# JuliaMolSim/DFTK.jl

Hardware: AMD Instinct MI355X
Metric: SCF iterations/sec (Hψ applies/sec) at fixed Ecut·atoms (higher is better)
Workload: dtype f64

## Files before the change

### dftk.jl_amd/_lib.py

```python
from __future__ import annotations

import ctypes as C
import os

from . import _build

c_cplx_p = C.c_void_p
_i64 = C.c_int64


class dftk_mi_cplx(C.Structure):
    _fields_ = [("re", C.c_double), ("im", C.c_double)]


class dftk_mi_batch_op(C.Structure):
    _fields_ = ([(name, C.c_int32) for name in ("type", "fiber", "trans", "m", "k", "i0", "mode", "flags", "join_next",
                                                 "sync_after", "status", "reserved")] +
                [(name, _i64) for name in ("n", "gm", "gn", "gk", "lda", "ldb", "ldc")] +
                [("alpha", dftk_mi_cplx), ("beta", dftk_mi_cplx), ("s0", C.c_double)] +
                [(name, C.c_void_p) for name in ("A", "B", "W", "W2", "W3", "C", "D", "E", "F", "kb", "host")] +
                [("bytes", C.c_uint64)])


class DftkMiError(RuntimeError):
    def __init__(self, status, msg):
        super().__init__(f"dftk_mi355x status {status}: {msg}")
        self.status = status


_SIGNATURES = {
    "dftk_mi_last_error": (C.c_char_p, []),
    "dftk_mi_version": (C.c_char_p, []),
    "dftk_mi_basis_create": (C.c_int, [C.c_int, C.c_int, C.c_int, C.c_double, C.c_int, C.POINTER(C.c_void_p)]),
    "dftk_mi_basis_destroy": (C.c_int, [C.c_void_p]),
    "dftk_mi_basis_sync": (C.c_int, [C.c_void_p]),
    "dftk_mi_basis_set_fft_batch": (C.c_int, [C.c_void_p, C.c_int]),
    "dftk_mi_basis_stream": (C.c_void_p, [C.c_void_p]),
    "dftk_mi_kblock_create": (C.c_int, [C.c_void_p, _i64, C.c_void_p, C.c_void_p, C.POINTER(C.c_void_p)]),
    "dftk_mi_kblock_destroy": (C.c_int, [C.c_void_p]),
    "dftk_mi_kblock_set_projectors": (C.c_int, [C.c_void_p, C.c_int, C.c_void_p, _i64, C.c_void_p]),
    "dftk_mi_kblock_set_potential": (C.c_int, [C.c_void_p, C.c_void_p]),
    "dftk_mi_apply_H": (C.c_int, [C.c_void_p, C.c_int, C.c_void_p, _i64, C.c_void_p, _i64]),
    "dftk_mi_apply_H_parts": (C.c_int, [C.c_void_p, C.c_int, C.c_int, C.c_void_p, _i64, C.c_void_p, _i64]),
    "dftk_mi_local_potential": (C.c_int, [C.c_void_p, C.c_void_p, C.c_void_p, C.c_void_p, C.c_int, C.c_void_p,
                                          C.c_void_p]),
    "dftk_mi_local_potential_collinear": (C.c_int, [C.c_void_p, C.c_void_p, C.c_void_p, C.c_void_p, C.c_int, C.c_void_p,
                                                    C.c_void_p]),
    "dftk_mi_density_accumulate_spin": (C.c_int, [C.c_void_p, C.c_int, C.c_void_p, _i64, C.c_void_p, C.c_void_p, C.c_int,
                                                  C.c_int]),
    "dftk_mi_kpoint_sphere_host": (C.c_int, [C.c_int, C.c_int, C.c_int, C.c_void_p, C.c_void_p, C.c_double, _i64,
                                             C.POINTER(_i64), C.c_void_p, C.c_void_p, C.c_void_p]),
    "dftk_mi_build_projectors_hgh": (C.c_int, [C.c_void_p, _i64, C.c_void_p, C.c_void_p, C.c_void_p, C.c_double, C.c_int,
                                               C.c_void_p, C.c_void_p, C.c_int, C.c_void_p, C.c_void_p, C.c_void_p, _i64,
                                               C.POINTER(C.c_int)]),
    "dftk_mi_atomic_superposition": (C.c_int, [C.c_void_p, C.c_int, C.c_void_p, C.c_int, C.c_void_p, C.c_int, C.c_void_p,
                                               C.c_void_p, C.c_void_p]),
    "dftk_mi_forces_local": (C.c_int, [C.c_void_p, C.c_void_p, C.c_int, C.c_void_p, C.c_int, C.c_void_p, C.c_void_p,
                                       C.c_void_p, C.c_void_p]),
    "dftk_mi_radial_transform": (C.c_int, [C.c_void_p, C.c_int, C.c_int, C.c_int, C.c_void_p, C.c_void_p, C.c_double, _i64,
                                           C.c_void_p, C.c_void_p]),
    "dftk_mi_radial_tile": (C.c_int, []),
    "dftk_mi_build_projectors_radial": (C.c_int, [C.c_void_p, _i64, C.c_void_p, C.c_void_p, C.c_void_p, C.c_double,
                                                  C.c_int, C.c_void_p, _i64, C.c_void_p, C.c_void_p, C.c_int, C.c_void_p,
                                                  C.c_void_p, C.c_void_p, _i64, C.POINTER(C.c_int)]),
    "dftk_mi_atomic_superposition_table": (C.c_int, [C.c_void_p, C.c_void_p, C.c_int, C.c_void_p, C.c_int, C.c_void_p,
                                                     C.c_void_p, C.c_void_p, C.c_void_p]),
    "dftk_mi_forces_local_table": (C.c_int, [C.c_void_p, C.c_void_p, C.c_int, C.c_void_p, C.c_int, C.c_void_p, C.c_void_p,
                                             C.c_void_p, C.c_void_p]),
    "dftk_mi_forces_nonlocal": (C.c_int, [C.c_void_p, C.c_void_p, C.c_int, C.c_void_p, _i64, C.c_void_p, C.c_int,
                                          C.c_void_p, C.c_void_p]),
    "dftk_mi_local_potential_displacement": (C.c_int, [C.c_void_p, C.c_void_p, C.c_int, C.c_void_p, C.c_int, C.c_void_p,
                                                       C.c_void_p]),
    "dftk_mi_dynmat_local": (C.c_int, [C.c_void_p, C.c_void_p, C.c_int, C.c_void_p, C.c_int, C.c_void_p, C.c_void_p,
                                       C.c_void_p, C.c_void_p]),
    "dftk_mi_nonlocal_displacement_apply": (C.c_int, [C.c_void_p, C.c_void_p, C.c_int, C.c_int, C.c_void_p, C.c_int,
                                                      C.c_void_p, _i64, C.c_void_p, _i64]),
    "dftk_mi_dynmat_nonlocal": (C.c_int, [C.c_void_p, C.c_void_p, C.c_int, C.c_void_p, _i64, C.c_void_p, _i64, C.c_void_p,
                                          C.c_void_p, C.c_int, C.c_void_p, C.c_void_p, C.c_void_p]),
    "dftk_mi_stress_kinetic_nonlocal": (C.c_int, [C.c_void_p, C.c_void_p, C.c_void_p, C.c_int, C.c_void_p, _i64, C.c_void_p,
                                                  C.c_int, C.c_void_p, C.c_void_p, C.c_int, C.c_void_p, C.c_void_p,
                                                  C.c_void_p, C.c_void_p]),
    "dftk_mi_stress_cube": (C.c_int, [C.c_void_p, C.c_void_p, C.c_int, C.c_void_p, C.c_int, C.c_void_p, C.c_void_p,
                                      C.c_void_p, C.c_void_p]),
    "dftk_mi_stress_xc": (C.c_int, [C.c_void_p, _i64, C.c_int, C.c_void_p, C.c_void_p, C.c_void_p, C.c_void_p, C.c_void_p,
                                    C.c_void_p]),
    "dftk_mi_xc_gga": (C.c_int, [C.c_void_p, _i64, C.c_void_p, C.c_void_p, C.c_int, C.c_double, C.c_void_p, C.c_void_p,
                                 C.c_void_p]),
    "dftk_mi_ifft_sphere": (C.c_int, [C.c_void_p, C.c_void_p, C.c_void_p]),
    "dftk_mi_fft_sphere": (C.c_int, [C.c_void_p, C.c_void_p, C.c_void_p]),
    "dftk_mi_density_accumulate": (C.c_int, [C.c_void_p, C.c_int, C.c_void_p, _i64, C.c_void_p, C.c_void_p]),
    "dftk_mi_sternheimer": (C.c_int, [C.c_void_p, C.c_int, C.c_void_p, _i64, C.c_void_p, C.c_int, C.c_void_p, _i64, C.c_void_p,
                                      _i64, C.c_void_p, C.c_int, C.c_int, C.c_void_p, _i64, C.c_void_p, _i64,
                                      C.POINTER(C.c_int), C.c_void_p, C.POINTER(C.c_int)]),
    "dftk_mi_density_response_accumulate": (C.c_int, [C.c_void_p, C.c_int, C.c_void_p, _i64, C.c_void_p, _i64, C.c_void_p,
                                                      C.c_void_p, C.c_void_p]),
    "dftk_mi_apply_kernel": (C.c_int, [C.c_void_p, C.c_void_p, C.c_void_p, C.c_void_p, C.c_int, C.c_void_p]),
    "dftk_mi_exx_apply": (C.c_int, [C.c_void_p, C.c_int, C.c_void_p, _i64, C.c_void_p, C.c_void_p, C.c_int, C.c_void_p, _i64,
                                    C.c_void_p, _i64, C.c_int]),
    "dftk_mi_lobpcg": (C.c_int, [C.c_void_p, C.c_int, C.c_void_p, _i64, C.c_double, C.c_int, C.c_int, C.c_int,
                                 C.c_int, C.c_uint64, C.c_void_p, C.c_void_p, C.POINTER(C.c_int),
                                 C.POINTER(C.c_int), C.POINTER(_i64)]),
    "dftk_mi_local_potential_gga": (C.c_int, [C.c_void_p, C.c_void_p, C.c_void_p, C.c_void_p, C.c_void_p, C.c_int,
                                              C.c_double, C.c_void_p, C.c_void_p]),
    "dftk_mi_local_potential_collinear_gga": (C.c_int, [C.c_void_p, C.c_void_p, C.c_void_p, C.c_void_p, C.c_void_p, C.c_int,
                                                        C.c_double, C.c_void_p, C.c_void_p]),
    "dftk_mi_local_potential_core": (C.c_int, [C.c_void_p, C.c_void_p, C.c_int, C.c_void_p, C.c_void_p, C.c_void_p,
                                               C.c_void_p, C.c_void_p, C.c_int, C.c_double, C.c_void_p, C.c_void_p]),
    "dftk_mi_cube_gradient": (C.c_int, [C.c_void_p, C.c_void_p, C.c_void_p, C.c_void_p]),
    "dftk_mi_xc_gga_spin": (C.c_int, [C.c_void_p, _i64, C.c_void_p, C.c_void_p, C.c_int, C.c_double, C.c_void_p, C.c_void_p,
                                      C.c_void_p]),
    "dftk_mi_symmetrize_rho": (C.c_int, [C.c_void_p, C.c_int, C.c_void_p, C.c_void_p, C.c_int, C.c_void_p, C.c_void_p]),
    "dftk_mi_mix_kerker": (C.c_int, [C.c_void_p, C.c_void_p, C.c_double, C.c_void_p, C.c_void_p]),
    "dftk_mi_mix_dielectric": (C.c_int, [C.c_void_p, C.c_void_p, C.c_double, C.c_double, C.c_void_p, C.c_void_p]),
    "dftk_mi_chi0_dielectric_apply": (C.c_int, [C.c_void_p, C.c_void_p, C.c_double, C.c_double, C.c_void_p, C.c_void_p]),
    "dftk_mi_cube_fourier_filter": (C.c_int, [C.c_void_p, C.c_void_p, C.c_void_p, C.c_void_p]),
    "dftk_mi_kblocks_set_potential": (C.c_int, [C.c_int, C.c_void_p, C.c_void_p]),
    "dftk_mi_lobpcg_multi": (C.c_int, [C.c_int, C.c_void_p, C.c_int, C.c_void_p, C.c_void_p, C.c_double, C.c_int, C.c_int,
                                       C.c_int, C.c_int, C.c_void_p, C.c_void_p, C.c_void_p, C.c_void_p, C.c_void_p,
                                       C.c_void_p, C.c_void_p]),
    "dftk_mi_density_accumulate_multi": (C.c_int, [C.c_int, C.c_void_p, C.c_void_p, C.c_void_p, C.c_void_p, C.c_void_p,
                                                   C.c_void_p]),
    "dftk_mi_density_accumulate_multi2": (C.c_int, [C.c_int, C.c_void_p, C.c_void_p, C.c_void_p, C.c_void_p, C.c_void_p,
                                                    C.c_void_p, C.c_void_p, C.c_void_p]),
    "dftk_mi_band_kinetic_multi": (C.c_int, [C.c_int, C.c_void_p, C.c_void_p, C.c_void_p, C.c_void_p, C.c_void_p]),
    "dftk_mi_batch_stats": (C.c_int, [C.POINTER(_i64), C.POINTER(_i64), C.POINTER(_i64), C.POINTER(_i64)]),
    "dftk_mi_lobpcg_small_stats": (C.c_int, [C.POINTER(_i64), C.POINTER(_i64)]),
    "dftk_mi_ortho_small": (C.c_int, [C.c_void_p, _i64, C.c_int, C.c_void_p, _i64, C.c_int, C.c_void_p, _i64, C.c_void_p,
                                      C.c_double, C.c_void_p]),
    "dftk_mi_batch_replay": (C.c_int, [C.c_void_p, C.c_int, C.c_int, C.c_void_p]),
    "dftk_mi_lobpcg_last_AX": (C.c_void_p, [C.c_void_p]),
    "dftk_mi_lobpcg_history": (C.c_int, [C.c_void_p, C.POINTER(C.c_int), C.POINTER(C.c_int), C.c_void_p, C.c_size_t,
                                         C.POINTER(C.c_int)]),
    "dftk_mi_columnwise_norms": (C.c_int, [C.c_void_p, _i64, C.c_int, C.c_void_p, _i64, C.c_void_p]),
    "dftk_mi_columnwise_dots": (C.c_int, [C.c_void_p, _i64, C.c_int, C.c_void_p, _i64, C.c_void_p, _i64, C.c_void_p]),
    "dftk_mi_ortho_qr": (C.c_int, [C.c_void_p, _i64, C.c_int, C.c_void_p, _i64, C.c_int, C.POINTER(C.c_int),
                                   C.POINTER(C.c_int)]),
    "dftk_mi_tpa_precondprep": (C.c_int, [C.c_void_p, C.c_int, C.c_void_p, _i64, C.c_void_p]),
    "dftk_mi_tpa_ldiv": (C.c_int, [C.c_void_p, C.c_int, C.c_void_p, _i64, C.c_void_p, C.c_double, C.c_void_p, _i64]),
    "dftk_mi_block_residual": (C.c_int, [C.c_void_p, C.c_int, C.c_void_p, _i64, C.c_void_p, _i64, C.c_void_p,
                                         C.c_void_p, _i64, C.c_void_p, C.c_void_p, C.c_void_p]),
    "dftk_mi_kblock_set_gamma_real": (C.c_int, [C.c_void_p, C.c_int]),
    "dftk_mi_gamma_half_size": (C.c_int, [C.c_void_p, C.POINTER(_i64)]),
    "dftk_mi_gamma_tables_host": (C.c_int, [C.c_int, C.c_int, C.c_int, _i64, C.c_void_p, C.POINTER(_i64), C.c_void_p,
                                            C.c_void_p]),
    "dftk_mi_gamma_compress": (C.c_int, [C.c_void_p, C.c_int, C.c_void_p, _i64, C.c_void_p, _i64]),
    "dftk_mi_gamma_compress_aligned": (C.c_int, [C.c_void_p, C.c_int, C.c_void_p, _i64, C.c_void_p, _i64]),
    "dftk_mi_gamma_expand": (C.c_int, [C.c_void_p, C.c_int, C.c_void_p, _i64, C.c_void_p, _i64]),
    "dftk_mi_gamma_apply_H": (C.c_int, [C.c_void_p, C.c_int, C.c_int, C.c_void_p, _i64, C.c_void_p, _i64]),
    "dftk_mi_density_accumulate_real": (C.c_int, [C.c_void_p, C.c_int, C.c_void_p, _i64, C.c_void_p, C.c_void_p]),
    "dftk_mi_shard_plan_host": (C.c_int, [C.c_int, C.c_int, C.c_int, C.c_void_p, C.c_void_p, C.c_void_p, C.c_void_p,
                                          C.c_void_p, C.c_void_p]),
    "dftk_mi_kblock_set_shard": (C.c_int, [C.c_void_p, C.c_void_p, C.c_void_p]),
    "dftk_mi_zgemm": (C.c_int, [C.c_void_p, C.c_char, _i64, _i64, _i64, dftk_mi_cplx, C.c_void_p, _i64,
                                C.c_void_p, _i64, dftk_mi_cplx, C.c_void_p, _i64]),
    "dftk_mi_zgemm_ex": (C.c_int, [C.c_void_p, C.c_char, _i64, _i64, _i64, dftk_mi_cplx, C.c_void_p, _i64,
                                   C.c_void_p, _i64, dftk_mi_cplx, C.c_void_p, _i64, C.c_int]),
    "dftk_mi_zgemm_plan_host": (C.c_int, [C.c_char, _i64, _i64, _i64, C.c_int, C.POINTER(C.c_int)]),
    "dftk_mi_heev": (C.c_int, [C.c_void_p, C.c_int, C.c_void_p, _i64, C.c_void_p, C.c_void_p, _i64]),
    "dftk_mi_prof_zgemm_shapes": (C.c_int, [C.c_void_p, C.c_int, C.c_void_p, C.c_void_p, C.POINTER(C.c_int)]),
    "dftk_mi_heev_lowest": (C.c_int, [C.c_void_p, C.c_int, C.c_int, C.c_void_p, _i64, C.c_void_p, C.c_void_p, _i64]),
    "dftk_mi_heev_sigma_host": (C.c_int, [C.c_int, C.c_void_p, C.c_int, C.POINTER(C.c_double), C.POINTER(C.c_double),
                                          C.POINTER(C.c_int), C.c_double]),
    "dftk_mi_potrf_trtri": (C.c_int, [C.c_void_p, C.c_int, C.c_void_p, _i64, C.c_void_p, _i64]),
    "dftk_mi_potrf_trtri_real": (C.c_int, [C.c_void_p, C.c_int, C.c_void_p, _i64, C.c_void_p, _i64]),
    "dftk_mi_comm_get_unique_id": (C.c_int, [C.c_char_p]),
    "dftk_mi_comm_init_rank": (C.c_int, [C.c_char_p, C.c_int, C.c_int, C.c_int, C.POINTER(C.c_void_p)]),
    "dftk_mi_comm_create_host": (C.c_int, [C.c_int, C.c_int, C.c_int, C.c_void_p, C.c_void_p, C.c_void_p,
                                           C.POINTER(C.c_void_p)]),
    "dftk_mi_comm_destroy": (C.c_int, [C.c_void_p]),
    "dftk_mi_comm_describe": (C.c_int, [C.c_void_p, C.POINTER(C.c_int), C.POINTER(C.c_int), C.POINTER(C.c_int)]),
    "dftk_mi_comm_rank": (C.c_int, [C.c_void_p]),
    "dftk_mi_comm_size": (C.c_int, [C.c_void_p]),
    "dftk_mi_allreduce_sum_f64": (C.c_int, [C.c_void_p, C.c_void_p, C.c_size_t, C.c_void_p]),
    "dftk_mi_prof_enable": (C.c_int, [C.c_void_p, C.c_int]),
    "dftk_mi_prof_get": (C.c_int, [C.c_void_p, C.c_int, C.POINTER(C.c_double), C.POINTER(C.c_double),
                                   C.POINTER(_i64)]),
    "dftk_mi_anderson_create": (C.c_int, [C.c_void_p, _i64, C.c_int, C.c_double, C.c_double, C.POINTER(C.c_void_p)]),
    "dftk_mi_anderson_destroy": (C.c_int, [C.c_void_p]),
    "dftk_mi_anderson_reset": (C.c_int, [C.c_void_p]),
    "dftk_mi_anderson_history": (C.c_int, [C.c_void_p]),
    "dftk_mi_anderson_step": (C.c_int, [C.c_void_p, C.c_void_p, C.c_double, C.c_void_p, C.c_void_p, C.POINTER(C.c_int)]),
    "dftk_mi_chi0_mix": (C.c_int, [C.c_void_p, C.c_int, C.c_void_p, C.c_void_p, C.c_void_p, C.c_double, C.c_int, C.c_double,
                                   C.c_double, C.c_void_p, C.c_double, C.c_int, C.c_int, C.c_void_p, C.POINTER(C.c_int),
                                   C.POINTER(C.c_int)]),
    "dftk_mi_launch_count": (C.c_int, [C.POINTER(_i64), C.POINTER(_i64)]),
    "dftk_mi_device_buffers_live": (C.c_int, [C.POINTER(_i64), C.POINTER(_i64)]),
    "dftk_mi_kblock_reuse_AX": (C.c_int, [C.c_void_p, C.c_int]),
    "dftk_mi_ax_reuse_count": (C.c_int, [C.POINTER(_i64)]),
    "dftk_mi_planes_reuse_count": (C.c_int, [C.POINTER(_i64)]),
    "dftk_mi_step_sums": (C.c_int, [C.c_void_p, _i64, C.c_void_p, C.c_void_p, C.c_void_p, C.c_void_p]),
    "dftk_mi_fermi_bisection": (C.c_int, [C.c_int, C.c_void_p, C.c_void_p, C.c_void_p, C.c_int, C.c_double, C.c_double,
                                          C.c_double, C.c_double, C.c_double, C.POINTER(C.c_double)]),
    "dftk_mi_diag_mfma_peak": (C.c_int, [C.c_void_p, C.c_int, C.c_int, C.POINTER(C.c_double)]),
    "dftk_mi_jacobi_schedule_host": (C.c_int, [C.c_int, C.c_int, C.POINTER(C.c_int), C.POINTER(C.c_int),
                                               C.POINTER(C.c_int)]),
    "dftk_mi_fft_plan_host": (C.c_int, [C.c_int, C.POINTER(C.c_int), C.POINTER(C.c_int), C.POINTER(C.c_int)]),
    "dftk_mi_sphere_tables_host": (C.c_int, [C.c_int, C.c_int, C.c_int, _i64, C.c_void_p, C.POINTER(_i64),
                                             C.POINTER(C.c_int), C.c_void_p, C.c_void_p]),
}

ALLREDUCE_FN = C.CFUNCTYPE(C.c_int, C.c_void_p, C.POINTER(C.c_double), C.c_size_t)
ALLTOALLV_FN = C.CFUNCTYPE(C.c_int, C.c_void_p, C.POINTER(C.c_double), C.POINTER(C.c_size_t), C.POINTER(C.c_size_t),
                           C.POINTER(C.c_double), C.POINTER(C.c_size_t), C.POINTER(C.c_size_t))

EXPORTED_SYMBOLS = tuple(_SIGNATURES)
_lib = None


def load(build_if_missing: bool = True):
    global _lib
    if _lib is not None:
        return _lib
    path = _build.LIBPATH
    if build_if_missing and _build.needs_build():
        _build.build()
    if not os.path.exists(path):
        raise RuntimeError(f"{path} is missing and could not be built; the MI355X hot path has no fallback")
    lib = C.CDLL(path, mode=C.RTLD_GLOBAL)
    for name, (res, args) in _SIGNATURES.items():
        fn = getattr(lib, name)
        fn.restype = res
        fn.argtypes = args
    version = lib.dftk_mi_version().decode()
    if not version.endswith("src=" + _build.source_hash()):
        raise RuntimeError(f"{path} was built from other sources ({version!r}, expected src={_build.source_hash()}): "
                           "stale binary, rebuild with python -m dftk_jl_amd._build")
    _lib = lib
    return lib


def check(status: int):
    if status != 0:
        msg = load().dftk_mi_last_error().decode(errors="replace")
        raise DftkMiError(status, msg)


def cplx(z) -> dftk_mi_cplx:
    z = complex(z)
    return dftk_mi_cplx(z.real, z.imag)
```

### dftk.jl_amd/csrc/api.cpp

```cpp
#include "common.h"
#include <chrono>
#include "batch.h"
#include <algorithm>
#include <cmath>
#include <cstdarg>
#include <cstdio>
#include <cstdlib>
#include <cstring>
#include <vector>

static thread_local char g_err[1024] = "";

void dftk_set_error(const char* fmt, ...) {
    va_list ap;
    va_start(ap, fmt);
    vsnprintf(g_err, sizeof(g_err), fmt, ap);
    va_end(ap);
}

extern "C" const char* dftk_mi_last_error(void) { return g_err; }

hipError_t dftk_scratch_malloc(void** p, size_t bytes) {
    static const bool poison = getenv("DFTK_MI_POISON") != nullptr;
    hipError_t e = hipMalloc(p, bytes);
// ... 1075 lines not shown
    HIPCHK(hipSetDevice(b->device));
    return stress_xc(b, n, n_spin, rho_d, vrho_d, e_d, vsigma_d, grad_d, out_h);
}

extern "C" int dftk_mi_xc_gga(dftk_mi_basis* b, int64_t n, const double* rho_d, const double* sigma_d, int xc_functionals,
                              double density_threshold, double* e_d, double* vrho_d, double* vsigma_d) {
    if (!b || n < 0 || !rho_d || !sigma_d || !e_d || !vrho_d || !vsigma_d || (xc_functionals & ~24) || !xc_functionals)
        return DFTK_MI_EINVAL;
    if (n == 0) return 0;
    HIPCHK(hipSetDevice(b->device));
    return xc_gga_pointwise(b, n, rho_d, sigma_d, xc_functionals, density_threshold, e_d, vrho_d, vsigma_d);
}

extern "C" int dftk_mi_xc_gga_spin(dftk_mi_basis* b, int64_t n, const double* rho_d, const double* sigma_d,
                                   int xc_functionals, double density_threshold, double* e_d, double* vrho_d,
                                   double* vsigma_d) {
    if (!b || n < 0 || !rho_d || !sigma_d || !e_d || !vrho_d || !vsigma_d || (xc_functionals & ~24) || !xc_functionals)
        return DFTK_MI_EINVAL;
    if (n == 0) return 0;
    HIPCHK(hipSetDevice(b->device));
    return xc_gga_spin_pointwise(b, n, rho_d, sigma_d, xc_functionals, density_threshold, e_d, vrho_d, vsigma_d);
}

extern "C" int dftk_mi_ifft_sphere(dftk_mi_kblock* kb, const dftk_mi_cplx* c_d, dftk_mi_cplx* cube_d) {
    if (!kb || !c_d || !cube_d) return DFTK_MI_EINVAL;
    HIPCHK(hipSetDevice(kb->basis->device));
    return launch_ifft_to_cube(kb, reinterpret_cast<const cd*>(c_d), reinterpret_cast<cd*>(cube_d));
}

extern "C" int dftk_mi_fft_sphere(dftk_mi_kblock* kb, const dftk_mi_cplx* cube_d, dftk_mi_cplx* c_d) {
    if (!kb || !c_d || !cube_d) return DFTK_MI_EINVAL;
    HIPCHK(hipSetDevice(kb->basis->device));
    return launch_fft_from_cube(kb, reinterpret_cast<const cd*>(cube_d), reinterpret_cast<cd*>(c_d));
}

extern "C" int dftk_mi_density_accumulate(dftk_mi_kblock* kb, int n_bands, const dftk_mi_cplx* psi_d, int64_t ld_psi,
                                          const double* weight_h, double* rho_d) {
    if (!kb || !psi_d || !weight_h || !rho_d || n_bands < 0 || ld_psi < local_rows(kb)) return DFTK_MI_EINVAL;
    if (n_bands == 0) return 0;
    HIPCHK(hipSetDevice(kb->basis->device));
    if (!kb->sh_comm) {
        prof_count(kb->basis, PROF_A2A_MODEL, 16.0 * (double)kb->n_G * n_bands);
        return launch_density(kb, n_bands, reinterpret_cast<const cd*>(psi_d), ld_psi, weight_h, rho_d);
    }
    if (ld_psi != local_rows(kb)) {
        dftk_set_error("sharded density: blocks must be packed (leading dimension == local rows)");
        return DFTK_MI_EINVAL;
    }
    cd *R1, *F, *Gf;
    CHK(shard_buffers(kb, n_bands, &R1, &F, &Gf));
    Transposer t(kb, n_bands);
    CHK(t.to_bands(reinterpret_cast<const cd*>(psi_d), R1, F));
    if (t.mine == 0) return 0;
    return launch_density(kb, t.mine, F, kb->n_G, weight_h + t.c0[t.me], rho_d);
}

extern "C" int dftk_mi_density_accumulate_spin(dftk_mi_kblock* kb, int n_bands, const dftk_mi_cplx* psi_d, int64_t ld_psi,
                                               const double* weight_h, double* rho_d, int spin, int n_spin) {
    if (!kb || !rho_d || n_spin < 1 || n_spin > 2 || spin < 0 || spin >= n_spin) return DFTK_MI_EINVAL;
    const int64_t N = (int64_t)kb->basis->nx * kb->basis->ny * kb->basis->nz;
    return dftk_mi_density_accumulate(kb, n_bands, psi_d, ld_psi, weight_h, rho_d + (int64_t)spin * N);
}

extern "C" int dftk_mi_kblock_set_gamma_real(dftk_mi_kblock* kb, int on) {
    if (!kb) return DFTK_MI_EINVAL;
    HIPCHK(hipSetDevice(kb->basis->device));
    return gamma_enable(kb, on);
}

extern "C" int dftk_mi_gamma_tables_host(int nx, int ny, int nz, int64_t n_G, const int64_t* mapping0_h,
                                         int64_t* n_half, int32_t* row_h, int32_t* partner_row_h) {
    if (nx < 1 || ny < 1 || nz < 1 || n_G < 1 || !mapping0_h || !n_half) return DFTK_MI_EINVAL;
    if ((row_h == nullptr) != (partner_row_h == nullptr)) return DFTK_MI_EINVAL;
    return gamma_tables_host(nx, ny, nz, n_G, mapping0_h, n_half, row_h, partner_row_h);
}

static int gamma_ready(dftk_mi_kblock* kb) {
    if (!kb || !kb->gr || !kb->gr->d_g) {
        dftk_set_error("gamma_real: call dftk_mi_kblock_set_gamma_real(kb, 1) first");
        return DFTK_MI_EINVAL;
    }
    return 0;
}

extern "C" int dftk_mi_gamma_half_size(dftk_mi_kblock* kb, int64_t* n_half) {
    if (!n_half) return DFTK_MI_EINVAL;
    CHK(gamma_ready(kb));
    *n_half = gamma_local_rows(kb);
    return 0;
}

extern "C" int dftk_mi_gamma_compress(dftk_mi_kblock* kb, int m, const dftk_mi_cplx* X_d, int64_t ldx,
                                      dftk_mi_cplx* Xh_d, int64_t ldh) {
    CHK(gamma_ready(kb));
    if (m < 0 || !X_d || !Xh_d || ldx < local_rows(kb) || ldh < gamma_local_rows(kb)) return DFTK_MI_EINVAL;
    HIPCHK(hipSetDevice(kb->basis->device));
    if (kb->sh_comm)
        return gamma_lobpcg_load(kb, m, reinterpret_cast<const cd*>(X_d), ldx, reinterpret_cast<cd*>(Xh_d), ldh);
    return gamma_compress(kb, m, reinterpret_cast<const cd*>(X_d), ldx, reinterpret_cast<cd*>(Xh_d), ldh);
}

extern "C" int dftk_mi_gamma_compress_aligned(dftk_mi_kblock* kb, int m, const dftk_mi_cplx* X_d, int64_t ldx,
                                              dftk_mi_cplx* Xh_d, int64_t ldh) {
    CHK(gamma_ready(kb));
    if (m < 0 || !X_d || !Xh_d || ldx < local_rows(kb) || ldh < gamma_local_rows(kb)) return DFTK_MI_EINVAL;
    HIPCHK(hipSetDevice(kb->basis->device));
    return gamma_lobpcg_load(kb, m, reinterpret_cast<const cd*>(X_d), ldx, reinterpret_cast<cd*>(Xh_d), ldh, true);
}

extern "C" int dftk_mi_gamma_expand(dftk_mi_kblock* kb, int m, const dftk_mi_cplx* Xh_d, int64_t ldh,
                                    dftk_mi_cplx* X_d, int64_t ldx) {
    CHK(gamma_ready(kb));
    if (m < 0 || !X_d || !Xh_d || ldx < local_rows(kb) || ldh < gamma_local_rows(kb)) return DFTK_MI_EINVAL;
    HIPCHK(hipSetDevice(kb->basis->device));
    if (kb->sh_comm)
        return gamma_lobpcg_store(kb, m, reinterpret_cast<const cd*>(Xh_d), ldh, reinterpret_cast<cd*>(X_d), ldx);
    return gamma_expand(kb, m, reinterpret_cast<const cd*>(Xh_d), ldh, reinterpret_cast<cd*>(X_d), ldx);
}

extern "C" int dftk_mi_gamma_apply_H(dftk_mi_kblock* kb, int which, int n_bands, const dftk_mi_cplx* psih_d,
                                     int64_t ld_psi, dftk_mi_cplx* Hpsih_d, int64_t ld_Hpsi) {
    CHK(gamma_ready(kb));
    if (!psih_d || !Hpsih_d || n_bands < 0 || (which & ~7) || ld_psi < gamma_local_rows(kb) ||
        ld_Hpsi < gamma_local_rows(kb))
        return DFTK_MI_EINVAL;
    HIPCHK(hipSetDevice(kb->basis->device));
    return gamma_apply_H(kb, which, n_bands, reinterpret_cast<const cd*>(psih_d), ld_psi,
                         reinterpret_cast<cd*>(Hpsih_d), ld_Hpsi);
}

extern "C" int dftk_mi_density_accumulate_real(dftk_mi_kblock* kb, int n_bands, const dftk_mi_cplx* psi_d,
                                               int64_t ld_psi, const double* weight_h, double* rho_d) {
    if (!kb || !psi_d || !weight_h || !rho_d || n_bands < 0 || ld_psi < local_rows(kb)) return DFTK_MI_EINVAL;
    if (n_bands == 0) return 0;
    HIPCHK(hipSetDevice(kb->basis->device));
    if (!kb->sh_comm) prof_count(kb->basis, PROF_A2A_MODEL, 8.0 * (double)kb->n_G * n_bands);
    return gamma_density(kb, n_bands, reinterpret_cast<const cd*>(psi_d), ld_psi, weight_h, rho_d);
}

extern "C" int dftk_mi_lobpcg(dftk_mi_kblock* kb, int M, dftk_mi_cplx* X_d, int64_t ldX, double tol, int miniter,
                              int maxiter, int n_conv_check, int use_tpa, uint64_t seed, double* lambda_h,
                              double* resid_h, int* n_iter, int* converged, int64_t* n_matvec) {
    if (!kb || !X_d || M < 1 || ldX < local_rows(kb) || !lambda_h || !resid_h || !n_iter || !converged || !n_matvec ||
        maxiter < 0)
        return DFTK_MI_EINVAL;
    HIPCHK(hipSetDevice(kb->basis->device));
    return lobpcg_run(kb, M, reinterpret_cast<cd*>(X_d), ldX, tol, miniter, maxiter, n_conv_check, use_tpa, seed,
                      lambda_h, resid_h, n_iter, converged, n_matvec);
}

extern "C" int dftk_mi_lobpcg_multi(int n_kblocks, dftk_mi_kblock* const* kbs, int M, dftk_mi_cplx* const* X_d,
                                    const int64_t* ldX, double tol, int miniter, int maxiter, int n_conv_check, int use_tpa,
                                    const uint64_t* seeds, double* lambda_h, double* resid_h, int* n_iter, int* converged,
                                    int64_t* n_matvec, int* status) {
    if (n_kblocks < 0 || (n_kblocks > 0 && (!kbs || !X_d || !ldX || !lambda_h || !resid_h || !n_iter || !converged ||
                                            !n_matvec || !status)) || M < 1 || maxiter < 0)
        return DFTK_MI_EINVAL;
    if (n_kblocks == 0) return 0;
    for (int i = 0; i < n_kblocks; ++i)
        if (!kbs[i] || !X_d[i] || ldX[i] < local_rows(kbs[i])) return DFTK_MI_EINVAL;
    HIPCHK(hipSetDevice(kbs[0]->basis->device));
    return lobpcg_run_multi(n_kblocks, kbs, M, reinterpret_cast<cd* const*>(X_d), ldX, tol, miniter, maxiter, n_conv_check,
                            use_tpa, seeds, lambda_h, resid_h, n_iter, converged, n_matvec, status);
}

extern "C" int dftk_mi_band_kinetic_multi(int n_kblocks, dftk_mi_kblock* const* kbs, const int* n_bands,
                                          const dftk_mi_cplx* const* psi_d, const int64_t* ld_psi, double* out_h) {
    if (n_kblocks < 0 || (n_kblocks > 0 && (!kbs || !n_bands || !psi_d || !ld_psi || !out_h))) return DFTK_MI_EINVAL;
    if (n_kblocks == 0) return 0;
    dftk_mi_basis* b = kbs[0] ? kbs[0]->basis : nullptr;
    if (!b) return DFTK_MI_EINVAL;
    size_t total = 0;
    for (int i = 0; i < n_kblocks; ++i) {
        if (!kbs[i] || kbs[i]->basis != b || kbs[i]->sh_comm || !psi_d[i] || n_bands[i] < 0 || ld_psi[i] < kbs[i]->n_G)
            return DFTK_MI_EINVAL;
        total += (size_t)n_bands[i];
    }
    HIPCHK(hipSetDevice(b->device));
    CHK(ensure_ws(b, total * sizeof(double)));
    double* d = reinterpret_cast<double*>(b->ws.get());
    std::vector<std::function<int()>> bodies;
    size_t off = 0;
    for (int i = 0; i < n_kblocks; ++i) {
        const size_t o = off;
        off += (size_t)n_bands[i];
        bodies.push_back([=]() {
            if (n_bands[i] == 0) return 0;
            CHK(ew_weighted_colsums(b, kbs[i]->n_G, n_bands[i], reinterpret_cast<const cd*>(psi_d[i]), ld_psi[i], kbs[i]->d_kin,
                                    d + o));
            return dev_d2h_sync(b, out_h + o, d + o, (size_t)n_bands[i] * sizeof(double));
        });
    }
    std::vector<int> rets;
    CHK(batch_run(b, bodies, rets));
    for (int r : rets)
        if (r != 0) return r;
    return 0;
}

extern "C" int dftk_mi_density_accumulate_multi(int n_kblocks, dftk_mi_kblock* const* kbs, const int* n_bands,
                                                const dftk_mi_cplx* const* psi_d, const int64_t* ld_psi,
                                                const double* weights_h, double* rho_d) {
    return dftk_mi_density_accumulate_multi2(n_kblocks, kbs, n_bands, psi_d, ld_psi, weights_h, rho_d, nullptr, nullptr);
}

extern "C" int dftk_mi_density_accumulate_multi2(int n_kblocks, dftk_mi_kblock* const* kbs, const int* n_bands,
                                                 const dftk_mi_cplx* const* psi_d, const int64_t* ld_psi,
                                                 const double* weights_h, double* rho_d, const double* weights2_h,
                                                 double* rho2_d) {
    if (n_kblocks < 0 || (n_kblocks > 0 && (!kbs || !n_bands || !psi_d || !ld_psi || !weights_h)) || !rho_d ||
        ((weights2_h == nullptr) != (rho2_d == nullptr)) || (rho2_d && rho2_d == rho_d))
        return DFTK_MI_EINVAL;
    if (n_kblocks == 0) return 0;
    dftk_mi_basis* b = kbs[0] ? kbs[0]->basis : nullptr;
    if (!b) return DFTK_MI_EINVAL;
    for (int i = 0; i < n_kblocks; ++i)
        if (!kbs[i] || kbs[i]->basis != b || kbs[i]->sh_comm || !psi_d[i] || n_bands[i] < 0 || ld_psi[i] < kbs[i]->n_G)
            return DFTK_MI_EINVAL;
    HIPCHK(hipSetDevice(b->device));
    std::vector<std::function<int()>> bodies;
    size_t off = 0;
    for (int i = 0; i < n_kblocks; ++i) {
        const double* w = weights_h + off;
        const double* w2 = weights2_h ? weights2_h + off : nullptr;
        off += (size_t)n_bands[i];
        bodies.push_back([=]() {
            return launch_density(kbs[i], n_bands[i], reinterpret_cast<const cd*>(psi_d[i]), ld_psi[i], w, rho_d, nullptr, w2,
                                  rho2_d);
        });
    }
    std::vector<int> rets;
    CHK(batch_run(b, bodies, rets));
    for (int r : rets)
        if (r != 0) return r;
    return 0;
}

extern "C" int dftk_mi_fermi_bisection(int n_k, const int* n_bands, const double* eig, const double* kweights, int smearing,
                                       double temperature, double filled, double n_electrons, double lo, double hi,
                                       double* eF_out) {
    if (n_k < 1 || !n_bands || !eig || !kweights || !eF_out || !(temperature > 0.0) || (smearing != 1 && smearing != 2) ||
        !(lo <= hi))
        return DFTK_MI_EINVAL;
    auto excess = [&](double eF) {
        double total = 0.0;
        const double* e = eig;
        for (int k = 0; k < n_k; ++k) {
            double sk = 0.0;
            for (int i = 0; i < n_bands[k]; ++i) {
                const double x = (e[i] - eF) / temperature;
                double f;
                if (smearing == 2) {
                    f = 0.5 * std::erfc(x);
                } else if (x > 0) {
                    const double y = std::exp(-x);
                    f = y / (1.0 + y);
                } else {
                    f = 1.0 / (1.0 + std::exp(x));
                }
                sk += filled * f;
            }
            total += kweights[k] * sk;
            e += n_bands[k];
        }
        return total - n_electrons;
    };
    for (int it = 0; it < 200; ++it) {
        const double mid = 0.5 * (lo + hi);
        if (mid == lo || mid == hi) break;
        if (excess(mid) < 0)
            lo = mid;
        else
            hi = mid;
    }
    *eF_out = 0.5 * (lo + hi);
    return 0;
}

extern "C" int dftk_mi_kblock_reuse_AX(dftk_mi_kblock* kb, int on) {
    if (!kb) return DFTK_MI_EINVAL;
    kb->ho.promise(on != 0);
    return 0;
}

extern "C" const dftk_mi_cplx* dftk_mi_lobpcg_last_AX(dftk_mi_kblock* kb) {
    return kb ? reinterpret_cast<const dftk_mi_cplx*>(kb->ho.last_AX()) : nullptr;
}

extern "C" int dftk_mi_zgemm(dftk_mi_basis* b, char transA, int64_t m, int64_t n, int64_t k, dftk_mi_cplx alpha,
                             const dftk_mi_cplx* A_d, int64_t lda, const dftk_mi_cplx* B_d, int64_t ldb,
                             dftk_mi_cplx beta, dftk_mi_cplx* C_d, int64_t ldc) {
    if (!b || m < 0 || n < 0 || k < 0 || !C_d) return DFTK_MI_EINVAL;
    HIPCHK(hipSetDevice(b->device));
    cd al = {alpha.re, alpha.im}, be = {beta.re, beta.im};
    return zgemm(b, transA, m, n, k, al, reinterpret_cast<const cd*>(A_d), lda, reinterpret_cast<const cd*>(B_d), ldb,
                 be, reinterpret_cast<cd*>(C_d), ldc);
}

int zgemm_plan_host(char transA, int64_t m, int64_t n, int64_t k, int flags, int* out);
extern "C" int dftk_mi_zgemm_plan_host(char transA, int64_t m, int64_t n, int64_t k, int flags, int* out12) {
    return zgemm_plan_host(transA, m, n, k, flags, out12);
}

extern "C" int dftk_mi_zgemm_ex(dftk_mi_basis* b, char transA, int64_t m, int64_t n, int64_t k, dftk_mi_cplx alpha,
                                const dftk_mi_cplx* A_d, int64_t lda, const dftk_mi_cplx* B_d, int64_t ldb,
                                dftk_mi_cplx beta, dftk_mi_cplx* C_d, int64_t ldc, int flags) {
    if (!b || m < 0 || n < 0 || k < 0 || !C_d || (flags & ~(3 | DFTK_MI_GEMM_REAL))) return DFTK_MI_EINVAL;
    HIPCHK(hipSetDevice(b->device));
    cd al = {alpha.re, alpha.im}, be = {beta.re, beta.im};
    return zgemm(b, transA, m, n, k, al, reinterpret_cast<const cd*>(A_d), lda, reinterpret_cast<const cd*>(B_d), ldb,
                 be, reinterpret_cast<cd*>(C_d), ldc, flags);
}

extern "C" int dftk_mi_heev(dftk_mi_basis* b, int n, dftk_mi_cplx* A_d, int64_t lda, double* W_h, dftk_mi_cplx* V_d,
                            int64_t ldv) {
    if (!b || n < 1 || !A_d || !W_h || !V_d || lda < n || ldv < n) return DFTK_MI_EINVAL;
    HIPCHK(hipSetDevice(b->device));
    return dense_heev(b, n, reinterpret_cast<cd*>(A_d), lda, W_h, reinterpret_cast<cd*>(V_d), ldv);
}

extern "C" int dftk_mi_heev_lowest(dftk_mi_basis* b, int n, int nev, dftk_mi_cplx* A_d, int64_t lda, double* W_h,
                                   dftk_mi_cplx* V_d, int64_t ldv) {
    if (!b || n < 1 || nev < 1 || nev > n || !A_d || !W_h || !V_d || lda < n || ldv < n) return DFTK_MI_EINVAL;
    HIPCHK(hipSetDevice(b->device));
    return dense_heev_lowest(b, n, nev, reinterpret_cast<cd*>(A_d), lda, W_h, reinterpret_cast<cd*>(V_d), ldv);
}
extern "C" int dftk_mi_heev_sigma_host(int n, const double* diag_h, int nev, double* sigma, double* gap_guess,
                                       int* hold_iterations, double norm_bound) {
    const int st = eig_choose_sigma_host(n, diag_h, nev, sigma, gap_guess);
    if (st != 0) return st;
    if (hold_iterations) *hold_iterations = norm_bound > 0.0 ? eig_hold_iterations_host(*gap_guess / norm_bound) : 0;
    return 0;
}

extern "C" int dftk_mi_potrf_trtri(dftk_mi_basis* b, int n, dftk_mi_cplx* A_d, int64_t lda, dftk_mi_cplx* invR_d,
                                   int64_t ldi) {
    if (!b || n < 1 || !A_d || !invR_d || lda < n || ldi < n) return DFTK_MI_EINVAL;
    HIPCHK(hipSetDevice(b->device));
    double a, c;
    return dense_potrf_trtri(b, n, reinterpret_cast<cd*>(A_d), lda, reinterpret_cast<cd*>(invR_d), ldi, &a, &c);
}

extern "C" int dftk_mi_potrf_trtri_real(dftk_mi_basis* b, int n, dftk_mi_cplx* A_d, int64_t lda, dftk_mi_cplx* invR_d,
                                        int64_t ldi) {
    if (!b || n < 1 || !A_d || !invR_d || lda < n || ldi < n) return DFTK_MI_EINVAL;
    HIPCHK(hipSetDevice(b->device));
    double a, c;
    return dense_potrf_trtri(b, n, reinterpret_cast<cd*>(A_d), lda, reinterpret_cast<cd*>(invR_d), ldi, &a, &c, true);
}

extern "C" int dftk_mi_lobpcg_history(dftk_mi_kblock* kb, int* M_out, int* n_iter_out, double* hist_h, size_t cap,
                                      int* n_svd_out) {
    if (!kb || kb->lob_hist.empty()) return DFTK_MI_EINVAL;
    if (M_out) *M_out = kb->lob_hist_M;
    if (n_iter_out) *n_iter_out = kb->lob_hist_iters;
    if (n_svd_out) *n_svd_out = kb->lob_n_svd;
    if (hist_h) {
        if (cap < kb->lob_hist.size()) return DFTK_MI_EINVAL;
        std::copy(kb->lob_hist.begin(), kb->lob_hist.end(), hist_h);
    }
    return 0;
}

static int fetch(dftk_mi_basis* b, const double* d, double* h, size_t n) {
    HIPCHK(hipMemcpyAsync(h, d, n * sizeof(double), hipMemcpyDeviceToHost, b->stream));
    HIPCHK(hipStreamSynchronize(b->stream));
    return 0;
}

extern "C" int dftk_mi_columnwise_norms(dftk_mi_basis* b, int64_t n, int m, const dftk_mi_cplx* X_d, int64_t ldx,
                                        double* norms_h) {
    if (!b || !X_d || !norms_h || n < 0 || m < 0 || ldx < n || m > 100000) return DFTK_MI_EINVAL;
    if (m == 0) return 0;
    HIPCHK(hipSetDevice(b->device));
    CHK(ensure_ws(b, (size_t)m * sizeof(double)));
    double* d = reinterpret_cast<double*>(b->ws.get());
    CHK(ew_colnorms(b, n, m, reinterpret_cast<const cd*>(X_d), ldx, d));
    return fetch(b, d, norms_h, m);
}

extern "C" int dftk_mi_columnwise_dots(dftk_mi_basis* b, int64_t n, int m, const dftk_mi_cplx* A_d, int64_t lda,
                                       const dftk_mi_cplx* B_d, int64_t ldb, dftk_mi_cplx* dots_h) {
    if (!b || !A_d || !B_d || !dots_h || n < 0 || m < 0 || lda < n || ldb < n) return DFTK_MI_EINVAL;
    if (m == 0) return 0;
    HIPCHK(hipSetDevice(b->device));
    CHK(ensure_ws(b, 2 * (size_t)m * sizeof(double)));
    double* d = reinterpret_cast<double*>(b->ws.get());
    CHK(ew_coldots(b, n, m, reinterpret_cast<const cd*>(A_d), lda, reinterpret_cast<const cd*>(B_d), ldb, d));
    CHK(ew_coldots_im(b, n, m, reinterpret_cast<const cd*>(A_d), lda, reinterpret_cast<const cd*>(B_d), ldb, d + m));
    std::vector<double> h(2 * (size_t)m);
    CHK(fetch(b, d, h.data(), h.size()));
    for (int i = 0; i < m; ++i) {
        dots_h[i].re = h[i];
        dots_h[i].im = h[m + i];
    }
    return 0;
}

extern "C" int dftk_mi_ortho_qr(dftk_mi_basis* b, int64_t n, int m, dftk_mi_cplx* X_d, int64_t ldx, int force_svd,
                                int* n_chol, int* used_svd) {
    if (!b || !X_d || n < 1 || m < 0 || ldx < n || m > n) return DFTK_MI_EINVAL;
    HIPCHK(hipSetDevice(b->device));
    return lobpcg_ortho(b, n, m, reinterpret_cast<cd*>(X_d), ldx, force_svd, n_chol, used_svd);
}

extern "C" int dftk_mi_tpa_precondprep(dftk_mi_kblock* kb, int m, const dftk_mi_cplx* X_d, int64_t ldx,
                                       double* mean_kin_h) {
    if (!kb || !X_d || !mean_kin_h || m < 0 || ldx < kb->n_G || kb->sh_comm) return DFTK_MI_EINVAL;
    if (m == 0) return 0;
    dftk_mi_basis* b = kb->basis;
    HIPCHK(hipSetDevice(b->device));
    CHK(ensure_ws(b, (size_t)m * sizeof(double)));
    double* d = reinterpret_cast<double*>(b->ws.get());
    CHK(ew_weighted_colsums(b, kb->n_G, m, reinterpret_cast<const cd*>(X_d), ldx, kb->d_kin, d));
    return fetch(b, d, mean_kin_h, m);
}

extern "C" int dftk_mi_tpa_ldiv(dftk_mi_kblock* kb, int m, const dftk_mi_cplx* R_d, int64_t ldr,
                                const double* mean_kin_h, double default_shift, dftk_mi_cplx* Y_d, int64_t ldy) {
    if (!kb || !R_d || !Y_d || m < 0 || ldr < kb->n_G || ldy < kb->n_G || kb->sh_comm) return DFTK_MI_EINVAL;
    if (m == 0) return 0;
    dftk_mi_basis* b = kb->basis;
    HIPCHK(hipSetDevice(b->device));
    CHK(ensure_ws(b, 2 * (size_t)m * sizeof(double)));
    double* d = reinterpret_cast<double*>(b->ws.get());
    if (mean_kin_h) {
        HIPCHK(hipMemcpyAsync(d, mean_kin_h, m * sizeof(double), hipMemcpyHostToDevice, b->stream));
        HIPCHK(hipStreamSynchronize(b->stream));
    }
    return ew_tpa(b, kb->n_G, m, reinterpret_cast<const cd*>(R_d), ldr, reinterpret_cast<cd*>(Y_d), ldy, kb->d_kin,
                  mean_kin_h ? d : nullptr, d + m, default_shift);
}

extern "C" int dftk_mi_block_residual(dftk_mi_kblock* kb, int m, const dftk_mi_cplx* AX_d, int64_t lda,
                                      const dftk_mi_cplx* X_d, int64_t ldx, const double* lambda_h, dftk_mi_cplx* R_d,
                                      int64_t ldr, double* norms_h, double* mean_kin_h, double* xx_h) {
    if (!kb || !AX_d || !X_d || !lambda_h || !R_d || !norms_h || m < 0 || lda < kb->n_G || ldx < kb->n_G ||
        ldr < kb->n_G || kb->sh_comm)
        return DFTK_MI_EINVAL;
    if (m == 0) return 0;
    dftk_mi_basis* b = kb->basis;
    HIPCHK(hipSetDevice(b->device));
    CHK(ensure_ws(b, 4 * (size_t)m * sizeof(double)));
    double* d = reinterpret_cast<double*>(b->ws.get());
    HIPCHK(hipMemcpyAsync(d, lambda_h, m * sizeof(double), hipMemcpyHostToDevice, b->stream));
    CHK(ew_residual(b, kb->n_G, m, reinterpret_cast<const cd*>(AX_d), lda, reinterpret_cast<const cd*>(X_d), ldx, d,
                    reinterpret_cast<cd*>(R_d), ldr, d + m, kb->d_kin, d + 2 * m, d + 3 * m));
    std::vector<double> h(3 * (size_t)m);
    CHK(fetch(b, d + m, h.data(), h.size()));
    for (int i = 0; i < m; ++i) {
        norms_h[i] = h[i];
        if (mean_kin_h) mean_kin_h[i] = h[m + i];
        if (xx_h) xx_h[i] = h[2 * m + i];
    }
    return 0;
}
```

### dftk.jl_amd/csrc/common.h

```cpp
#pragma once
#include <hip/hip_runtime.h>
#include <stdint.h>
#include <stddef.h>
#include <string>
#include <map>
#include <vector>
#include <memory>
#include "devbuf.h"
#include "handover.h"
#include "../../include/dftk_mi355x.h"

typedef double2 cd;

#include <atomic>
extern std::atomic<int64_t> g_dftk_launches, g_dftk_host_syncs;
inline hipError_t dftk_counted_stream_sync(hipStream_t s) {
    g_dftk_host_syncs.fetch_add(1, std::memory_order_relaxed);
    return (hipStreamSynchronize)(s);
}
#define hipStreamSynchronize(s) dftk_counted_stream_sync(s)
#undef hipLaunchKernelGGL
#define hipLaunchKernelGGL(kernelName, ...)                               \
    do {                                                                  \
        g_dftk_launches.fetch_add(1, std::memory_order_relaxed);          \
        hipLaunchKernelGGLInternal((kernelName), __VA_ARGS__);            \
    } while (0)

void dftk_set_error(const char* fmt, ...);
hipError_t dftk_scratch_malloc(void** p, size_t bytes);

#define HIPCHK(expr)                                                                      \
    do {                                                                                  \
        hipError_t _e = (expr);                                                           \
        if (_e != hipSuccess) {                                                           \
            dftk_set_error("%s failed: %s (%s:%d)", #expr, hipGetErrorString(_e), __FILE__, __LINE__); \
            return DFTK_MI_EHIP;                                                          \
        }                                                                                 \
    } while (0)

#define CHK(expr)                                 \
    do {                                          \
        int _s = (expr);                          \
        if (_s != 0) return _s;                   \
    } while (0)

struct WsCarver {
    void** slot[16];
    size_t at[16];
    int n = 0;
    size_t off = 0;
    template <class T>
    void take(T** p, size_t count) {
        slot[n] = reinterpret_cast<void**>(p);
        at[n++] = off;
        off += (count * sizeof(T) + 255) & ~(size_t)255;
    }
    size_t bytes() const { return off; }
    void bind(void* base) const {
        for (int i = 0; i < n; ++i) *slot[i] = static_cast<char*>(base) + at[i];
    }
};

template <int K>
__device__ inline void block_reduce(double* v) {
    __shared__ double sh[K][256];
#pragma unroll
    for (int k = 0; k < K; ++k) sh[k][threadIdx.x] = v[k];
    __syncthreads();
    for (int h = 128; h > 0; h >>= 1) {
        if ((int)threadIdx.x < h)
#pragma unroll
            for (int k = 0; k < K; ++k) sh[k][threadIdx.x] += sh[k][threadIdx.x + h];
        __syncthreads();
    }
    if (threadIdx.x == 0)
#pragma unroll
        for (int k = 0; k < K; ++k) v[k] = sh[k][0];
}

__device__ __forceinline__ double wave_sum(double v) {
#pragma unroll
    for (int off = 32; off > 0; off >>= 1) v += __shfl_down(v, off, 64);
    return v;
}
template <int NT>
__device__ __forceinline__ double block_sum(double v, double* sh) {
    v = wave_sum(v);
    const int lane = threadIdx.x & 63, w = threadIdx.x >> 6;
    if (lane == 0) sh[w] = v;
    __syncthreads();
    double r = 0.0;
    if (threadIdx.x == 0) {
#pragma unroll
        for (int i = 0; i < NT / 64; ++i) r += sh[i];
    }
    __syncthreads();
    return r;
}

#define DFTK_MAX_RADICES 32
struct FftAxis {
    int n;
    int nrad;
    int rad[DFTK_MAX_RADICES];
    const cd* tw;
    const int* pos;
};

int  plan_radices(int n, int* nrad, int* rad);
void plan_positions(int n, int nrad, const int* rad, int* pos);

struct StreamOwner {
    hipStream_t s = nullptr;
    StreamOwner() = default;
    StreamOwner(const StreamOwner&) = delete;
    StreamOwner& operator=(const StreamOwner&) = delete;
    ~StreamOwner() { if (s) hipStreamDestroy(s); }
    operator hipStream_t() const { return s; }
};
struct dftk_mi_basis {
    int nx = 0, ny = 0, nz = 0, nxp = 0;
    double volume = 0.0;
    int device = 0;
    StreamOwner stream;
    FftAxis ax[3] = {};
    DevTable<void> d_tables[6];
    int fft_batch = 0;
    DevBuf<cd> T1;
    DevBuf<cd> T2;
    DevBuf<void> ws;
    DevTable<double> d_scalars;
    PinnedBuf<double> h_scalars;
    Buf<char, Mem::PinnedMapped> h_fetch;
    int use_mfma = 0;
    std::unique_ptr<struct Prof> prof;
    DevBuf<void> dense_ws;
    DevBuf<void> eig_ws;
    struct dftk_mi_comm* comm = nullptr;
    DevTable<void> symm_tab; uint64_t symm_key = 0; int symm_n = 0;
    DevBuf<void> resp_ws;
    DevBuf<void> exx_ws;
};

enum ProfFamily {
    PROF_ZGEMM = 0,
    PROF_FFT_A = 1,
    PROF_FFT_B = 2,
    PROF_FFT_C = 3,
    PROF_FFT_D = 4,
    PROF_FFT_E = 5,
    PROF_DENS_Z = 6,
    PROF_HEEV = 7,
    PROF_CHOL = 8,
    PROF_APPLY_H = 9,
    PROF_ZGEMM_BYTES = 10,
    PROF_ZGEMM_STRUCT = 11,
    PROF_ZGEMM_EXEC = 12,
    PROF_COMM = 13,
    PROF_ZGEMM_CPLX = 14,
    PROF_EW = 15,
    PROF_HOST_WAIT = 16,
    PROF_AR_MODEL = 17,
    PROF_A2A_MODEL = 18,
    PROF_NFAM = 24
};
struct Prof {
    bool on = false;
    struct Pair { hipEvent_t a, b; int fam; uint64_t tag; double work; };
    struct Shape { double ms = 0, work = 0; int64_t n = 0; };
    std::map<uint64_t, Shape> shapes;
    std::vector<Pair> pending;
    std::vector<Pair> pool;
    int open = 0;
    int mute = 0;
    bool shape_tags = false;
    double ms[PROF_NFAM] = {0};
    double work[PROF_NFAM] = {0};
    int64_t launches[PROF_NFAM] = {0};
    Prof() = default;
    Prof(const Prof&) = delete;
    Prof& operator=(const Prof&) = delete;
    ~Prof() {
        for (auto* v : {&pending, &pool})
            for (auto& pr : *v) {
                hipEventDestroy(pr.a);
                hipEventDestroy(pr.b);
            }
    }
};
int prof_begin(dftk_mi_basis* b, int fam, double work, uint64_t tag = 0);
void prof_end(dftk_mi_basis* b, int slot);
int prof_resolve(dftk_mi_basis* b);
struct ProfScope {
    dftk_mi_basis* b;
    int slot;
    ProfScope(dftk_mi_basis* basis, int fam, double work) : b(basis), slot(prof_begin(basis, fam, work)) {}
    ~ProfScope() { prof_end(b, slot); }
    ProfScope(const ProfScope&) = delete;
    ProfScope& operator=(const ProfScope&) = delete;
};
void prof_count(dftk_mi_basis* b, int fam, double work);
const size_t HOST_FETCH_BYTES = 256 * 1024;
int host_wait(dftk_mi_basis* b);
int host_fetch(dftk_mi_basis* b, void* dst_h, const void* src_d, size_t bytes);

struct GammaReal {
    bool on = false;
    int64_t n_half = 0;
    DevTable<int> d_g, d_mg;
    DevTable<double> d_kin_half;
    DevTable<cd> P_half;
    const cd* P_src = nullptr;
    int P_n_p = 0;
    DevBuf<cd> buf;
    std::vector<int64_t> half_rows;
};

struct dftk_mi_kblock {
    dftk_mi_basis* basis = nullptr;
    int device = 0;
    int64_t n_G = 0;
    int64_t n_lines = 0;
    int nzx = 0;
    int z_lo = 0;
    DevTable<int> d_cpos;
    DevTable<int> d_line_start;
    DevTable<int> d_line_ypos;
    DevTable<int> d_zls;
    DevTable<int> d_zpos;
    DevTable<int> d_zval;
    DevTable<int> d_line_yval;
    DevTable<int> d_cx;
    DevTable<double> d_kin;
    std::shared_ptr<DevTable<double>> Vs_buf;
    bool Vs_shared = false;
    double* d_Vs = nullptr;
    int n_p = 0;
    const cd* P = nullptr;
    int64_t ldP = 0;
    DevTable<double> d_D;
    int D_bw = 0;
    DevBuf<cd> lob_buf;
    LobHandover ho;
    dftk_mi_comm* sh_comm = nullptr;
    std::vector<int64_t> sh_rows;
    DevBuf<cd> sh_buf;
    std::vector<double> lob_hist; int lob_hist_M = 0, lob_hist_iters = 0, lob_n_svd = 0;
    std::vector<int64_t> h_mapping;
    std::vector<double> h_kin;
    std::unique_ptr<GammaReal> gr;
    DevTable<int32_t> d_G3;
};

int fft_ensure_scratch(dftk_mi_basis* b, dftk_mi_kblock* kb, int nb);
int launch_local_apply(dftk_mi_kblock* kb, int nb, const cd* psi, int64_t ldpsi, cd* out,
                       int64_t ldout, bool add_kinetic, bool have_local, const double* shift_d = nullptr);
int launch_ifft_to_cube(dftk_mi_kblock* kb, const cd* c, cd* cube, int nb = 1);
int launch_fft_from_cube(dftk_mi_kblock* kb, const cd* cube, cd* c, int nb = 1);
int launch_density(dftk_mi_kblock* kb, int nb, const cd* psi, int64_t ldpsi, const double* w_h, double* rho,
                   const double* w_im_h = nullptr, const double* w2_h = nullptr, double* rho2 = nullptr,
                   bool keep_planes = false);
int fft_group_size(const dftk_mi_basis* b);
int launch_planes_fill(dftk_mi_kblock* kb, int b0, int nbb, const cd* psi, int64_t ldpsi, cd* planes);
int launch_local_apply_from_planes(dftk_mi_kblock* kb, int nb, cd* planes, cd* out, int64_t ldout);
int launch_density_response(dftk_mi_kblock* kb, int nb, const cd* psi, int64_t ldpsi, const cd* dpsi, int64_t lddpsi,
                            const double* wo_h, const double* wd_h, double* drho);
int launch_pad_potential(dftk_mi_kblock* kb, const double* V);
int launch_kinetic_only(dftk_mi_kblock* kb, int nb, const cd* psi, int64_t ldpsi, cd* out,
                        int64_t ldout, bool accumulate, bool use_kin);

int zgemm(dftk_mi_basis* b, char transA, int64_t m, int64_t n, int64_t k, cd alpha, const cd* A,
          int64_t lda, const cd* B, int64_t ldb, cd beta, cd* C, int64_t ldc, int upper = 0);
int ensure_ws(dftk_mi_basis* b, size_t bytes);
template <class B>
int scratch_grow(dftk_mi_basis* b, B& buf, size_t need, size_t slack = 0) {
    if (need <= buf.bytes()) return 0;
    HIPCHK(hipStreamSynchronize(b->stream));
    HIPCHK(buf.reserve(need, slack));
    return 0;
}

int dense_potrf_trtri(dftk_mi_basis* b, int n, cd* A, int64_t lda, cd* invR, int64_t ldi,
                      double* normest_R, double* normest_invR, bool real_input = false);
int dense_heev(dftk_mi_basis* b, int n, cd* A, int64_t lda, double* W_h, cd* V, int64_t ldv);
int dense_heev_full(dftk_mi_basis* b, int n, cd* A, int64_t lda, double* W_h, cd* V, int64_t ldv);
int dense_input_norms(dftk_mi_basis* b, int n, const cd* A, int64_t lda, double* off2, double* dg2, double* im2);
int dense_heev_lowest(dftk_mi_basis* b, int n, int nev, cd* A, int64_t lda, double* W_h, cd* V, int64_t ldv);
int eig_choose_sigma_host(int n, const double* diag, int nev, double* sigma, double* gap_guess);
int eig_hold_iterations_host(double gap_over_norm);
struct ProfMute {
    dftk_mi_basis* b;
    explicit ProfMute(dftk_mi_basis* basis) : b(basis) { if (b->prof) b->prof->mute += 1; }
    ~ProfMute() { if (b->prof) b->prof->mute -= 1; }
    ProfMute(const ProfMute&) = delete;
    ProfMute& operator=(const ProfMute&) = delete;
};
int jacobi_schedule_host(int n, int round, int* nb_out, int* pairs, int* where);
int apply_D(dftk_mi_kblock* kb, int n_bands, const cd* X , cd* Y);
int ew_colreduce(dftk_mi_basis* b, int mode, int64_t n, int m, const cd* X, int64_t ldx, const cd* Y, int64_t ldy,
                 const double* w, double* out_d);
int ew_colnorms(dftk_mi_basis* b, int64_t n, int m, const cd* X, int64_t ldx, double* out_d);
int ew_coldots(dftk_mi_basis* b, int64_t n, int m, const cd* X, int64_t ldx, const cd* Y, int64_t ldy,
               double* out_re_d);
int ew_residual(dftk_mi_basis* b, int64_t n, int m, const cd* AX, int64_t lda, const cd* X, int64_t ldx,
                const double* lam_d, cd* R, int64_t ldr, double* norms_d, const double* kin, double* mean_kin_d,
                double* xx_d);
int ew_tpa(dftk_mi_basis* b, int64_t n, int m, const cd* src, int64_t lds, cd* dst, int64_t ldd, const double* kin,
           const double* mean_kin_d, double* norms_d, double default_shift = 1.0);
int ew_scale_cols(dftk_mi_basis* b, int64_t n, int m, cd* X, int64_t ldx, const double* s_d, bool invert);
int ew_copy(dftk_mi_basis* b, int64_t n, int m, const cd* X, int64_t ldx, cd* Y, int64_t ldy);
int ew_add(dftk_mi_basis* b, int64_t n, int m, const cd* X, int64_t ldx, cd* Y, int64_t ldy);
int ew_sub_real(dftk_mi_basis* b, int64_t n, const double* a, const double* c, double* out);
int ew_fill_zero(dftk_mi_basis* b, cd* X, size_t count);
int ew_sub_identity_shifted(dftk_mi_basis* b, int rows, int cols, cd* C, int64_t ldc, int row0);
int ew_gather_cols(dftk_mi_basis* b, int64_t n, int m, const cd* X, int64_t ldx, const int* perm_d,
                   cd* Y, int64_t ldy);
int ew_add_diag(dftk_mi_basis* b, int n, cd* A, int64_t lda, double shift);
int ew_frob2(dftk_mi_basis* b, int64_t n, int m, const cd* X, int64_t ldx, double* out_d);
int ew_hermitize_upper(dftk_mi_basis* b, int n, cd* A, int64_t lda);
int ew_conj_transpose(dftk_mi_basis* b, int n, const cd* A, int64_t lda, cd* B, int64_t ldb);
int ew_square(dftk_mi_basis* b, double* d, size_t n);
int ew_sqrt(dftk_mi_basis* b, double* d, size_t n);
int ew_coldots_im(dftk_mi_basis* b, int64_t n, int m, const cd* X, int64_t ldx, const cd* Y, int64_t ldy,
                  double* out_im_d);
int ew_weighted_colsums(dftk_mi_basis* b, int64_t n, int m, const cd* X, int64_t ldx, const double* w_d,
                        double* out_d);

int comm_size(const dftk_mi_comm* c);
int comm_rank(const dftk_mi_comm* c);
int comm_allreduce(dftk_mi_comm* c, dftk_mi_basis* b, double* d, size_t n);
int comm_allreduce_norms(dftk_mi_comm* c, dftk_mi_basis* b, double* d, size_t n);
int comm_alltoallv(dftk_mi_comm* c, dftk_mi_basis* b, const cd* send, const size_t* soff, const size_t* scnt,
                   cd* recv, const size_t* roff, const size_t* rcnt);

int local_potential_collinear(dftk_mi_kblock* cube_kb, const double* rho, const double* core, const double* vloc,
                              const double* green, int fun_mask, double* V_out, double* energies_h);
int local_potential_lda(dftk_mi_kblock* cube_kb, const double* recip_h, const double* rho, const double* core,
                        const double* grad_core, const double* vloc, const double* green, int fun_mask, double threshold,
                        double* V_out, double* energies_h);
int local_potential_collinear_gga(dftk_mi_kblock* cube_kb, const double* recip_h, const double* rho, const double* core,
                                  const double* grad_core, const double* vloc, const double* green, int fun_mask,
                                  double threshold, double* V_out, double* energies_h);
int xc_gga_spin_pointwise(dftk_mi_basis* b, int64_t n, const double* rho, const double* sigma, int fun_mask,
                          double threshold, double* e, double* vrho, double* vsigma);

int apply_kernel_lda(dftk_mi_kblock* cube_kb, const double* rho, const double* drho, const double* green, int fun_mask,
                     double* dV_out);

int cube_symmetrize(dftk_mi_kblock* cube_kb, int n_sym, const int32_t* S_h, const double* tau_h, int do_lowpass,
                    const double* rho_in, double* rho_out);
int cube_fourier_filter(dftk_mi_kblock* cube_kb, int kind, const double* recip_h, double p0, double p1,
                        const double* mult_d, const double* f, double* out);
int cube_gradient(dftk_mi_kblock* cube_kb, const double* recip_h, const double* f, double* grad);
int xc_gga_pointwise(dftk_mi_basis* b, int64_t n, const double* rho, const double* sigma, int fun_mask,
                     double threshold, double* e, double* vrho, double* vsigma);

int sphere_enumerate_host(int nx, int ny, int nz, const double* B, const double* k, double Ecut, int64_t cap,
                          int64_t* n_G_out, int64_t* mapping0, double* kinetic, int32_t* G_out);
int build_projectors_hgh(dftk_mi_basis* b, int64_t n_rows, const int32_t* G_d, const double* recip_h, const double* k_h,
                         double volume, int n_species, const double* rp_h, const int* nproj_h, int n_atoms,
                         const int* species_of_atom_h, const double* positions_h, cd* P_d, int64_t ldP, int* n_p_out);

int atomic_superposition(dftk_mi_kblock* cube_kb, int kind, const double* recip_h, int n_species, const double* par_h,
                         int n_atoms, const int* species_of_atom_h, const double* positions_h, double* out_d);
int build_projectors_radial(dftk_mi_basis* b, int64_t n_rows, const int32_t* G_d, const double* recip_h,
                            const double* k_h, double volume, int n_species, const double* R_d, int64_t ldR,
                            const int* first_chan_h, const int* n_chan_h, int n_atoms, const int* species_of_atom_h,
                            const double* positions_h, cd* P_d, int64_t ldP, int* n_p_out);
int atomic_superposition_table(dftk_mi_kblock* cube_kb, const double* recip_h, int n_species, const double* ff_d,
                               int n_atoms, const int* species_of_atom_h, const double* positions_h,
                               const double* coef_h, double* out_d);
int forces_local_table(dftk_mi_kblock* cube_kb, const double* recip_h, int n_species, const double* ff_d, int n_atoms,
                       const int* species_of_atom_h, const double* positions_h, const double* rho_d, double* forces_h);
int radial_transform(dftk_mi_basis* b, int kind, int l, int n_r, const double* r_h, const double* wf_h, double Zion,
                     int64_t n_q, const double* q_d, double* out_d);
int check_species_grouped(const char* who, int n_species, int n_atoms, const int* species_of_atom_h);
std::vector<cd> phase_tables_host(int nx, int ny, int nz, int n_atoms, const double* positions_h);
struct ProjCol;
int list_projector_columns(int n_species, const double* rp_h, const int* nproj_h, int n_atoms,
                           const int* species_of_atom_h, const double* positions_h, std::vector<ProjCol>* cols,
                           std::vector<int>* col_start = nullptr);

int gamma_tables_host(int nx, int ny, int nz, int64_t n_G, const int64_t* mapping, int64_t* n_half_out, int32_t* g,
                      int32_t* mg);
int gamma_enable(dftk_mi_kblock* kb, int on);
int gamma_compress(dftk_mi_kblock* kb, int m, const cd* X, int64_t ldx, cd* H, int64_t ldh);
int gamma_compress_aligned(dftk_mi_kblock* kb, int m, const cd* X, int64_t ldx, cd* H, int64_t ldh);
int gamma_expand(dftk_mi_kblock* kb, int m, const cd* H, int64_t ldh, cd* X, int64_t ldx);
int gamma_apply_H(dftk_mi_kblock* kb, int which, int nb, const cd* psi, int64_t ldpsi, cd* Hpsi, int64_t ldH);
int gamma_density(dftk_mi_kblock* kb, int nb, const cd* psi, int64_t ldpsi, const double* w_h, double* rho);
int gamma_ensure_buf(dftk_mi_kblock* kb, size_t elems);
int gamma_pack_pairs(dftk_mi_kblock* kb, int nb, const cd* H, int64_t ldh, cd* Z, int64_t ldz);
int gamma_unpack_pairs(dftk_mi_kblock* kb, int nb, const cd* W, int64_t ldw, cd* H, int64_t ldh);
int gamma_pack_full(dftk_mi_kblock* kb, int nb, const cd* X, int64_t ldx, cd* Z, int64_t ldz);
int gamma_gather_P(dftk_mi_kblock* kb, int ncols, const cd* P, int64_t ldP, cd* Ph, int64_t ldh, double* asym_mag_h);
int gamma_density_bands(dftk_mi_kblock* kb, int nb, const cd* psi, int64_t ldpsi, const double* w_h, double* rho);
bool planes_eligible(const dftk_mi_kblock* kb);
int gamma_apply_local_from_planes(dftk_mi_kblock* kb, int nb, const cd* X, int64_t ldx, cd* Hpsi, int64_t ldH);
int64_t gamma_local_rows(const dftk_mi_kblock* kb);
int64_t gamma_row0(const dftk_mi_kblock* kb);
int gamma_projectors(dftk_mi_kblock* kb);
int gamma_projectors_renew(dftk_mi_kblock* kb, size_t elems);
int gamma_apply_H_sharded(dftk_mi_kblock* kb, int which, int nb, const cd* psi, int64_t ldpsi, cd* Hpsi, int64_t ldH);
int gamma_projectors_sharded(dftk_mi_kblock* kb);
int gamma_density_sharded(dftk_mi_kblock* kb, int nb, const cd* psi, int64_t ldpsi, const double* w_h, double* rho);
int gamma_lobpcg_load(dftk_mi_kblock* kb, int M, const cd* Xuser, int64_t ldX, cd* Xh, int64_t ldh, bool align = false);
int gamma_lobpcg_store(dftk_mi_kblock* kb, int M, const cd* Xh, int64_t ldh, cd* Xuser, int64_t ldX);
int apply_nonlocal_rows(dftk_mi_kblock* kb, int nb, const cd* P, int64_t ldP, int64_t rows, const cd* psi,
                        int64_t ldpsi, cd* Hpsi, int64_t ldH, bool accumulate, int gemm_flags, dftk_mi_comm* comm);

int forces_local(dftk_mi_kblock* cube_kb, const double* recip_h, int n_species, const double* par_h, int n_atoms,
                 const int* species_of_atom_h, const double* positions_h, const double* rho_d, double* forces_h);
int forces_nonlocal(dftk_mi_kblock* kb, const double* kcoord_h, int nb, const cd* psi, int64_t ld_psi,
                    const double* weight_h, int n_atoms, const int* col_start_h, double* forces_h);
int ensure_G3(dftk_mi_kblock* kb);
int launch_nl_operands_full(dftk_mi_basis* b, int64_t rows, int nb, int64_t row0, const int* G3, const double* kcoord_h,
                            const cd* psi, int64_t ldpsi, cd* Z, int64_t ldz);
int launch_rowsum(dftk_mi_basis* b, int rows, int64_t n, const double* in, double scale, double* out);
int launch_real_to_cplx(dftk_mi_basis* b, int64_t n, const double* x, cd* y);

int stress_kinetic_nonlocal(dftk_mi_kblock* kb, const double* recip_h, const double* kcoord_h, int nb, const cd* psi,
                            int64_t ld_psi, const double* weight_h, int n_species, const double* rp_h, const int* nproj_h,
                            int n_atoms, const int* species_of_atom_h, const double* positions_h, const int* col_start_h,
                            double* stress_h);
int stress_cube(dftk_mi_kblock* cube_kb, const double* recip_h, int n_species, const double* par_h, int n_atoms,
                const int* species_of_atom_h, const double* positions_h, const double* rho_d, double* out_h);
int stress_xc(dftk_mi_basis* b, int64_t n, int n_spin, const double* rho_d, const double* vrho_d, const double* e_d,
              const double* vsigma_d, const double* grad_d, double* out_h);

int resp_update_xr(dftk_mi_basis* b, int64_t n, int m, const double* gamma_d, const double* pc_d, const cd* p, int64_t ldp,
                   const cd* c, int64_t ldc, cd* x, int64_t ldx, cd* r, int64_t ldr);
int resp_update_p(dftk_mi_basis* b, int64_t n, int m, const double* gamma_new_d, const double* gamma_old_d, const cd* z,
                  int64_t ldz, cd* p, int64_t ldp);
int resp_axpby(dftk_mi_basis* b, int64_t n, int m, double a, const double* sd, const cd* X, int64_t ldx, double bcoef, cd* Y,
               int64_t ldy);
int resp_scale_inv(dftk_mi_basis* b, int n_extra, int m, cd* S, int64_t lds, const double* ee_d, const double* e_d);
int resp_broadcast(dftk_mi_basis* b, int m, const double* src_d, double* dst_d);

int sternheimer_run(dftk_mi_kblock* kb, int n_occ, const cd* psi_occ, int64_t ld_occ, const double* eps_h, int n_extra,
                    const cd* psi_extra, int64_t ld_extra, const cd* rhs, int64_t ld_rhs, const double* tol_h, int miniter,
                    int maxiter, const cd* dpsi0, int64_t ld_dpsi0, cd* dpsi, int64_t ld_dpsi, int* n_iter, double* resid_h,
                    int* converged);



int lobpcg_ortho(dftk_mi_basis* b, int64_t n, int m, cd* X, int64_t ldx, int force_svd, int* n_chol, int* used_svd);
int lobpcg_run_multi(int n_kb, dftk_mi_kblock* const* kbs, int M, cd* const* X, const int64_t* ldX, double tol, int miniter,
                     int maxiter, int n_conv_check, int use_tpa, const uint64_t* seeds, double* lambda_h, double* resid_h,
                     int* n_iter, int* converged, int64_t* n_matvec, int* status);
int lobpcg_run(dftk_mi_kblock* kb, int M, cd* X, int64_t ldX, double tol, int miniter, int maxiter,
               int n_conv_check, int use_tpa, uint64_t seed, double* lambda_h, double* resid_h,
               int* n_iter, int* converged, int64_t* n_matvec);
```

### dftk.jl_amd/csrc/eig_kernels.hip

```cpp
#include "common.h"
#include "batch.h"
#include <cmath>
#include <cstdio>
#include <cstdlib>
#include <cstring>
#include <vector>
#include <numeric>
#include <algorithm>
#include <chrono>

static const double EIG_L_HAT = 1e-2;

namespace {

__global__ __launch_bounds__(256) void k_eig_colstats(int n, const cd* __restrict__ A, int64_t lda,
                                                      double* __restrict__ diag, double* __restrict__ rowabs) {
    __shared__ double sh[4];
    const int j = blockIdx.x;
    double s = 0.0;
    for (int i = threadIdx.x; i < n; i += 256) {
        const cd v = A[i + (int64_t)j * lda];
        s += sqrt(v.x * v.x + v.y * v.y);
    }
    const double t = block_sum<256>(s, sh);
    if (threadIdx.x == 0) {
        rowabs[j] = t;
        diag[j] = A[j + (int64_t)j * lda].x;
    }
}

template <bool REAL>
__global__ __launch_bounds__(256) void k_eig_init(int n, const cd* __restrict__ A, int64_t lda, double sigma, double inv_nrm,
                                                  cd* __restrict__ X, int64_t ldt) {
    const int j = blockIdx.y;
    const int i = blockIdx.x * 256 + threadIdx.x;
    if (REAL) {
        const int nrows = 2 * (int)ldt;
        if (i >= nrows) return;
        double v = 0.0;
        if (i < n) v = (A[i + (int64_t)j * lda].x - (i == j ? sigma : 0.0)) * inv_nrm;
        reinterpret_cast<double*>(X + (int64_t)j * ldt)[i] = v;
    } else {
        if (i >= n) return;
        cd v = A[i + (int64_t)j * lda];
        if (i == j) v.x -= sigma;
        X[i + (int64_t)j * ldt] = make_double2(v.x * inv_nrm, v.y * inv_nrm);
    }
}

#define EPT 32
__global__ __launch_bounds__(256) void k_eig_poly(int n, cd* __restrict__ Y, int64_t ldy, double c1, double c2, int ntile,
                                                  double* __restrict__ part) {
    __shared__ cd tile[EPT][EPT + 1];
    __shared__ double sh[4];
    int t = blockIdx.x, bj = 0;
    while (t > bj) {
        t -= bj + 1;
        ++bj;
    }
    const int bi = t;
    const int tx = threadIdx.x & 31, ty = threadIdx.x >> 5;
    double tr = 0.0, fro = 0.0;
#pragma unroll
    for (int r = 0; r < EPT; r += 8) {
        const int i = bi * EPT + tx, j = bj * EPT + ty + r;
        cd v = make_double2(0.0, 0.0);
        if (i < n && j < n && i <= j) {
            const cd y = Y[i + (int64_t)j * ldy];
            const double dre = (i == j ? 1.0 : 0.0) - y.x;
            const double e2 = dre * dre + y.y * y.y;
            if (i == j) {
                tr += dre;
                fro += dre * dre;
            } else {
                fro += 2.0 * e2;
            }
            v = make_double2((i == j ? c1 : 0.0) + c2 * y.x, i == j ? 0.0 : c2 * y.y);
            Y[i + (int64_t)j * ldy] = v;
        }
        tile[ty + r][tx] = v;
    }
    __syncthreads();
#pragma unroll
    for (int r = 0; r < EPT; r += 8) {
        const int j = bj * EPT + tx, i = bi * EPT + ty + r;
        if (i < n && j < n && i < j) {
            const cd v = tile[tx][ty + r];
            Y[j + (int64_t)i * ldy] = make_double2(v.x, -v.y);
        }
    }
    const double a = block_sum<256>(tr, sh);
    const double f = block_sum<256>(fro, sh);
    if (threadIdx.x == 0) {
        part[2 * blockIdx.x] = a;
        part[2 * blockIdx.x + 1] = f;
    }
    (void)ntile;
}

template <bool REAL>
__global__ void k_eig_diag_tall(int n, const cd* __restrict__ U, int64_t ldt, double* __restrict__ d) {
    const int c = blockIdx.x * blockDim.x + threadIdx.x;
    if (c >= n) return;
    if (REAL)
        d[c] = reinterpret_cast<const double*>(U + (int64_t)c * ldt)[c];
    else
        d[c] = U[c + (int64_t)c * ldt].x;
}

template <bool REAL>
__global__ __launch_bounds__(256) void k_eig_proj_cols(int n, const cd* __restrict__ U, int64_t ldt, const int* __restrict__ sel,
                                                       cd* __restrict__ Bt, int64_t ldb) {
    const int c = blockIdx.y;
    const int s = sel[c];
    const int i = blockIdx.x * 256 + threadIdx.x;
    if (REAL) {
        if (i >= 2 * (int)ldb) return;
        double v = 0.0;
        if (i < n) v = -0.5 * reinterpret_cast<const double*>(U + (int64_t)s * ldt)[i] + (i == s ? 0.5 : 0.0);
        reinterpret_cast<double*>(Bt + (int64_t)c * ldb)[i] = v;
    } else {
        if (i >= n) return;
        const cd u = U[i + (int64_t)s * ldt];
        Bt[i + (int64_t)c * ldb] = make_double2(-0.5 * u.x + (i == s ? 0.5 : 0.0), -0.5 * u.y);
    }
}

__global__ __launch_bounds__(256) void k_eig_tall_to_cd(int n, const cd* __restrict__ T, int64_t ldt, cd* __restrict__ C,
                                                        int64_t ldc) {
    const int c = blockIdx.y;
    const int i = blockIdx.x * 256 + threadIdx.x;
    if (i >= n) return;
    C[i + (int64_t)c * ldc] = make_double2(reinterpret_cast<const double*>(T + (int64_t)c * ldt)[i], 0.0);
}

int ws_ensure(dftk_mi_basis* b, size_t bytes) {
    return scratch_grow(b, b->eig_ws, bytes);
}

double a_of(double l) { return std::sqrt(3.0 / (1.0 + l + l * l)); }
double l_next(double l, double a) { return 0.5 * a * l * (3.0 - a * a * l * l); }

}

int eig_choose_sigma_host(int n, const double* diag, int nev, double* sigma, double* gap_guess) {
    if (n < 2 || nev < 1 || nev >= n || !diag || !sigma || !gap_guess) return DFTK_MI_EINVAL;
    std::vector<double> ds(diag, diag + n);
    std::nth_element(ds.begin(), ds.begin() + (nev - 1), ds.end());
    const double dn = ds[nev - 1];
    const double d1 = *std::min_element(ds.begin(), ds.begin() + nev);
    const double dnext = *std::min_element(ds.begin() + nev, ds.end());
    double spacing = (dn - d1) / std::max(nev - 1, 1);
    if (!(spacing > 0.0)) spacing = 1e-8 * std::max(1.0, std::fabs(dn));
    double margin = 0.5 * spacing;
    const double gap = dnext - dn;
    if (gap > 2.0 * margin) margin = std::min(0.5 * gap, 4.0 * spacing);
    *sigma = dn + margin;
    *gap_guess = 0.2 * margin;
    return 0;
}

int eig_hold_iterations_host(double gap_over_norm) {
    const double grow = 1.5 * a_of(EIG_L_HAT);
    const double l0 = std::max(gap_over_norm, 1e-14);
    if (l0 >= EIG_L_HAT) return 0;
    const int m1 = (int)std::ceil(std::log(EIG_L_HAT / l0) / std::log(grow));
    return std::min(m1, 34);
}

template <bool REAL>
static int heev_lowest_impl(dftk_mi_basis* b, int n, int nev, cd* A, int64_t lda, double* W_h, cd* V, int64_t ldv,
                            bool* fell_back) {
    static const bool trace = getenv("DFTK_MI_HEEV_TRACE") != nullptr;
    const auto t_start = std::chrono::steady_clock::now();
    auto ms_since = [&](const std::chrono::steady_clock::time_point& t0) {
        return std::chrono::duration<double, std::milli>(std::chrono::steady_clock::now() - t0).count();
    };
    *fell_back = true;
    const int rf = REAL ? DFTK_MI_GEMM_REAL : 0;
    const int64_t ldt = REAL ? (n + 1) / 2 : n;
    const int64_t tk = REAL ? ldt : n;
    const int kcap = std::min(n - 1, std::max(nev + 64, (3 * nev) / 2));
    const int ntile1 = (n + EPT - 1) / EPT, ntile = ntile1 * (ntile1 + 1) / 2;
    const size_t szTall = (size_t)ldt * n, szY = (size_t)n * n, szB = (size_t)ldt * kcap, szK = (size_t)kcap * kcap;
    const size_t n_cd = 3 * szTall + szY + 3 * szB + (REAL ? (size_t)n * kcap : 0) + 4 * szK;
    const size_t n_dbl = 3 * (size_t)n + 2 * (size_t)ntile + 64;
    CHK(ws_ensure(b, n_cd * sizeof(cd) + n_dbl * sizeof(double) + (size_t)n * sizeof(int) + 256));
    cd* w = reinterpret_cast<cd*>(b->eig_ws.get());
    auto take = [&](size_t c) {
        cd* r = w;
        w += c;
        return r;
    };
    cd* X0 = take(szTall);
    cd* Xa = take(szTall);
    cd* Xb = take(szTall);
    cd* Y = take(szY);
    cd* Bt[2] = {take(szB), take(szB)};
    cd* Tt = take(szB);
    cd* Bc = REAL ? take((size_t)n * kcap) : nullptr;
    cd* O = take(szK);
    cd* invR = take(szK);
    cd* Gk = take(szK);
    cd* Vk = take(szK);
    double* d_diag = reinterpret_cast<double*>(w);
    double* d_rowabs = d_diag + n;
    double* d_udiag = d_rowabs + n;
    double* d_part = d_udiag + n;
    int* d_sel = reinterpret_cast<int*>(d_part + 2 * ntile + 64);
    const cd ONE = make_double2(1.0, 0.0), ZERO = make_double2(0.0, 0.0);

    hipLaunchKernelGGL(k_eig_colstats, dim3(n), dim3(256), 0, b->stream, n, A, lda, d_diag, d_rowabs);
    std::vector<double> hd(2 * (size_t)n);
    CHK(host_fetch(b, hd.data(), d_diag, hd.size() * sizeof(double)));
    double sigma, gap_guess;
    CHK(eig_choose_sigma_host(n, hd.data(), nev, &sigma, &gap_guess));
    double nrm = 0.0;
    for (int i = 0; i < n; ++i) {
        if (!std::isfinite(hd[i]) || !std::isfinite(hd[n + i])) return DFTK_MI_NUM_NONFINITE;
        nrm = std::max(nrm, std::fabs(hd[i] - sigma) + hd[n + i] - std::fabs(hd[i]));
    }
    nrm *= 1.0 + 1e-8;
    if (!(nrm > 0.0)) return 0;
    const unsigned rowblocks = (unsigned)((2 * ldt + 255) / 256);
    hipLaunchKernelGGL(k_eig_init<REAL>, dim3(rowblocks, n), dim3(256), 0, b->stream, n, A, lda, sigma, 1.0 / nrm, X0, ldt);
    HIPCHK(hipGetLastError());

    cd* Xc = X0;
    cd* Xn = Xa;
    int its = 0;
    std::vector<double> hpart(2 * (size_t)ntile);
    auto gram_poly = [&](double a) -> int {
        CHK(zgemm(b, 'C', n, n, tk, ONE, Xc, ldt, Xc, ldt, ZERO, Y, n, rf | DFTK_MI_GEMM_UPPER));
        hipLaunchKernelGGL(k_eig_poly, dim3(ntile), dim3(256), 0, b->stream, n, Y, (int64_t)n, 1.5 * a, -0.5 * a * a * a, ntile,
                           d_part);
        HIPCHK(hipGetLastError());
        return 0;
    };
    auto advance = [&]() -> int {
        CHK(zgemm(b, 'N', ldt, n, n, ONE, Xc, ldt, Y, n, ZERO, Xn, ldt, rf));
        Xc = Xn;
        Xn = (Xc == Xa) ? Xb : Xa;
        ++its;
        return 0;
    };
    auto error_norm = [&](double* e) -> int {
        CHK(host_fetch(b, hpart.data(), d_part, hpart.size() * sizeof(double)));
        double f = 0.0;
        for (int t = 0; t < ntile; ++t) f += hpart[2 * t + 1];
        if (!std::isfinite(f)) return DFTK_MI_NUM_NONFINITE;
        *e = std::sqrt(f);
        return 0;
    };
    int m1 = eig_hold_iterations_host(gap_guess / nrm);
    bool converged = false;
    int rescues = 0;
    for (; rescues <= 3 && !converged; ++rescues) {
        const double ah = a_of(EIG_L_HAT);
        for (int i = 0; i < m1; ++i) {
            CHK(gram_poly(ah));
            CHK(advance());
        }
        for (double l = EIG_L_HAT; l < 1.0 - 1e-9;) {
            const double a = a_of(l);
            CHK(gram_poly(a));
            CHK(advance());
            l = l_next(l, a);
        }
        for (int chk = 0; chk < 10; ++chk) {
            double e;
            CHK(gram_poly(1.0));
            CHK(error_norm(&e));
            if (trace) fprintf(stderr, "[heev lowest%s] n=%d nev=%d its=%d ||I - X^2||_F=%.3e\n", REAL ? " real" : "", n, nev, its, e);
            if (e < 1e-10) {
                if (e >= 1e-13) CHK(advance());
                converged = true;
                break;
            }
            if (e > 0.9) break;
            CHK(advance());
            if (e < 3e-6) {
                converged = true;
                break;
            }
        }
        m1 = 6;
    }
    if (!converged) {
        if (trace) fprintf(stderr, "[heev lowest] n=%d: no convergence of the sign iteration after %d iterations -> full solver\n", n, its);
        return 0;
    }
    const double ms_sign = ms_since(t_start);
    if (REAL)
        hipLaunchKernelGGL(k_eig_diag_tall<true>, dim3((n + 255) / 256), dim3(256), 0, b->stream, n, Xc, ldt, d_udiag);
    else
        hipLaunchKernelGGL(k_eig_diag_tall<false>, dim3((n + 255) / 256), dim3(256), 0, b->stream, n, Xc, ldt, d_udiag);
    std::vector<double> p(n);
    CHK(host_fetch(b, p.data(), d_udiag, n * sizeof(double)));
    double trP = 0.0;
    for (int i = 0; i < n; ++i) {
        p[i] = 0.5 * (1.0 - p[i]);
        trP += p[i];
    }
    const int k = (int)std::lround(trP);
    if (!(std::fabs(trP - k) < 1e-6) || k < nev || k > kcap) {
        if (trace) fprintf(stderr, "[heev lowest] n=%d nev=%d: trace(P)=%.9f (k cap %d) -> full solver\n", n, nev, trP, kcap);
        return 0;
    }
    std::vector<int> sel(n);
    std::iota(sel.begin(), sel.end(), 0);
    std::stable_sort(sel.begin(), sel.end(), [&](int x, int y) { return p[x] > p[y]; });
    sel.resize(k);
    std::sort(sel.begin(), sel.end());
    HIPCHK(hipMemcpyAsync(d_sel, sel.data(), k * sizeof(int), hipMemcpyHostToDevice, b->stream));
    CHK(host_wait(b));
    hipLaunchKernelGGL(k_eig_proj_cols<REAL>, dim3(rowblocks, k), dim3(256), 0, b->stream, n, Xc, ldt, d_sel, Bt[0], ldt);
    HIPCHK(hipGetLastError());
    int cur = 0;
    for (int pass = 0; pass < 3; ++pass) {
        CHK(zgemm(b, 'C', k, k, tk, ONE, Bt[cur], ldt, Bt[cur], ldt, ZERO, O, k, rf | DFTK_MI_GEMM_UPPER));
        CHK(ew_hermitize_upper(b, k, O, k));
        double nR = 0.0, nI = 0.0;
        const int st = dense_potrf_trtri(b, k, O, k, invR, k, &nR, &nI, REAL);
        if (st > 0) {
            if (trace) fprintf(stderr, "[heev lowest] n=%d k=%d: Cholesky-QR pass %d failed -> full solver\n", n, k, pass);
            return 0;
        }
        if (st != 0) return st;
        CHK(zgemm(b, 'N', ldt, k, k, ONE, Bt[cur], ldt, invR, k, ZERO, Bt[cur ^ 1], ldt, rf | DFTK_MI_GEMM_B_UPPER));
        cur ^= 1;
        const double cond = nR * nI;
        if (trace) fprintf(stderr, "[heev lowest] n=%d k=%d sigma=%.6f its=%d pass %d cond(R)~%.2e\n", n, k, sigma, its, pass, cond);
        if (pass >= 1 && 2.220446049250313e-16 * cond * cond < 1e-15) break;
        if (pass == 0 && cond < 16.0) break;
    }
    cd* Bq = Bt[cur];
    const cd* Bcoef = Bq;
    if (REAL) {
        hipLaunchKernelGGL(k_eig_tall_to_cd, dim3((n + 255) / 256, k), dim3(256), 0, b->stream, n, Bq, ldt, Bc, (int64_t)n);
        Bcoef = Bc;
    }
    CHK(zgemm(b, 'N', ldt, k, n, ONE, X0, ldt, Bcoef, n, ZERO, Tt, ldt, rf));
    CHK(zgemm(b, 'C', k, k, tk, ONE, Bq, ldt, Tt, ldt, ZERO, Gk, k, rf | DFTK_MI_GEMM_UPPER));
    CHK(ew_hermitize_upper(b, k, Gk, k));
    std::vector<double> th(k);
    double ms_basis = 0.0;
    if (trace) {
        CHK(host_wait(b));
        ms_basis = ms_since(t_start) - ms_sign;
    }
    {
        const int st = dense_heev_full(b, k, Gk, k, th.data(), Vk, k);
        if (st != 0) return st;
    }
    if (trace)
        fprintf(stderr, "[heev lowest timing] n=%d nev=%d k=%d its=%d: sign %.2f ms, basis + projection %.2f ms, Jacobi(k) %.2f ms\n", n,
                nev, k, its, ms_sign, ms_basis, ms_since(t_start) - ms_sign - ms_basis);
    if (REAL) {
        CHK(zgemm(b, 'N', ldt, nev, k, ONE, Bq, ldt, Vk, k, ZERO, Tt, ldt, rf));
        hipLaunchKernelGGL(k_eig_tall_to_cd, dim3((n + 255) / 256, nev), dim3(256), 0, b->stream, n, Tt, ldt, V, ldv);
    } else {
        CHK(zgemm(b, 'N', n, nev, k, ONE, Bq, ldt, Vk, k, ZERO, V, ldv, rf));
    }
    HIPCHK(hipGetLastError());
    for (int i = 0; i < nev; ++i) W_h[i] = sigma + nrm * th[i];
    *fell_back = false;
    return 0;
}

int dense_heev_lowest(dftk_mi_basis* b, int n, int nev, cd* A, int64_t lda, double* W_h, cd* V, int64_t ldv) {
    if (n <= 0) return 0;
    static const int min_n = getenv("DFTK_MI_HEEV_PARTIAL_MIN") ? atoi(getenv("DFTK_MI_HEEV_PARTIAL_MIN")) : 384;
    static const bool off = getenv("DFTK_MI_HEEV_PARTIAL") && atoi(getenv("DFTK_MI_HEEV_PARTIAL")) == 0;
    if (off || batching() || !b->use_mfma || n < min_n || nev < 1 || 10 * nev > 6 * n)
        return dense_heev(b, n, A, lda, W_h, V, ldv);
    bool fell_back = true;
    int st;
    {
        ProfScope scope(b, PROF_HEEV, (double)n);
        ProfMute mute(b);
        double off2 = 0.0, dg2 = 0.0, im2 = 0.0;
        CHK(dense_input_norms(b, n, A, lda, &off2, &dg2, &im2));
        if (!std::isfinite(off2 + dg2 + im2)) return DFTK_MI_NUM_NONFINITE;
        st = im2 == 0.0 ? heev_lowest_impl<true>(b, n, nev, A, lda, W_h, V, ldv, &fell_back)
                        : heev_lowest_impl<false>(b, n, nev, A, lda, W_h, V, ldv, &fell_back);
        if (st == 0 && fell_back) return dense_heev_full(b, n, A, lda, W_h, V, ldv);
    }
    if (st != 0) return st;
    static const bool poison = getenv("DFTK_MI_POISON") != nullptr;
    if (poison && nev < n) {
        for (int i = nev; i < n; ++i) W_h[i] = std::nan("");
        HIPCHK(hipMemset2DAsync(V + (int64_t)nev * ldv, (size_t)ldv * sizeof(cd), 0xFF, (size_t)n * sizeof(cd), (size_t)(n - nev),
                                b->stream));
    }
    return 0;
}
```

### dftk.jl_amd/csrc/gemm_kernels.hip

```cpp
#include "common.h"
#include "batch.h"
#include <cstdio>
#include <cstdlib>
#include <type_traits>
#include <map>
#include <vector>
#include <cmath>
#include <algorithm>
#include <mutex>

typedef double v4d __attribute__((ext_vector_type(4)));


#define LT_KT 8
#define GEMM_RM 2
#define GEMM_WAVES 4
#define GEMM_BM (GEMM_WAVES * GEMM_RM * 16)
#define M3_RN 2
#define M3_BN (16 * M3_RN)
#define M3_RN_REAL 4
#define M3_BN_REAL (16 * M3_RN_REAL)
#define M3_MIN_BLOCKS 2
template <bool CONJA, int MODE, bool REAL, int RN>
__global__ __launch_bounds__(GEMM_WAVES * 64, M3_MIN_BLOCKS) void k_zgemm_3m(int m, int n, int K, int kchunk, int gm, int gn,
                                                               int rt0, int ct0, int lsplit, int upper,
                                                               int shift_ct, int shift_rt, int nsplit, const cd* __restrict__ A, int64_t lda,
                                                               const cd* __restrict__ B, int64_t ldb,
                                                               cd* __restrict__ C, int64_t ldc, cd alpha, cd beta,
                                                               cd* __restrict__ slab) {
    constexpr int BN = 16 * RN;
    static_assert(RN == 2 || RN == 4, "B staging handles one or two columns per thread");
    __shared__ cd sA[2][LT_KT][GEMM_BM];
    __shared__ cd sB[2][LT_KT][BN];
    const int id = blockIdx.x;
    const int xcd = id & 7, slot = id >> 3;
    int z, row_t, col_t;
    if (upper & 16) {
        constexpr int q = GEMM_BM / BN;
        int L = 0;
        for (int r = 0; r < gm; ++r) L += max(0, gn - r * q);
        const int N = L * nsplit, per = (N + 7) >> 3;
        const int item = xcd * per + slot;
        if (slot >= per || item >= N) return;
        z = item / L;
        int t = item - z * L, r = 0;
        while (t >= gn - r * q) {
            t -= gn - r * q;
            ++r;
        }
        row_t = r;
        col_t = r * q + t;
    } else if (upper & 4) {
        const int per = gm * gn;
        z = (slot / per) * 8 + xcd;
        const int rem = slot % per;
        row_t = rem / gn;
        col_t = rem - row_t * gn;
        if (z >= nsplit) return;
    } else {
        col_t = slot % gn;
        const int R = (slot / gn) * 8 + xcd;
        if (R >= gm * nsplit) return;
        z = R / gm;
        row_t = R - z * gm;
        if (upper & 8) {
            const int g = (gm % 8 == 0) ? 8 : (gm % 4 == 0) ? 4 : (gm % 2 == 0) ? 2 : 1;
            row_t = (row_t + (z * g) / 8) % gm;
        }
    }

    const int tid = threadIdx.x;
    const int lane = tid & 63, wave = tid >> 6;
    const int li = lane & 15, lk = lane >> 4;
    const int tr = lsplit < 0 ? row_t + rt0 : (row_t < lsplit ? row_t : rt0);
    const int tcn = lsplit < 0 ? col_t + ct0 : (row_t < lsplit ? ct0 : row_t - lsplit);
    const bool shifted = tcn == shift_ct;
    const bool rshifted = tr == shift_rt;
    const int I0 = rshifted ? m - GEMM_BM : tr * GEMM_BM, J0 = shifted ? n - BN : tcn * BN;
    const int jmin = shifted ? tcn * BN : 0, imin = tr * GEMM_BM;
    if ((upper & 1) && imin >= J0 + BN) return;
    const int i0 = I0 + wave * (GEMM_RM * 16);
    const int kbeg = z * kchunk;
    const int kend = min(min(K, kbeg + kchunk), (upper & 2) ? J0 + BN : K);
    constexpr bool FULL = MODE == 1;
    const int rmv = FULL ? GEMM_RM : min(GEMM_RM, max(0, (m - i0 + 15) >> 4));
    const int rnv = FULL ? RN : min(RN, max(0, (n - J0 + 15) >> 4));
    const bool active = FULL || (rmv > 0 && rnv > 0);

    v4d acc1[GEMM_RM][RN], acc2[GEMM_RM][RN], acc3[GEMM_RM][RN];
#pragma unroll
    for (int a = 0; a < GEMM_RM; ++a)
#pragma unroll
        for (int b = 0; b < RN; ++b) {
            acc1[a][b] = (v4d){0.0, 0.0, 0.0, 0.0};
            acc2[a][b] = (v4d){0.0, 0.0, 0.0, 0.0};
            acc3[a][b] = (v4d){0.0, 0.0, 0.0, 0.0};
        }

    const int tk = tid & 7, tc = tid >> 3;
    const cd *pA0, *pA1, *pA2, *pA3, *pB0, *pB1;
    {
        auto a_ptr = [&](int r) -> const cd* {
            if (CONJA) {
                int c = I0 + tc + 32 * r;
                if (c > m - 1) c = m - 1;
                return A + (int64_t)c * lda + kbeg + tk;
            } else {
                int i = I0 + (tid & 127);
                if (i > m - 1) i = m - 1;
                return A + i + (int64_t)(kbeg + (tid >> 7) + 2 * r) * lda;
            }
        };
        auto b_ptr = [&](int r) -> const cd* {
            int c = J0 + tc + 32 * r;
            if (c > n - 1) c = n - 1;
            return B + (int64_t)c * ldb + kbeg + tk;
        };
        pA0 = a_ptr(0);
        pA1 = a_ptr(1);
        pA2 = a_ptr(2);
        pA3 = a_ptr(3);
        pB0 = b_ptr(0);
        pB1 = b_ptr(RN == 4 ? 1 : 0);
    }
    const int64_t stepA = CONJA ? (int64_t)LT_KT : (int64_t)LT_KT * lda;
    struct Stage {
        cd a0, a1, a2, a3, b0, b1;
    };
    auto advance = [&]() {
        pA0 += stepA;
        pA1 += stepA;
        pA2 += stepA;
        pA3 += stepA;
        pB0 += LT_KT;
        if (RN == 4) pB1 += LT_KT;
    };
    auto load_fast = [&]() -> Stage {
        Stage st;
        st.a0 = *pA0;
        st.a1 = *pA1;
        st.a2 = *pA2;
        st.a3 = *pA3;
        st.b0 = *pB0;
        if (RN == 4) st.b1 = *pB1;
        advance();
        return st;
    };
    auto load_tile = [&](int k0) -> Stage {
        Stage st;
        const int oB = max(0, k0 + tk - (kend - 1));
        if (CONJA) {
            st.a0 = *(pA0 - oB);
            st.a1 = *(pA1 - oB);
            st.a2 = *(pA2 - oB);
            st.a3 = *(pA3 - oB);
        } else {
            const int kk = k0 + (tid >> 7) - (kend - 1);
            st.a0 = *(pA0 - (int64_t)max(0, kk) * lda);
            st.a1 = *(pA1 - (int64_t)max(0, kk + 2) * lda);
            st.a2 = *(pA2 - (int64_t)max(0, kk + 4) * lda);
            st.a3 = *(pA3 - (int64_t)max(0, kk + 6) * lda);
        }
        st.b0 = *(pB0 - oB);
        if (RN == 4) st.b1 = *(pB1 - oB);
        advance();
        return st;
    };
    auto mask_tile = [&](Stage st, int k0) -> Stage {
        const cd czero = make_double2(0.0, 0.0);
        const bool vB = (k0 + tk) < kend;
        if (CONJA) {
            if (!vB) st.a0 = st.a1 = st.a2 = st.a3 = czero;
        } else {
            const int kk = k0 + (tid >> 7);
            if (kk >= kend) st.a0 = czero;
            if (kk + 2 >= kend) st.a1 = czero;
            if (kk + 4 >= kend) st.a2 = czero;
            if (kk + 6 >= kend) st.a3 = czero;
        }
        if (!vB) st.b0 = st.b1 = czero;
        return st;
    };
    auto store_tile = [&](int buf, const Stage& st) {
        if (CONJA) {
            sA[buf][tk][(tc) ^ tk] = st.a0;
            sA[buf][tk][(tc + 32) ^ tk] = st.a1;
            sA[buf][tk][(tc + 64) ^ tk] = st.a2;
            sA[buf][tk][(tc + 96) ^ tk] = st.a3;
        } else {
            const int kk = tid >> 7, ii = tid & 127;
            sA[buf][kk][ii] = st.a0;
            sA[buf][kk + 2][ii] = st.a1;
            sA[buf][kk + 4][ii] = st.a2;
            sA[buf][kk + 6][ii] = st.a3;
        }
        sB[buf][tk][(tc) ^ tk] = st.b0;
        if (RN == 4) sB[buf][tk][(tc + 32) ^ tk] = st.b1;
    };
    struct Frag {
        cd a[GEMM_RM], b[RN];
    };
    auto read_frag = [&](int buf, int h) -> Frag {
        Frag f;
        const int kk = 2 * lk + h;
#pragma unroll
        for (int a = 0; a < GEMM_RM; ++a) {
            const int c = wave * (GEMM_RM * 16) + a * 16 + li;
            f.a[a] = sA[buf][kk][CONJA ? (c ^ kk) : c];
        }
#pragma unroll
        for (int b = 0; b < RN; ++b) {
            const int c = b * 16 + li;
            f.b[b] = sB[buf][kk][c ^ kk];
        }
        return f;
    };
    auto mfma_half = [&](const Frag& f, auto nopred_tag) {
        constexpr bool NOPRED = decltype(nopred_tag)::value;
        double bs[RN];
#pragma unroll
        for (int b = 0; b < RN; ++b) bs[b] = f.b[b].x + f.b[b].y;
#pragma unroll
        for (int a = 0; a < GEMM_RM; ++a) {
            if (NOPRED || a < rmv) {
                const double ar = f.a[a].x, ai = f.a[a].y;
                const double as = CONJA ? ar - ai : ar + ai;
#pragma unroll
                for (int b = 0; b < RN; ++b)
                    if (NOPRED || b < rnv) acc1[a][b] = __builtin_amdgcn_mfma_f64_16x16x4f64(ar, f.b[b].x, acc1[a][b], 0, 0, 0);
#pragma unroll
                for (int b = 0; b < RN; ++b)
                    if (NOPRED || b < rnv) {
                        if (REAL && CONJA)
                            acc1[a][b] = __builtin_amdgcn_mfma_f64_16x16x4f64(ai, f.b[b].y, acc1[a][b], 0, 0, 0);
                        else
                            acc2[a][b] = __builtin_amdgcn_mfma_f64_16x16x4f64(ai, REAL ? f.b[b].x : f.b[b].y, acc2[a][b],
                                                                              0, 0, 0);
                    }
                if (!REAL) {
#pragma unroll
                    for (int b = 0; b < RN; ++b)
                        if (NOPRED || b < rnv) acc3[a][b] = __builtin_amdgcn_mfma_f64_16x16x4f64(as, bs[b], acc3[a][b], 0, 0, 0);
                }
            }
        }
    };

    const int nt = (kend - kbeg + LT_KT - 1) / LT_KT;
    if (nt > 0) {
        Stage st = load_tile(kbeg);
        if (nt == 1) st = mask_tile(st, kbeg);
        store_tile(0, st);
        if (nt > 1) st = load_tile(kbeg + LT_KT);
        __syncthreads();
        Frag f0 = read_frag(0, 0);
        int t = 0;
        if (FULL) {
            for (; t + 3 < nt; ++t) {
                Frag f1 = read_frag(t & 1, 1);
                store_tile((t + 1) & 1, st);
                st = load_fast();
                mfma_half(f0, std::true_type{});
#pragma unroll
                for (int i = 0; i < GEMM_RM + RN; ++i) {
                    __builtin_amdgcn_sched_group_barrier(0x008, 1, 0);
                    __builtin_amdgcn_sched_group_barrier(0x100, 1, 0);
                }
#pragma unroll
                for (int i = 0; i < 4 + RN / 2; ++i) {
                    __builtin_amdgcn_sched_group_barrier(0x008, 1, 0);
                    __builtin_amdgcn_sched_group_barrier(0x200, 1, 0);
                    __builtin_amdgcn_sched_group_barrier(0x020, 1, 0);
                    __builtin_amdgcn_sched_group_barrier(0x002, 2, 0);
                }
                __syncthreads();
                f0 = read_frag((t + 1) & 1, 0);
                mfma_half(f1, std::true_type{});
#pragma unroll
                for (int i = 0; i < GEMM_RM + RN; ++i) {
                    __builtin_amdgcn_sched_group_barrier(0x008, 2, 1);
                    __builtin_amdgcn_sched_group_barrier(0x100, 1, 1);
                }
            }
        }
        for (; t < nt; ++t) {
            const bool more = (t + 1) < nt;
            Frag f1 = read_frag(t & 1, 1);
            if (more) {
                if (t + 2 == nt) st = mask_tile(st, kbeg + (t + 1) * LT_KT);
                store_tile((t + 1) & 1, st);
                if (t + 2 < nt) st = load_tile(kbeg + (t + 2) * LT_KT);
            }
            if (active) mfma_half(f0, std::integral_constant<bool, FULL>{});
            __syncthreads();
            if (more) f0 = read_frag((t + 1) & 1, 0);
            if (active) mfma_half(f1, std::integral_constant<bool, FULL>{});
        }
    }
    if (!active) return;

    const int j0 = J0;
    const bool direct = (slab == nullptr);
    cd* sl = direct ? nullptr : slab + (int64_t)z * m * n;
#pragma unroll
    for (int a = 0; a < GEMM_RM; ++a)
#pragma unroll
        for (int b = 0; b < RN; ++b)
#pragma unroll
            for (int r = 0; r < 4; ++r) {
                const int gi = i0 + a * 16 + lk + 4 * r;
                const int gj = j0 + b * 16 + li;
                if (gi < m && gj < n && gj >= jmin && gi >= imin) {
                    const double p1 = acc1[a][b][r], p2 = acc2[a][b][r], p3 = acc3[a][b][r];
                    const double vr = REAL ? p1 : (CONJA ? p1 + p2 : p1 - p2);
                    const double vi = REAL ? (CONJA ? 0.0 : p2) : (CONJA ? p3 - p1 + p2 : p3 - p1 - p2);
                    if (direct) {
                        cd* c = C + gi + (int64_t)gj * ldc;
                        cd o = make_double2(alpha.x * vr - alpha.y * vi, alpha.x * vi + alpha.y * vr);
                        if (beta.x != 0.0 || beta.y != 0.0) {
                            const cd old = *c;
                            o.x += beta.x * old.x - beta.y * old.y;
                            o.y += beta.x * old.y + beta.y * old.x;
                        }
                        *c = o;
                    } else {
                        sl[gi + (int64_t)gj * m] = make_double2(vr, vi);
                    }
                }
            }
}

#define REDUCE_UPPER_BN 64
__global__ void k_zgemm_reduce(int m, int n, int mi, int nj, int nsI, const cd* __restrict__ slabI, int nsB,
                               const cd* __restrict__ slabB, cd* __restrict__ C, int64_t ldc, cd alpha, cd beta,
                               int upper) {
    const int64_t idx = (int64_t)blockIdx.x * blockDim.x + threadIdx.x;
    if (idx >= (int64_t)m * n) return;
    const int j = (int)(idx / m);
    const int i = (int)(idx - (int64_t)j * m);
    if ((upper & 1) && (i / GEMM_BM) * GEMM_BM >= (j / REDUCE_UPPER_BN) * REDUCE_UPPER_BN + REDUCE_UPPER_BN)
        return;
    const bool interior = i < mi && j < nj;
    const int nsplit = interior ? nsI : nsB;
    const cd* slab = interior ? slabI : slabB;
    if (nsplit < 0) return;
    double sr = 0.0, si = 0.0;
    for (int z = 0; z < nsplit; ++z) {
        const cd v = slab[(int64_t)z * m * n + idx];
        sr += v.x;
        si += v.y;
    }
    cd* c = C + i + (int64_t)j * ldc;
    cd o = make_double2(alpha.x * sr - alpha.y * si, alpha.x * si + alpha.y * sr);
    if (beta.x != 0.0 || beta.y != 0.0) {
        const cd old = *c;
        o.x += beta.x * old.x - beta.y * old.y;
        o.y += beta.x * old.y + beta.y * old.x;
    }
    *c = o;
}

template <bool CONJA>
__global__ void k_zgemm_naive(int m, int n, int K, const cd* __restrict__ A, int64_t lda,
                              const cd* __restrict__ B, int64_t ldb, cd* __restrict__ C, int64_t ldc, cd alpha,
                              cd beta, int real) {
    const int64_t idx = (int64_t)blockIdx.x * blockDim.x + threadIdx.x;
    if (idx >= (int64_t)m * n) return;
    const int j = (int)(idx / m);
    const int i = (int)(idx - (int64_t)j * m);
    double sr = 0.0, si = 0.0;
    for (int k = 0; k < K; ++k) {
        cd a = CONJA ? A[k + (int64_t)i * lda] : A[i + (int64_t)k * lda];
        if (CONJA) a.y = -a.y;
        cd b = B[k + (int64_t)j * ldb];
        if (real && !CONJA) b.y = 0.0;
        sr += a.x * b.x - a.y * b.y;
        si += a.x * b.y + a.y * b.x;
    }
    if (real && CONJA) si = 0.0;
    cd* c = C + i + (int64_t)j * ldc;
    cd o = make_double2(alpha.x * sr - alpha.y * si, alpha.x * si + alpha.y * sr);
    if (beta.x != 0.0 || beta.y != 0.0) {
        const cd old = *c;
        o.x += beta.x * old.x - beta.y * old.y;
        o.y += beta.x * old.y + beta.y * old.x;
    }
    *c = o;
}

__global__ __launch_bounds__(256) void k_mfma_peak(int iters, double* out) {
    v4d acc[8];
#pragma unroll
    for (int i = 0; i < 8; ++i) acc[i] = (v4d){0.0, 0.0, 0.0, 0.0};
    double a = 1.0 + threadIdx.x * 1e-9, bb = 1.0 - threadIdx.x * 1e-9;
    for (int it = 0; it < iters; ++it) {
#pragma unroll
        for (int i = 0; i < 8; ++i) acc[i] = __builtin_amdgcn_mfma_f64_16x16x4f64(a, bb, acc[i], 0, 0, 0);
    }
    double s = 0.0;
#pragma unroll
    for (int i = 0; i < 8; ++i) s += acc[i][0] + acc[i][1] + acc[i][2] + acc[i][3];
    if (s == 12345.678) out[0] = s;
}

template <int NACC>
__global__ __launch_bounds__(256) void k_mfma_cycles(int iters, double* out) {
    v4d acc[8];
#pragma unroll
    for (int i = 0; i < 8; ++i) acc[i] = (v4d){0.0, 0.0, 0.0, 0.0};
    double a = 1.0 + threadIdx.x * 1e-9, bb = 1.0 - threadIdx.x * 1e-9;
    const long long c0 = clock64();
    const long long w0 = wall_clock64();
    for (int it = 0; it < iters; ++it) {
#pragma unroll
        for (int i = 0; i < 8; ++i)
            acc[i % NACC] = __builtin_amdgcn_mfma_f64_16x16x4f64(a, bb, acc[i % NACC], 0, 0, 0);
    }
    double s = 0.0;
#pragma unroll
    for (int i = 0; i < 8; ++i) s += acc[i][0] + acc[i][1] + acc[i][2] + acc[i][3];
    const long long c1 = clock64();
    const long long w1 = wall_clock64();
    if (blockIdx.x == 0 && threadIdx.x == 0) {
        out[1] = (double)(c1 - c0);
        out[2] = (double)(w1 - w0);
        out[3] = s;
    }
}

extern "C" int dftk_mi_diag_mfma_peak(dftk_mi_basis* b, int waves_per_simd, int iters, double* tflops) {
    if (!b || !tflops || waves_per_simd < 1 || iters < 1) return DFTK_MI_EINVAL;
    HIPCHK(hipSetDevice(b->device));
    hipEvent_t e0, e1;
    HIPCHK(hipEventCreate(&e0));
    HIPCHK(hipEventCreate(&e1));
    const int blocks = 256 * waves_per_simd;
    hipLaunchKernelGGL(k_mfma_peak, dim3(blocks), dim3(256), 0, b->stream, 10, b->d_scalars);
    HIPCHK(hipEventRecord(e0, b->stream));
    hipLaunchKernelGGL(k_mfma_peak, dim3(blocks), dim3(256), 0, b->stream, iters, b->d_scalars);
    HIPCHK(hipEventRecord(e1, b->stream));
    HIPCHK(hipEventSynchronize(e1));
    float ms = 0.f;
    HIPCHK(hipEventElapsedTime(&ms, e0, e1));
    const double flops = (double)blocks * 4.0 * iters * 8.0 * 2048.0;
    *tflops = flops / (ms * 1e-3) / 1e12;
    for (int nacc : {8, 2, 1}) {
        if (nacc == 8) hipLaunchKernelGGL(k_mfma_cycles<8>, dim3(blocks), dim3(256), 0, b->stream, iters, b->d_scalars);
        if (nacc == 2) hipLaunchKernelGGL(k_mfma_cycles<2>, dim3(blocks), dim3(256), 0, b->stream, iters, b->d_scalars);
        if (nacc == 1) hipLaunchKernelGGL(k_mfma_cycles<1>, dim3(blocks), dim3(256), 0, b->stream, iters, b->d_scalars);
        HIPCHK(hipMemcpyAsync(b->h_scalars, b->d_scalars, 4 * sizeof(double), hipMemcpyDeviceToHost, b->stream));
        HIPCHK(hipStreamSynchronize(b->stream));
        fprintf(stderr, "[diag] %d wave(s)/SIMD, %d independent accumulators: %.1f shader clocks per MFMA, clock %.0f MHz\n",
                waves_per_simd, nacc, b->h_scalars[1] / (8.0 * iters), b->h_scalars[1] / (b->h_scalars[2] / 100.0));
    }
    hipEventDestroy(e0);
    hipEventDestroy(e1);
    return 0;
}

int ensure_ws(dftk_mi_basis* b, size_t bytes) {
    return scratch_grow(b, b->ws, bytes, bytes / 4);
}

struct Split {
    int nsplit, kchunk;
    bool zmajor;
    cd* slab;
    bool compact = false;
    int live = 0;
};
#define GEMM_SLOTS (256 * M3_MIN_BLOCKS)
static Split gemm_plan_split(int64_t m, int64_t n, int64_t k, int upper, const std::vector<int>& live_rows, bool border,
                             bool compact_ok = false) {
    const int64_t slots = GEMM_SLOTS;
    const int64_t plane = (int64_t)m * n * (int64_t)sizeof(cd);
    static std::map<std::vector<int64_t>, std::pair<int, int>> plan_cache;
    static std::mutex plan_mutex;
    std::lock_guard<std::mutex> plan_lock(plan_mutex);
    const bool rot_rows = (upper & 1) && (int)live_rows.size() <= 4;
    int64_t total = 0;
    for (int v : live_rows) total += v;
    const int gm_s = (int)live_rows.size();
    int best_ns = 1, best_zm = compact_ok ? 2 : 0;
    if (k >= 128 && total > 0 && total < slots) {
        const std::vector<int64_t> key = {m, n, k, (int64_t)(upper & 1), (int64_t)border, (int64_t)rot_rows,
                                          (int64_t)compact_ok};
        auto it = plan_cache.find(key);
        if (it != plan_cache.end()) {
            best_ns = it->second.first;
            best_zm = it->second.second;
        } else {
            int64_t max_ns = k >= 2048 ? k / 256 : k / 64;
            if (max_ns > 1024) max_ns = 1024;
            const int64_t max_by_ws = (int64_t)(1024ull << 20) / plane;
            if (max_ns > max_by_ws) max_ns = max_by_ws;
            if (max_ns > 2 * slots / total + 8) max_ns = 2 * slots / total + 8;
            if (max_ns < 1) max_ns = 1;
            const double per_xcd = (double)slots / 8.0;
            const double slab_cost = 2.0 * (double)plane / 5e12 / 3.7e-6;
            double best = 1e300;
            for (int ns = 1; ns <= max_ns; ++ns) {
                int kc = (int)((k + ns - 1) / ns);
                kc = (kc + 7) & ~7;
                if ((int)((k + kc - 1) / kc) != ns) continue;
                for (int zm = 0; zm < 3; ++zm) {
                    if (zm == 1 && (ns < 8 || k < 2048)) continue;
                    if (zm == 2 && !compact_ok) continue;
                    int64_t load[8] = {0, 0, 0, 0, 0, 0, 0, 0};
                    if (zm == 2) {
                        load[0] = (total * ns + 7) / 8;
                    } else if (zm) {
                        for (int z = 0; z < ns; ++z) load[z & 7] += total;
                    } else {
                        const int64_t R = (int64_t)gm_s * ns;
                        const int g8 = (gm_s % 8 == 0) ? 8 : (gm_s % 4 == 0) ? 4 : (gm_s % 2 == 0) ? 2 : 1;
                        for (int64_t r = 0; r < R; ++r) {
                            const int64_t z = r / gm_s;
                            const int64_t row = rot_rows ? (r % gm_s + (z * g8) / 8) % gm_s : r % gm_s;
                            load[r & 7] += live_rows[row];
                        }
                    }
                    int64_t mx = 0;
                    for (int x = 0; x < 8; ++x) mx = load[x] > mx ? load[x] : mx;
                    const double rounds = std::ceil((double)mx / per_xcd);
                    const double cost = rounds * (kc / 8.0 + 12.0) + (ns > 1 ? slab_cost * ns : 0.0) - 1e-3 * zm;
                    if (cost < best) {
                        best = cost;
                        best_ns = ns;
                        best_zm = zm;
                    }
                }
            }
            if (plan_cache.size() > 4096) plan_cache.clear();
            plan_cache[key] = {best_ns, best_zm};
        }
    }
    int kc = (int)((k + best_ns - 1) / best_ns);
    kc = (kc + 7) & ~7;
    const int ns = (int)((k + kc - 1) / kc);
    Split sp{ns, kc, best_zm == 1 && ns >= 8, nullptr};
    sp.compact = best_zm == 2;
    sp.live = (int)total;
    return sp;
}

struct GemmTiling {
    int BNt;
    int gm, gmf, gnf, gnt, nright, nbottom;
    int shift;
    int gnI;
    int shift_r;
    int gmI;
    Split I, B;
};
static GemmTiling gemm_tiling(int64_t m, int64_t n, int64_t k, int upper, bool real) {
    GemmTiling t;
    t.BNt = real ? M3_BN_REAL : M3_BN;
    t.gm = (int)((m + GEMM_BM - 1) / GEMM_BM);
    t.gnt = (int)((n + t.BNt - 1) / t.BNt);
    t.gmf = (int)(m / GEMM_BM);
    t.gnf = (int)(n / t.BNt);
    t.shift = (t.gnt > t.gnf && t.gnf >= 1) ? 1 : 0;
    t.gnI = t.gnf + t.shift;
    t.shift_r = (t.gm > t.gmf && t.gmf >= 1) ? 1 : 0;
    t.gmI = t.gmf + t.shift_r;
    t.nright = (t.gnt > t.gnf && !t.shift) ? t.gm : 0;
    t.nbottom = (t.gm > t.gmf && !t.shift_r) ? t.gnI : 0;
    auto live = [&](int tr, int tc) {
        const int64_t jend = (t.shift && tc == t.gnf) ? n : (int64_t)tc * t.BNt + t.BNt;
        return !(upper & 1) || (int64_t)tr * GEMM_BM < jend;
    };
    std::vector<int> rowsI(t.gmI, 0), rowsB(t.nright + t.nbottom, 0);
    for (int tr = 0; tr < t.gmI; ++tr)
        for (int tc = 0; tc < t.gnI; ++tc) rowsI[tr] += live(tr, tc) ? 1 : 0;
    for (int e = 0; e < t.nright; ++e) rowsB[e] = live(e, t.gnf) ? 1 : 0;
    for (int e = 0; e < t.nbottom; ++e) rowsB[t.nright + e] = live(t.gmf, e) ? 1 : 0;
    bool compact_ok = (upper & 1) && GEMM_BM % t.BNt == 0;
    for (int tr = 0; tr < t.gmI && compact_ok; ++tr)
        compact_ok = rowsI[tr] == std::max(0, t.gnI - tr * (GEMM_BM / t.BNt));
    t.I = gemm_plan_split(m, n, k, upper, rowsI, false, compact_ok);
    t.B = gemm_plan_split(m, n, k, upper, rowsB, true);
    return t;
}
int zgemm_plan_host(char transA, int64_t m, int64_t n, int64_t k, int flags, int* out) {
    if (m <= 0 || n <= 0 || k <= 0 || (flags & ~(3 | DFTK_MI_GEMM_REAL)) || !out) return DFTK_MI_EINVAL;
    (void)transA;
    const GemmTiling t = gemm_tiling(m, n, k, flags & 3, (flags & DFTK_MI_GEMM_REAL) != 0);
    const int v[12] = {t.BNt, t.gmf, t.gnf, t.nright, t.nbottom, t.I.nsplit, t.I.kchunk, t.I.compact ? 2 : t.I.zmajor ? 1 : 0,
                       t.B.nsplit, t.B.kchunk, t.B.zmajor ? 1 : 0, t.shift};
    for (int i = 0; i < 12; ++i) out[i] = v[i];
    return 0;
}

int zgemm(dftk_mi_basis* b, char transA, int64_t m, int64_t n, int64_t k, cd alpha, const cd* A, int64_t lda,
          const cd* B, int64_t ldb, cd beta, cd* C, int64_t ldc, int upper_in) {
    const int upper = upper_in & 3;
    const bool real = (upper_in & DFTK_MI_GEMM_REAL) != 0;
    if (m <= 0 || n <= 0) return 0;
    const bool conja = (transA == 'C' || transA == 'c');
    if (!conja && !(transA == 'N' || transA == 'n')) {
        dftk_set_error("zgemm: transA must be 'N' or 'C'");
        return DFTK_MI_EINVAL;
    }
    if (m > INT32_MAX || n > INT32_MAX || k > INT32_MAX) return DFTK_MI_EINVAL;
    if (batching()) {
        BOp o;
        o.b = b;
        o.type = BOP_ZGEMM; o.trans = conja ? 'C' : 'N'; o.gm = m; o.gn = n; o.gk = k; o.alpha = alpha; o.A = A; o.lda = lda;
        o.B = B; o.ldb = ldb; o.beta = beta; o.C = C; o.ldc = ldc; o.flags = upper_in;
        return batch_record(std::move(o));
    }
    if (k <= 0) {
        hipLaunchKernelGGL(k_zgemm_reduce, dim3((unsigned)((m * n + 255) / 256)), dim3(256), 0, b->stream, (int)m,
                           (int)n, (int)m, (int)n, 0, (const cd*)nullptr, 0, (const cd*)nullptr, C, ldc, alpha, beta, 0);
        HIPCHK(hipGetLastError());
        return 0;
    }
    static const bool trace = getenv("DFTK_MI_TRACE_GEMM") != nullptr;
    if (trace) fprintf(stderr, "[zgemm] %c %lld %lld %lld\n", transA, (long long)m, (long long)n, (long long)k);
    static const bool shapes_env = getenv("DFTK_MI_GEMM_SHAPES") != nullptr;
    const bool shapes = shapes_env || (b->prof && b->prof->shape_tags);
    const uint64_t tag = !shapes ? 0
                                 : ((uint64_t)conja << 63) | ((uint64_t)(m & 0x7FFFF) << 42) | ((uint64_t)(real ? 1 : 0) << 61) |
                                       ((uint64_t)(n & 0x3FFFF) << 22) | ((uint64_t)(upper_in & 3) << 40) |
                                       (uint64_t)(k & 0x3FFFFF) | (1ull << 62);
    const GemmTiling til = gemm_tiling(m, n, k, upper, real);
    double useful = 0.0, executed = 0.0;
    if (b->prof && b->prof->on) {
        const double mac_useful = real ? 4.0 : 8.0;
        if (!(upper & 3)) {
            useful = mac_useful * (double)m * (double)n * (double)k;
        } else {
            for (int64_t j = 0; j < n; ++j) {
                const double rows = (upper & 1) ? (double)std::min<int64_t>(m, j + 1) : (double)m;
                const double kk = (upper & 2) ? (double)std::min<int64_t>(k, j + 1) : (double)k;
                useful += mac_useful * rows * kk;
            }
        }
        const double per_mac = real ? 4.0 : b->use_mfma ? 6.0 : 8.0;
        const int BNt = til.BNt;
        auto kext = [&](int tc) {
            const int64_t j0 = (til.shift && tc == til.gnf) ? n - BNt : (int64_t)tc * BNt;
            return (double)((upper & 2) ? std::min<int64_t>(k, j0 + BNt) : k);
        };
        auto live = [&](int64_t i0, int tc) {
            const int64_t jend = (til.shift && tc == til.gnf) ? n : std::min<int64_t>(n, (int64_t)tc * BNt + BNt);
            return !(upper & 1) || i0 < jend;
        };
        for (int tr = 0; tr < til.gmI; ++tr)
            for (int tc = 0; tc < til.gnI; ++tc)
                if (live((int64_t)tr * GEMM_BM, tc)) executed += per_mac * GEMM_BM * BNt * kext(tc);
        const int64_t mrem = m - (int64_t)til.gmf * GEMM_BM;
        const double rows_b = (double)(((mrem + 31) / 32) * 32);
        for (int tc = 0; tc < til.nbottom; ++tc)
            if (live((int64_t)til.gmf * GEMM_BM, tc)) executed += per_mac * rows_b * BNt * kext(tc);
        for (int tr = 0; tr < til.nright; ++tr) {
            const double rr = tr < til.gmf ? (double)GEMM_BM : rows_b;
            if (live((int64_t)tr * GEMM_BM, til.gnf)) executed += per_mac * rr * BNt * kext(til.gnf);
        }
        if (!b->use_mfma) executed = useful;
    }
    const int slot = prof_begin(b, (upper & 3) ? PROF_ZGEMM_STRUCT : PROF_ZGEMM, useful, tag);
    if (slot >= 0) {
        b->prof->work[PROF_ZGEMM_BYTES] += 16.0 * ((double)m * k + (double)k * n +
                                                   (double)m * n * ((beta.x != 0.0 || beta.y != 0.0) ? 2.0 : 1.0));
        b->prof->work[PROF_ZGEMM_EXEC] += executed;
        b->prof->work[PROF_ZGEMM_CPLX] += real ? 2.0 * useful : useful;
    }
    struct ProfGuard {
        dftk_mi_basis* b;
        int s;
        ~ProfGuard() { prof_end(b, s); }
    } guard{b, slot};
    if (!b->use_mfma) {
        const unsigned blocks = (unsigned)((m * n + 255) / 256);
        if (conja)
            hipLaunchKernelGGL(k_zgemm_naive<true>, dim3(blocks), dim3(256), 0, b->stream, (int)m, (int)n, (int)k, A,
                               lda, B, ldb, C, ldc, alpha, beta, real ? 1 : 0);
        else
            hipLaunchKernelGGL(k_zgemm_naive<false>, dim3(blocks), dim3(256), 0, b->stream, (int)m, (int)n, (int)k,
                               A, lda, B, ldb, C, ldc, alpha, beta, real ? 1 : 0);
        HIPCHK(hipGetLastError());
        return 0;
    }
    const int64_t plane = (int64_t)m * n * (int64_t)sizeof(cd);
    auto grid_for = [&](int gm_s, int gn_s, int ns) -> int64_t {
        const int64_t rows_total = (int64_t)gm_s * ns;
        return ((rows_total + 7) / 8) * 8 * gn_s;
    };
    const int BNt = til.BNt, gmf = til.gmf, gnf = til.gnf, nright = til.nright, nbottom = til.nbottom;
    Split spI = til.I, spB = til.B;
    const size_t bytesI = spI.nsplit > 1 ? (size_t)spI.nsplit * plane : 0;
    const size_t bytesB = spB.nsplit > 1 ? (size_t)spB.nsplit * plane : 0;
    if (bytesI + bytesB) CHK(ensure_ws(b, bytesI + bytesB));
    if (bytesI) spI.slab = (cd*)b->ws.get();
    if (bytesB) spB.slab = (cd*)((char*)b->ws.get() + bytesI);
    auto launch = [&](int mode, int gm_s, int gn_s, int rt0, int ct0, int lsplit, const Split& sp) -> int {
        if (gm_s <= 0 || gn_s <= 0) return 0;
        const bool zmajor = sp.zmajor;
        const bool compact = sp.compact && mode == 1 && lsplit < 0;
        const int64_t nblk = compact  ? (((int64_t)sp.live * sp.nsplit + 7) / 8) * 8
                             : zmajor ? (int64_t)((sp.nsplit + 7) / 8) * 8 * gm_s * gn_s
                                      : grid_for(gm_s, gn_s, sp.nsplit);
        if (nblk > INT32_MAX) return DFTK_MI_EINVAL;
        dim3 grid((unsigned)nblk);
        const int upper = (upper_in & 3) | (compact ? 16 : zmajor ? 4 : 0) |
                          ((!compact && !zmajor && (upper_in & 1) && gm_s <= 4) ? 8 : 0);
#define DFTK_LAUNCH_3M(CJ, MD)                                                                                         \
    if (real) DFTK_LAUNCH_3M_(CJ, MD, true, M3_RN_REAL);                                                               \
    else DFTK_LAUNCH_3M_(CJ, MD, false, M3_RN)
#define DFTK_LAUNCH_3M_(CJ, MD, RL, RNN)                                                                               \
    hipLaunchKernelGGL((k_zgemm_3m<CJ, MD, RL, RNN>), grid, dim3(GEMM_WAVES * 64), 0, b->stream, (int)m, (int)n, (int)k,  \
                       sp.kchunk, gm_s, gn_s, rt0, ct0, lsplit, upper, til.shift ? gnf : -1,                           \
                       (til.shift_r && lsplit < 0) ? gmf : -1, sp.nsplit, A, lda, B, ldb, C,                           \
                       ldc, alpha, beta, sp.slab)
        if (conja) {
            if (mode == 1) { DFTK_LAUNCH_3M(true, 1); }
            else { DFTK_LAUNCH_3M(true, 0); }
        } else {
            if (mode == 1) { DFTK_LAUNCH_3M(false, 1); }
            else { DFTK_LAUNCH_3M(false, 0); }
        }
#undef DFTK_LAUNCH_3M
#undef DFTK_LAUNCH_3M_
        return 0;
    };
    CHK(launch(1, til.gmI, til.gnI, 0, 0, -1, spI));
    CHK(launch(0, nright + nbottom, 1, gmf, gnf, nright, spB));
    if (spI.slab || spB.slab)
        hipLaunchKernelGGL(k_zgemm_reduce, dim3((unsigned)((m * n + 255) / 256)), dim3(256), 0, b->stream, (int)m,
                           (int)n, til.shift_r ? (int)m : gmf * GEMM_BM, til.shift ? (int)n : gnf * BNt, spI.slab ? spI.nsplit : -1, spI.slab,
                           spB.slab ? spB.nsplit : -1, spB.slab, C, ldc, alpha, beta, upper);
    HIPCHK(hipGetLastError());
    return 0;
}
```

### include/dftk_mi355x.h

```cpp
#ifndef DFTK_MI355X_H
#define DFTK_MI355X_H

#include <stddef.h>
#include <stdint.h>

#ifdef __cplusplus
extern "C" {
#endif

typedef struct { double re, im; } dftk_mi_cplx;

typedef struct dftk_mi_basis  dftk_mi_basis;
typedef struct dftk_mi_kblock dftk_mi_kblock;
typedef struct dftk_mi_comm   dftk_mi_comm;

#define DFTK_MI_OK                 0
#define DFTK_MI_EINVAL            (-1)
#define DFTK_MI_EHIP              (-2)
#define DFTK_MI_ERCCL             (-3)
#define DFTK_MI_ENOGPU            (-100)
#define DFTK_MI_NUM_NONFINITE       1
#define DFTK_MI_NUM_CHOLESKY        2
#define DFTK_MI_NUM_NORMALIZATION   3
#define DFTK_MI_NUM_EIGEN           4
#define DFTK_MI_NUM_TOO_SMALL       5

const char* dftk_mi_last_error(void);
const char* dftk_mi_version(void);

int dftk_mi_basis_create(int nx, int ny, int nz, double unit_cell_volume, int device,
                         dftk_mi_basis** basis_out);
int dftk_mi_basis_destroy(dftk_mi_basis* basis);
int dftk_mi_basis_sync(dftk_mi_basis* basis);
int dftk_mi_basis_set_fft_batch(dftk_mi_basis* basis, int n_bands_per_batch);
void* dftk_mi_basis_stream(dftk_mi_basis* basis);

int dftk_mi_kblock_create(dftk_mi_basis* basis, int64_t n_G, const int64_t* mapping0_h,
                          const double* kinetic_h ,
                          dftk_mi_kblock** kb_out);
int dftk_mi_kblock_destroy(dftk_mi_kblock* kb);
int dftk_mi_kblock_set_projectors(dftk_mi_kblock* kb, int n_p, const dftk_mi_cplx* P_d, int64_t ldP,
                                  const double* D_h);
int dftk_mi_kblock_set_potential(dftk_mi_kblock* kb, const double* V_d);
int dftk_mi_kblocks_set_potential(int n_kblocks, dftk_mi_kblock* const* kbs, const double* V_d);

int dftk_mi_apply_H(dftk_mi_kblock* kb, int n_bands, const dftk_mi_cplx* psi_d, int64_t ld_psi,
                    dftk_mi_cplx* Hpsi_d, int64_t ld_Hpsi);
int dftk_mi_apply_H_parts(dftk_mi_kblock* kb, int which, int n_bands, const dftk_mi_cplx* psi_d,
                          int64_t ld_psi, dftk_mi_cplx* Hpsi_d, int64_t ld_Hpsi);

int dftk_mi_kpoint_sphere_host(int nx, int ny, int nz, const double* recip_lattice_h, const double* kcoord_h,
                               double Ecut, int64_t cap, int64_t* n_G, int64_t* mapping0_h, double* kinetic_h,
                               int32_t* G_h);
int dftk_mi_build_projectors_hgh(dftk_mi_basis* basis, int64_t n_rows, const int32_t* G_d,
                                 const double* recip_lattice_h, const double* kcoord_h, double unit_cell_volume,
                                 int n_species, const double* rp_h, const int* n_proj_h, int n_atoms,
                                 const int* species_of_atom_h, const double* positions_h, dftk_mi_cplx* P_d,
                                 int64_t ldP, int* n_p);

int dftk_mi_atomic_superposition(dftk_mi_kblock* cube_kb, int kind, const double* recip_lattice_h, int n_species,
                                 const double* params_h, int n_atoms, const int* species_of_atom_h,
                                 const double* positions_h, double* out_d);
int dftk_mi_forces_local(dftk_mi_kblock* cube_kb, const double* recip_lattice_h, int n_species, const double* params_h,
                         int n_atoms, const int* species_of_atom_h, const double* positions_h, const double* rho_d,
                         double* forces_h);
int dftk_mi_radial_transform(dftk_mi_basis* basis, int kind, int l, int n_r, const double* r_h, const double* wf_h,
                             double Zion, int64_t n_q, const double* q_d, double* out_d);
int dftk_mi_radial_tile(void);
int dftk_mi_build_projectors_radial(dftk_mi_basis* basis, int64_t n_rows, const int32_t* G_d,
                                    const double* recip_lattice_h, const double* kcoord_h, double unit_cell_volume,
                                    int n_species, const double* R_d, int64_t ldR, const int* first_chan_h,
                                    const int* n_chan_h, int n_atoms, const int* species_of_atom_h,
                                    const double* positions_h, dftk_mi_cplx* P_d, int64_t ldP, int* n_p);
int dftk_mi_atomic_superposition_table(dftk_mi_kblock* cube_kb, const double* recip_lattice_h, int n_species,
                                       const double* ff_d, int n_atoms, const int* species_of_atom_h,
                                       const double* positions_h, const double* coeff_h, double* out_d);
int dftk_mi_forces_local_table(dftk_mi_kblock* cube_kb, const double* recip_lattice_h, int n_species, const double* ff_d,
                               int n_atoms, const int* species_of_atom_h, const double* positions_h,
                               const double* rho_d, double* forces_h);
int dftk_mi_forces_nonlocal(dftk_mi_kblock* kb, const double* kcoord_h, int n_bands, const dftk_mi_cplx* psi_d,
                            int64_t ld_psi, const double* weight_h, int n_atoms, const int* col_start_h,
                            double* forces_h);

int dftk_mi_local_potential_displacement(dftk_mi_kblock* cube_kb, const double* recip_lattice_h, int n_species,
                                         const double* params_h, int species, const double* position_h, double* out_d);
int dftk_mi_dynmat_local(dftk_mi_kblock* cube_kb, const double* recip_lattice_h, int n_species, const double* params_h,
                         int n_atoms, const int* species_of_atom_h, const double* positions_h, const double* rho_d,
                         double* out_h);
int dftk_mi_nonlocal_displacement_apply(dftk_mi_kblock* kb, const double* kcoord_h, int atom, int n_atoms,
                                        const int* col_start_h, int n_bands, const dftk_mi_cplx* psi_d, int64_t ld_psi,
                                        dftk_mi_cplx* out_d, int64_t ld_out);
int dftk_mi_dynmat_nonlocal(dftk_mi_kblock* kb, const double* kcoord_h, int n_bands, const dftk_mi_cplx* psi_d,
                            int64_t ld_psi, const dftk_mi_cplx* dpsi_d, int64_t ld_dpsi, const double* w_h,
                            const double* wd_h, int n_atoms, const int* col_start_h, double* dforces_h, double* hess_h);

int dftk_mi_stress_kinetic_nonlocal(dftk_mi_kblock* kb, const double* recip_lattice_h, const double* kcoord_h,
                                    int n_bands, const dftk_mi_cplx* psi_d, int64_t ld_psi, const double* weight_h,
                                    int n_species, const double* rp_h, const int* n_proj_h, int n_atoms,
                                    const int* species_of_atom_h, const double* positions_h, const int* col_start_h,
                                    double* stress_h);
int dftk_mi_stress_cube(dftk_mi_kblock* cube_kb, const double* recip_lattice_h, int n_species, const double* params_h,
                        int n_atoms, const int* species_of_atom_h, const double* positions_h, const double* rho_d,
                        double* out_h);
int dftk_mi_stress_xc(dftk_mi_basis* basis, int64_t n, int n_spin, const double* rho_d, const double* vrho_d,
                      const double* e_d, const double* vsigma_d, const double* grad_d, double* out_h);

#define DFTK_MI_XC_LDA_X     1
#define DFTK_MI_XC_LDA_C_VWN 2
#define DFTK_MI_XC_LDA_C_PW  4
#define DFTK_MI_XC_LDA_XC_TETER93 32
int dftk_mi_local_potential(dftk_mi_kblock* cube_kb, const double* rho_d, const double* V_loc_d,
                            const double* poisson_green_d, int xc_functionals, double* V_out_d, double* energies_h);

int dftk_mi_local_potential_collinear(dftk_mi_kblock* cube_kb, const double* rho_d, const double* V_loc_d,
                                      const double* poisson_green_d, int xc_functionals, double* V_out_d,
                                      double* energies_h);

int dftk_mi_local_potential_gga(dftk_mi_kblock* cube_kb, const double* recip_lattice_h, const double* rho_d,
                                const double* V_loc_d, const double* poisson_green_d, int xc_functionals,
                                double density_threshold, double* V_out_d, double* energies_h);

int dftk_mi_local_potential_collinear_gga(dftk_mi_kblock* cube_kb, const double* recip_lattice_h, const double* rho_d,
                                          const double* V_loc_d, const double* poisson_green_d, int xc_functionals,
                                          double density_threshold, double* V_out_d, double* energies_h);

int dftk_mi_local_potential_core(dftk_mi_kblock* cube_kb, const double* recip_lattice_h, int n_spin, const double* rho_d,
                                 const double* rho_core_d, const double* grad_core_d, const double* V_loc_d,
                                 const double* poisson_green_d, int xc_functionals, double density_threshold,
                                 double* V_out_d, double* energies_h);
int dftk_mi_cube_gradient(dftk_mi_kblock* cube_kb, const double* recip_lattice_h, const double* f_d, double* grad_d);

int dftk_mi_symmetrize_rho(dftk_mi_kblock* cube_kb, int n_sym, const int32_t* S_h, const double* tau_h, int do_lowpass,
                           const double* rho_in_d, double* rho_out_d);
int dftk_mi_mix_kerker(dftk_mi_kblock* cube_kb, const double* recip_lattice_h, double kTF, const double* dF_d,
                       double* drho_d);
int dftk_mi_mix_dielectric(dftk_mi_kblock* cube_kb, const double* recip_lattice_h, double kTF, double eps_r,
                           const double* dF_d, double* drho_d);
int dftk_mi_chi0_dielectric_apply(dftk_mi_kblock* cube_kb, const double* recip_lattice_h, double kTF, double eps_r,
                                  const double* dV_d, double* out_d);
int dftk_mi_cube_fourier_filter(dftk_mi_kblock* cube_kb, const double* multiplier_d, const double* f_d, double* out_d);

#define DFTK_MI_XC_GGA_X_PBE 8
#define DFTK_MI_XC_GGA_C_PBE 16
int dftk_mi_xc_gga(dftk_mi_basis* basis, int64_t n, const double* rho_d, const double* sigma_d, int xc_functionals,
                   double density_threshold, double* e_d, double* vrho_d, double* vsigma_d);

int dftk_mi_xc_gga_spin(dftk_mi_basis* basis, int64_t n, const double* rho_d, const double* sigma_d, int xc_functionals,
                        double density_threshold, double* e_d, double* vrho_d, double* vsigma_d);

int dftk_mi_ifft_sphere(dftk_mi_kblock* kb, const dftk_mi_cplx* c_d, dftk_mi_cplx* cube_d);
int dftk_mi_fft_sphere(dftk_mi_kblock* kb, const dftk_mi_cplx* cube_d, dftk_mi_cplx* c_d);

int dftk_mi_density_accumulate(dftk_mi_kblock* kb, int n_bands, const dftk_mi_cplx* psi_d,
                               int64_t ld_psi, const double* weight_h, double* rho_d);

int dftk_mi_density_accumulate_spin(dftk_mi_kblock* kb, int n_bands, const dftk_mi_cplx* psi_d, int64_t ld_psi,
                                    const double* weight_h, double* rho_d, int spin, int n_spin);

int dftk_mi_sternheimer(dftk_mi_kblock* kb, int n_occ, const dftk_mi_cplx* psi_occ_d, int64_t ld_occ, const double* eps_h,
                        int n_extra, const dftk_mi_cplx* psi_extra_d, int64_t ld_extra, const dftk_mi_cplx* rhs_d,
                        int64_t ld_rhs, const double* tol_h, int miniter, int maxiter, const dftk_mi_cplx* dpsi0_d,
                        int64_t ld_dpsi0, dftk_mi_cplx* dpsi_d, int64_t ld_dpsi, int* n_iter, double* resid_h,
                        int* converged);
int dftk_mi_density_response_accumulate(dftk_mi_kblock* kb, int n_bands, const dftk_mi_cplx* psi_d, int64_t ld_psi,
                                        const dftk_mi_cplx* dpsi_d, int64_t ld_dpsi, const double* w_occ_h,
                                        const double* w_docc_h, double* drho_d);
int dftk_mi_apply_kernel(dftk_mi_kblock* cube_kb, const double* rho_d, const double* drho_d, const double* poisson_green_d,
                         int xc_functionals, double* dV_d);

int dftk_mi_exx_apply(dftk_mi_kblock* kb, int n_occ, const dftk_mi_cplx* phi_d, int64_t ld_phi, const double* weight_h,
                      const double* kernel_d, int n_bands, const dftk_mi_cplx* psi_d, int64_t ld_psi, dftk_mi_cplx* W_d,
                      int64_t ld_W, int accumulate);

int dftk_mi_lobpcg(dftk_mi_kblock* kb, int M, dftk_mi_cplx* X_d, int64_t ldX, double tol,
                   int miniter, int maxiter, int n_conv_check, int use_tpa, uint64_t seed,
                   double* lambda_h, double* resid_h, int* n_iter, int* converged,
                   int64_t* n_matvec);
int dftk_mi_lobpcg_multi(int n_kblocks, dftk_mi_kblock* const* kbs, int M, dftk_mi_cplx* const* X_d, const int64_t* ldX,
                         double tol, int miniter, int maxiter, int n_conv_check, int use_tpa, const uint64_t* seeds,
                         double* lambda_h, double* resid_h, int* n_iter, int* converged, int64_t* n_matvec, int* status);
int dftk_mi_density_accumulate_multi(int n_kblocks, dftk_mi_kblock* const* kbs, const int* n_bands,
                                     const dftk_mi_cplx* const* psi_d, const int64_t* ld_psi, const double* weights_h,
                                     double* rho_d);
int dftk_mi_density_accumulate_multi2(int n_kblocks, dftk_mi_kblock* const* kbs, const int* n_bands,
                                      const dftk_mi_cplx* const* psi_d, const int64_t* ld_psi, const double* weights_h,
                                      double* rho_d, const double* weights2_h, double* rho2_d);
int dftk_mi_band_kinetic_multi(int n_kblocks, dftk_mi_kblock* const* kbs, const int* n_bands,
                               const dftk_mi_cplx* const* psi_d, const int64_t* ld_psi, double* out_h);
int dftk_mi_batch_stats(int64_t* rounds, int64_t* ops, int64_t* merged_launches, int64_t* sequential_ops);
int dftk_mi_lobpcg_small_stats(int64_t* calls, int64_t* restarts);
int dftk_mi_ortho_small(dftk_mi_basis* basis, int64_t n, int m, dftk_mi_cplx* X_d, int64_t ldx, int ny, const dftk_mi_cplx* Y_d,
                        int64_t ldy, const double* norms_d, double tol, double* res4_h);
enum {
    DFTK_MI_BOP_ZGEMM = 0, DFTK_MI_BOP_COLRED = 1, DFTK_MI_BOP_RESIDUAL = 2, DFTK_MI_BOP_TPA = 3, DFTK_MI_BOP_SCALE = 4,
    DFTK_MI_BOP_COPY = 5, DFTK_MI_BOP_FILL0 = 6, DFTK_MI_BOP_SUBID = 7, DFTK_MI_BOP_GATHER = 8, DFTK_MI_BOP_ADDDIAG = 9,
    DFTK_MI_BOP_HERMIT = 10, DFTK_MI_BOP_CTRANS = 11, DFTK_MI_BOP_H2D = 12, DFTK_MI_BOP_D2H = 13, DFTK_MI_BOP_POTRF = 14,
    DFTK_MI_BOP_HEEV = 15, DFTK_MI_BOP_APPLYD = 18, DFTK_MI_BOP_ORTHO = 19
};
typedef struct dftk_mi_batch_op {
    int32_t type, fiber, trans, m, k, i0, mode, flags, join_next, sync_after;
    int32_t status;
    int32_t reserved;
    int64_t n, gm, gn, gk, lda, ldb, ldc;
    dftk_mi_cplx alpha, beta;
    double s0;
    const void *A, *B, *W, *W2, *W3;
    void *C, *D, *E, *F;
    dftk_mi_kblock* kb;
    void* host;
    uint64_t bytes;
} dftk_mi_batch_op;
int dftk_mi_batch_replay(dftk_mi_basis* basis, int n_fibers, int n_ops, dftk_mi_batch_op* ops);
int dftk_mi_lobpcg_history(dftk_mi_kblock* kb, int* M, int* n_iter, double* hist_h, size_t cap, int* n_svd);
int dftk_mi_kblock_reuse_AX(dftk_mi_kblock* kb, int on);
int dftk_mi_ax_reuse_count(int64_t* calls);
int dftk_mi_planes_reuse_count(int64_t* calls);

const dftk_mi_cplx* dftk_mi_lobpcg_last_AX(dftk_mi_kblock* kb);

int dftk_mi_columnwise_norms(dftk_mi_basis* basis, int64_t n, int m, const dftk_mi_cplx* X_d, int64_t ldx,
                             double* norms_h );
int dftk_mi_columnwise_dots(dftk_mi_basis* basis, int64_t n, int m, const dftk_mi_cplx* A_d, int64_t lda,
                            const dftk_mi_cplx* B_d, int64_t ldb, dftk_mi_cplx* dots_h );
int dftk_mi_ortho_qr(dftk_mi_basis* basis, int64_t n, int m, dftk_mi_cplx* X_d, int64_t ldx, int force_svd,
                     int* n_chol, int* used_svd);
int dftk_mi_tpa_precondprep(dftk_mi_kblock* kb, int m, const dftk_mi_cplx* X_d, int64_t ldx, double* mean_kin_h);
int dftk_mi_tpa_ldiv(dftk_mi_kblock* kb, int m, const dftk_mi_cplx* R_d, int64_t ldr, const double* mean_kin_h,
                     double default_shift, dftk_mi_cplx* Y_d, int64_t ldy);
int dftk_mi_block_residual(dftk_mi_kblock* kb, int m, const dftk_mi_cplx* AX_d, int64_t lda,
                           const dftk_mi_cplx* X_d, int64_t ldx, const double* lambda_h, dftk_mi_cplx* R_d,
                           int64_t ldr, double* norms_h, double* mean_kin_h, double* xx_h);

int dftk_mi_zgemm(dftk_mi_basis* basis, char transA, int64_t m, int64_t n, int64_t k,
                  dftk_mi_cplx alpha, const dftk_mi_cplx* A_d, int64_t lda,
                  const dftk_mi_cplx* B_d, int64_t ldb, dftk_mi_cplx beta,
                  dftk_mi_cplx* C_d, int64_t ldc);
#define DFTK_MI_GEMM_UPPER 1
#define DFTK_MI_GEMM_B_UPPER 2
#define DFTK_MI_GEMM_REAL 8
int dftk_mi_zgemm_ex(dftk_mi_basis* basis, char transA, int64_t m, int64_t n, int64_t k,
                     dftk_mi_cplx alpha, const dftk_mi_cplx* A_d, int64_t lda,
                     const dftk_mi_cplx* B_d, int64_t ldb, dftk_mi_cplx beta,
                     dftk_mi_cplx* C_d, int64_t ldc, int flags);
int dftk_mi_heev(dftk_mi_basis* basis, int n, dftk_mi_cplx* A_d, int64_t lda, double* W_h,
                 dftk_mi_cplx* V_d, int64_t ldv);
int dftk_mi_heev_lowest(dftk_mi_basis* basis, int n, int nev, dftk_mi_cplx* A_d, int64_t lda, double* W_h,
                        dftk_mi_cplx* V_d, int64_t ldv);
int dftk_mi_heev_sigma_host(int n, const double* diag_h, int nev, double* sigma, double* gap_guess,
                            int* hold_iterations, double norm_bound);
int dftk_mi_potrf_trtri(dftk_mi_basis* basis, int n, dftk_mi_cplx* A_d, int64_t lda,
                        dftk_mi_cplx* invR_d, int64_t ldi);
int dftk_mi_potrf_trtri_real(dftk_mi_basis* basis, int n, dftk_mi_cplx* A_d, int64_t lda,
                             dftk_mi_cplx* invR_d, int64_t ldi);

int dftk_mi_comm_get_unique_id(char id_out[128]);
int dftk_mi_comm_init_rank(const char id[128], int n_ranks, int rank, int device,
                           dftk_mi_comm** comm_out);
typedef int (*dftk_mi_allreduce_fn)(void* user, double* buf_h, size_t n);
typedef int (*dftk_mi_alltoallv_fn)(void* user, const double* send_h, const size_t* send_counts,
                                    const size_t* send_offsets, double* recv_h, const size_t* recv_counts,
                                    const size_t* recv_offsets);
int dftk_mi_comm_create_host(int n_ranks, int rank, int device, dftk_mi_allreduce_fn allreduce,
                             dftk_mi_alltoallv_fn alltoallv, void* user, dftk_mi_comm** comm_out);
int dftk_mi_comm_destroy(dftk_mi_comm* comm);
int dftk_mi_comm_describe(const dftk_mi_comm* comm, int* backend, int* n_ranks, int* version);
int dftk_mi_comm_rank(const dftk_mi_comm* comm);
int dftk_mi_comm_size(const dftk_mi_comm* comm);
int dftk_mi_allreduce_sum_f64(dftk_mi_comm* comm, double* buf_d, size_t n, void* stream);

int dftk_mi_kblock_set_shard(dftk_mi_kblock* kb, dftk_mi_comm* comm, const int64_t* row_starts_h);

int dftk_mi_kblock_set_gamma_real(dftk_mi_kblock* kb, int on);
int dftk_mi_gamma_half_size(dftk_mi_kblock* kb, int64_t* n_half);
int dftk_mi_gamma_tables_host(int nx, int ny, int nz, int64_t n_G, const int64_t* mapping0_h, int64_t* n_half,
                              int32_t* row_h, int32_t* partner_row_h);
int dftk_mi_gamma_compress(dftk_mi_kblock* kb, int m, const dftk_mi_cplx* X_d, int64_t ldx, dftk_mi_cplx* Xh_d,
                           int64_t ldh);
int dftk_mi_gamma_compress_aligned(dftk_mi_kblock* kb, int m, const dftk_mi_cplx* X_d, int64_t ldx, dftk_mi_cplx* Xh_d,
                                   int64_t ldh);
int dftk_mi_gamma_expand(dftk_mi_kblock* kb, int m, const dftk_mi_cplx* Xh_d, int64_t ldh, dftk_mi_cplx* X_d,
                         int64_t ldx);
int dftk_mi_gamma_apply_H(dftk_mi_kblock* kb, int which, int n_bands, const dftk_mi_cplx* psih_d, int64_t ld_psi,
                          dftk_mi_cplx* Hpsih_d, int64_t ld_Hpsi);
int dftk_mi_density_accumulate_real(dftk_mi_kblock* kb, int n_bands, const dftk_mi_cplx* psi_d, int64_t ld_psi,
                                    const double* weight_h, double* rho_d);

int dftk_mi_shard_plan_host(int n_ranks, int rank, int n_bands, const int64_t* row_starts_h, int* band_starts,
                            int64_t* slab_off, int64_t* slab_cnt, int64_t* band_off, int64_t* band_cnt);

int dftk_mi_prof_enable(dftk_mi_basis* basis, int on);
int dftk_mi_prof_get(dftk_mi_basis* basis, int family, double* total_ms, double* work, int64_t* launches);
typedef struct dftk_mi_anderson dftk_mi_anderson;
int dftk_mi_anderson_create(dftk_mi_basis* basis, int64_t n, int m, double maxcond, double errorfactor,
                            dftk_mi_anderson** out);
int dftk_mi_anderson_destroy(dftk_mi_anderson* acc);
int dftk_mi_anderson_reset(dftk_mi_anderson* acc);
int dftk_mi_anderson_history(const dftk_mi_anderson* acc);
int dftk_mi_anderson_step(dftk_mi_anderson* acc, const double* x_d, double alpha, const double* Pf_d, double* x_next_d,
                          int* n_history );
int dftk_mi_chi0_mix(dftk_mi_kblock* cube_kblock, int n_comp, const double* recip_lattice_h, const double* poisson_d,
                     const double* ldos_d, double dvol, int dielectric, double kTF, double eps_r, const double* dF_d,
                     double reltol, int krylovdim, int maxiter, double* drho_d, int* n_applies, int* converged);

int dftk_mi_launch_count(int64_t* launches, int64_t* host_syncs);

int dftk_mi_device_buffers_live(int64_t* count, int64_t* bytes);

int dftk_mi_step_sums(dftk_mi_basis* basis, int64_t n, const double* a_d, const double* b_d, const double* c_d, double* out_h);

int dftk_mi_fermi_bisection(int n_k, const int* n_bands, const double* eig, const double* kweights, int smearing,
                            double temperature, double filled, double n_electrons, double lo, double hi, double* eF_out);
int dftk_mi_prof_zgemm_shapes(dftk_mi_basis* basis, int cap, int64_t* rows6, double* ms, int* count);

int dftk_mi_diag_mfma_peak(dftk_mi_basis* basis, int waves_per_simd, int iters, double* tflops);

int dftk_mi_zgemm_plan_host(char transA, int64_t m, int64_t n, int64_t k, int flags, int* out12);
int dftk_mi_jacobi_schedule_host(int n, int round, int* n_blocks, int* pairs ,
                                 int* where );
int dftk_mi_fft_plan_host(int n, int* n_radices, int* radices , int* pos );
int dftk_mi_sphere_tables_host(int nx, int ny, int nz, int64_t n_G, const int64_t* mapping0_h,
                               int64_t* n_lines, int* n_zplanes, int64_t* line_id ,
                               int64_t* line_start );

#ifdef __cplusplus
}
#endif
#endif
```

Baseline: 5.741.

## Compute only upper triangle of symmetric eigensolver GEMM products and mirror

After: 6.277 (median of 6 runs). +9.3%, better.

```diff
diff --git a/dftk.jl_amd/_lib.py b/dftk.jl_amd/_lib.py
--- a/dftk.jl_amd/_lib.py
+++ b/dftk.jl_amd/_lib.py
@@ -156,8 +156,10 @@
     "dftk_mi_zgemm_ex": (C.c_int, [C.c_void_p, C.c_char, _i64, _i64, _i64, dftk_mi_cplx, C.c_void_p, _i64,
                                    C.c_void_p, _i64, dftk_mi_cplx, C.c_void_p, _i64, C.c_int]),
     "dftk_mi_zgemm_plan_host": (C.c_int, [C.c_char, _i64, _i64, _i64, C.c_int, C.POINTER(C.c_int)]),
+    "dftk_mi_zgemm_fold_host": (C.c_int, [C.c_char, _i64, _i64, _i64, C.c_int, C.c_int, C.POINTER(C.c_int), C.POINTER(C.c_int)]),
     "dftk_mi_heev": (C.c_int, [C.c_void_p, C.c_int, C.c_void_p, _i64, C.c_void_p, C.c_void_p, _i64]),
     "dftk_mi_prof_zgemm_shapes": (C.c_int, [C.c_void_p, C.c_int, C.c_void_p, C.c_void_p, C.POINTER(C.c_int)]),
+    "dftk_mi_eig_mirror_tall": (C.c_int, [C.c_void_p, C.c_int, C.c_int, C.c_void_p, _i64]),
     "dftk_mi_heev_lowest": (C.c_int, [C.c_void_p, C.c_int, C.c_int, C.c_void_p, _i64, C.c_void_p, C.c_void_p, _i64]),
     "dftk_mi_heev_sigma_host": (C.c_int, [C.c_int, C.c_void_p, C.c_int, C.POINTER(C.c_double), C.POINTER(C.c_double),
                                           C.POINTER(C.c_int), C.c_double]),
diff --git a/dftk.jl_amd/csrc/api.cpp b/dftk.jl_amd/csrc/api.cpp
--- a/dftk.jl_amd/csrc/api.cpp
+++ b/dftk.jl_amd/csrc/api.cpp
@@ -1401,10 +1401,15 @@
     return zgemm_plan_host(transA, m, n, k, flags, out12);
 }
 
+int zgemm_fold_host(char transA, int64_t m, int64_t n, int64_t k, int flags, int cap, int* items4, int* count);
+extern "C" int dftk_mi_zgemm_fold_host(char transA, int64_t m, int64_t n, int64_t k, int flags, int cap, int* items4, int* count) {
+    return zgemm_fold_host(transA, m, n, k, flags, cap, items4, count);
+}
+
 extern "C" int dftk_mi_zgemm_ex(dftk_mi_basis* b, char transA, int64_t m, int64_t n, int64_t k, dftk_mi_cplx alpha,
                                 const dftk_mi_cplx* A_d, int64_t lda, const dftk_mi_cplx* B_d, int64_t ldb,
                                 dftk_mi_cplx beta, dftk_mi_cplx* C_d, int64_t ldc, int flags) {
-    if (!b || m < 0 || n < 0 || k < 0 || !C_d || (flags & ~(3 | DFTK_MI_GEMM_REAL))) return DFTK_MI_EINVAL;
+    if (!b || m < 0 || n < 0 || k < 0 || !C_d || (flags & ~(3 | DFTK_MI_GEMM_REAL | DFTK_MI_GEMM_SYM_RESULT))) return DFTK_MI_EINVAL;
     HIPCHK(hipSetDevice(b->device));
     cd al = {alpha.re, alpha.im}, be = {beta.re, beta.im};
     return zgemm(b, transA, m, n, k, al, reinterpret_cast<const cd*>(A_d), lda, reinterpret_cast<const cd*>(B_d), ldb,
@@ -1416,6 +1421,12 @@
     if (!b || n < 1 || !A_d || !W_h || !V_d || lda < n || ldv < n) return DFTK_MI_EINVAL;
     HIPCHK(hipSetDevice(b->device));
     return dense_heev(b, n, reinterpret_cast<cd*>(A_d), lda, W_h, reinterpret_cast<cd*>(V_d), ldv);
+}
+
+extern "C" int dftk_mi_eig_mirror_tall(dftk_mi_basis* b, int n, int real, dftk_mi_cplx* X_d, int64_t ldt) {
+    if (!b || n < 1 || !X_d || ldt < (real ? (n + 1) / 2 : n) || 2 * ldt > INT32_MAX) return DFTK_MI_EINVAL;
+    HIPCHK(hipSetDevice(b->device));
+    return eig_mirror_tall(b, n, real != 0, reinterpret_cast<cd*>(X_d), ldt);
 }
 
 extern "C" int dftk_mi_heev_lowest(dftk_mi_basis* b, int n, int nev, dftk_mi_cplx* A_d, int64_t lda, double* W_h,
diff --git a/dftk.jl_amd/csrc/common.h b/dftk.jl_amd/csrc/common.h
--- a/dftk.jl_amd/csrc/common.h
+++ b/dftk.jl_amd/csrc/common.h
@@ -269,6 +269,8 @@
 int launch_kinetic_only(dftk_mi_kblock* kb, int nb, const cd* psi, int64_t ldpsi, cd* out,
                         int64_t ldout, bool accumulate, bool use_kin);
 
+#define GEMM_SYM_RESULT DFTK_MI_GEMM_SYM_RESULT
+bool zgemm_sym_result_pays(int64_t m, int64_t n, int64_t k, bool real);
 int zgemm(dftk_mi_basis* b, char transA, int64_t m, int64_t n, int64_t k, cd alpha, const cd* A,
           int64_t lda, const cd* B, int64_t ldb, cd beta, cd* C, int64_t ldc, int upper = 0);
 int ensure_ws(dftk_mi_basis* b, size_t bytes);
@@ -286,6 +288,7 @@
 int dense_heev_full(dftk_mi_basis* b, int n, cd* A, int64_t lda, double* W_h, cd* V, int64_t ldv);
 int dense_input_norms(dftk_mi_basis* b, int n, const cd* A, int64_t lda, double* off2, double* dg2, double* im2);
 int dense_heev_lowest(dftk_mi_basis* b, int n, int nev, cd* A, int64_t lda, double* W_h, cd* V, int64_t ldv);
+int eig_mirror_tall(dftk_mi_basis* b, int n, bool real, cd* X, int64_t ldt);
 int eig_choose_sigma_host(int n, const double* diag, int nev, double* sigma, double* gap_guess);
 int eig_hold_iterations_host(double gap_over_norm);
 struct ProfMute {
diff --git a/dftk.jl_amd/csrc/eig_kernels.hip b/dftk.jl_amd/csrc/eig_kernels.hip
--- a/dftk.jl_amd/csrc/eig_kernels.hip
+++ b/dftk.jl_amd/csrc/eig_kernels.hip
@@ -4,6 +4,7 @@
 #include <cstdio>
 #include <cstdlib>
 #include <cstring>
+#include <type_traits>
 #include <vector>
 #include <numeric>
 #include <algorithm>
@@ -98,6 +99,42 @@
     (void)ntile;
 }
 
+template <class T>
+__global__ __launch_bounds__(256) void k_eig_mirror(int n, int rows, T* __restrict__ X, int64_t ld) {
+    __shared__ T tile[EPT][EPT + 1];
+    int t = blockIdx.x, bj = 0;
+    while (t > bj) {
+        t -= bj + 1;
+        ++bj;
+    }
+    const int bi = t;
+    const int tx = threadIdx.x & 31, ty = threadIdx.x >> 5;
+    constexpr bool CPLX = std::is_same<T, cd>::value;
+#pragma unroll
+    for (int r = 0; r < EPT; r += 8) {
+        const int i = bi * EPT + tx, j = bj * EPT + ty + r;
+        T v = T();
+        if (i < n && j < n && i <= j) v = X[i + (int64_t)j * ld];
+        if constexpr (CPLX) {
+            if (i == j && i < n && v.y != 0.0) {
+                v.y = 0.0;
+                X[i + (int64_t)j * ld] = v;
+            }
+        }
+        tile[ty + r][tx] = v;
+    }
+    __syncthreads();
+#pragma unroll
+    for (int r = 0; r < EPT; r += 8) {
+        const int j = bj * EPT + tx, i = bi * EPT + ty + r;
+        if (i < n && j < rows && i < j) {
+            T v = tile[tx][ty + r];
+            if constexpr (CPLX) v.y = -v.y;
+            X[j + (int64_t)i * ld] = v;
+        }
+    }
+}
+
 template <bool REAL>
 __global__ void k_eig_diag_tall(int n, const cd* __restrict__ U, int64_t ldt, double* __restrict__ d) {
     const int c = blockIdx.x * blockDim.x + threadIdx.x;
@@ -141,6 +178,17 @@
 double a_of(double l) { return std::sqrt(3.0 / (1.0 + l + l * l)); }
 double l_next(double l, double a) { return 0.5 * a * l * (3.0 - a * a * l * l); }
 
+}
+
+int eig_mirror_tall(dftk_mi_basis* b, int n, bool real, cd* X, int64_t ldt) {
+    const int mrows = real ? 2 * (int)ldt : n, mt1 = (mrows + EPT - 1) / EPT;
+    if (real)
+        hipLaunchKernelGGL(k_eig_mirror<double>, dim3(mt1 * (mt1 + 1) / 2), dim3(256), 0, b->stream, n, mrows,
+                           reinterpret_cast<double*>(X), 2 * ldt);
+    else
+        hipLaunchKernelGGL(k_eig_mirror<cd>, dim3(mt1 * (mt1 + 1) / 2), dim3(256), 0, b->stream, n, mrows, X, ldt);
+    HIPCHK(hipGetLastError());
+    return 0;
 }
 
 int eig_choose_sigma_host(int n, const double* diag, int nev, double* sigma, double* gap_guess) {
@@ -237,8 +285,10 @@
         HIPCHK(hipGetLastError());
         return 0;
     };
+    const bool sym = zgemm_sym_result_pays(ldt, n, n, REAL);
     auto advance = [&]() -> int {
-        CHK(zgemm(b, 'N', ldt, n, n, ONE, Xc, ldt, Y, n, ZERO, Xn, ldt, rf));
+        CHK(zgemm(b, 'N', ldt, n, n, ONE, Xc, ldt, Y, n, ZERO, Xn, ldt, rf | (sym ? GEMM_SYM_RESULT : 0)));
+        if (sym) CHK(eig_mirror_tall(b, n, REAL, Xn, ldt));
         Xc = Xn;
         Xn = (Xc == Xa) ? Xb : Xa;
         ++its;
diff --git a/dftk.jl_amd/csrc/gemm_kernels.hip b/dftk.jl_amd/csrc/gemm_kernels.hip
--- a/dftk.jl_amd/csrc/gemm_kernels.hip
+++ b/dftk.jl_amd/csrc/gemm_kernels.hip
@@ -21,7 +21,16 @@
 #define M3_RN_REAL 4
 #define M3_BN_REAL (16 * M3_RN_REAL)
 #define M3_MIN_BLOCKS 2
-template <bool CONJA, int MODE, bool REAL, int RN>
+__host__ __device__ inline bool gemm_fold_item(int id, int gm, int gn, int* row_t, int* col1, int* col2) {
+    const int xcd = id & 7, slot = id >> 3;
+    const int np = (gn + 1) >> 1, p = slot % np;
+    *row_t = (slot / np) * 8 + xcd;
+    *col1 = gn - 1 - p;
+    *col2 = (p != gn - 1 - p) ? p : -1;
+    return *row_t < gm;
+}
+
+template <bool CONJA, int MODE, bool REAL, int RN, bool FOLD = false>
 __global__ __launch_bounds__(GEMM_WAVES * 64, M3_MIN_BLOCKS) void k_zgemm_3m(int m, int n, int K, int kchunk, int gm, int gn,
                                                                int rt0, int ct0, int lsplit, int upper,
                                                                int shift_ct, int shift_rt, int nsplit, const cd* __restrict__ A, int64_t lda,
@@ -35,8 +44,12 @@
     const int id = blockIdx.x;
     const int xcd = id & 7, slot = id >> 3;
     int z, row_t, col_t;
-    if (upper & 16) {
-        constexpr int q = GEMM_BM / BN;
+    int col2 = -1;
+    if (FOLD) {
+        if (!gemm_fold_item(id, gm, gn, &row_t, &col_t, &col2)) return;
+        z = 0;
+    } else if (upper & 16) {
+        const int q = (GEMM_BM << ((upper >> 5) & 1)) / BN;
         int L = 0;
         for (int r = 0; r < gm; ++r) L += max(0, gn - r * q);
         const int N = L * nsplit, per = (N + 7) >> 3;
@@ -73,15 +86,15 @@
     const int lane = tid & 63, wave = tid >> 6;
     const int li = lane & 15, lk = lane >> 4;
     const int tr = lsplit < 0 ? row_t + rt0 : (row_t < lsplit ? row_t : rt0);
-    const int tcn = lsplit < 0 ? col_t + ct0 : (row_t < lsplit ? ct0 : row_t - lsplit);
-    const bool shifted = tcn == shift_ct;
+    int tcn = lsplit < 0 ? col_t + ct0 : (row_t < lsplit ? ct0 : row_t - lsplit);
+    bool shifted = tcn == shift_ct;
     const bool rshifted = tr == shift_rt;
-    const int I0 = rshifted ? m - GEMM_BM : tr * GEMM_BM, J0 = shifted ? n - BN : tcn * BN;
-    const int jmin = shifted ? tcn * BN : 0, imin = tr * GEMM_BM;
-    if ((upper & 1) && imin >= J0 + BN) return;
+    const int I0 = rshifted ? m - GEMM_BM : tr * GEMM_BM, imin = tr * GEMM_BM;
+    int J0 = shifted ? n - BN : tcn * BN, jmin = shifted ? tcn * BN : 0;
+    if ((upper & 1) && (imin << ((upper >> 5) & 1)) >= J0 + BN) return;
     const int i0 = I0 + wave * (GEMM_RM * 16);
     const int kbeg = z * kchunk;
-    const int kend = min(min(K, kbeg + kchunk), (upper & 2) ? J0 + BN : K);
+    int kend = min(min(K, kbeg + kchunk), (upper & 2) ? J0 + BN : K);
     constexpr bool FULL = MODE == 1;
     const int rmv = FULL ? GEMM_RM : min(GEMM_RM, max(0, (m - i0 + 15) >> 4));
     const int rnv = FULL ? RN : min(RN, max(0, (n - J0 + 15) >> 4));
@@ -99,7 +112,7 @@
 
     const int tk = tid & 7, tc = tid >> 3;
     const cd *pA0, *pA1, *pA2, *pA3, *pB0, *pB1;
-    {
+    auto init_ptrs = [&]() {
         auto a_ptr = [&](int r) -> const cd* {
             if (CONJA) {
                 int c = I0 + tc + 32 * r;
@@ -122,7 +135,8 @@
         pA3 = a_ptr(3);
         pB0 = b_ptr(0);
         pB1 = b_ptr(RN == 4 ? 1 : 0);
-    }
+    };
+    init_ptrs();
     const int64_t stepA = CONJA ? (int64_t)LT_KT : (int64_t)LT_KT * lda;
     struct Stage {
         cd a0, a1, a2, a3, b0, b1;
@@ -181,7 +195,8 @@
         if (!vB) st.b0 = st.b1 = czero;
         return st;
     };
-    auto store_tile = [&](int buf, const Stage& st) {
+    int cB0 = (upper & 2) ? J0 + tc - tk : INT32_MAX, cB1 = (upper & 2) ? J0 + tc + 32 - tk : INT32_MAX;
+    auto store_tile = [&](int buf, const Stage& st, int k0) {
         if (CONJA) {
             sA[buf][tk][(tc) ^ tk] = st.a0;
             sA[buf][tk][(tc + 32) ^ tk] = st.a1;
@@ -194,8 +209,14 @@
             sA[buf][kk + 4][ii] = st.a2;
             sA[buf][kk + 6][ii] = st.a3;
         }
-        sB[buf][tk][(tc) ^ tk] = st.b0;
-        if (RN == 4) sB[buf][tk][(tc + 32) ^ tk] = st.b1;
+        if (!CONJA) {
+            const bool z0 = k0 > cB0, z1 = k0 > cB1;
+            sB[buf][tk][(tc) ^ tk] = make_double2(z0 ? 0.0 : st.b0.x, z0 ? 0.0 : st.b0.y);
+            if (RN == 4) sB[buf][tk][(tc + 32) ^ tk] = make_double2(z1 ? 0.0 : st.b1.x, z1 ? 0.0 : st.b1.y);
+        } else {
+            sB[buf][tk][(tc) ^ tk] = st.b0;
+            if (RN == 4) sB[buf][tk][(tc + 32) ^ tk] = st.b1;
+        }
     };
     struct Frag {
         cd a[GEMM_RM], b[RN];
@@ -246,88 +267,113 @@
         }
     };
 
-    const int nt = (kend - kbeg + LT_KT - 1) / LT_KT;
-    if (nt > 0) {
-        Stage st = load_tile(kbeg);
-        if (nt == 1) st = mask_tile(st, kbeg);
-        store_tile(0, st);
-        if (nt > 1) st = load_tile(kbeg + LT_KT);
-        __syncthreads();
-        Frag f0 = read_frag(0, 0);
-        int t = 0;
-        if (FULL) {
-            for (; t + 3 < nt; ++t) {
-                Frag f1 = read_frag(t & 1, 1);
-                store_tile((t + 1) & 1, st);
-                st = load_fast();
-                mfma_half(f0, std::true_type{});
-#pragma unroll
-                for (int i = 0; i < GEMM_RM + RN; ++i) {
-                    __builtin_amdgcn_sched_group_barrier(0x008, 1, 0);
-                    __builtin_amdgcn_sched_group_barrier(0x100, 1, 0);
-                }
-#pragma unroll
-                for (int i = 0; i < 4 + RN / 2; ++i) {
-                    __builtin_amdgcn_sched_group_barrier(0x008, 1, 0);
-                    __builtin_amdgcn_sched_group_barrier(0x200, 1, 0);
-                    __builtin_amdgcn_sched_group_barrier(0x020, 1, 0);
-                    __builtin_amdgcn_sched_group_barrier(0x002, 2, 0);
-                }
-                __syncthreads();
-                f0 = read_frag((t + 1) & 1, 0);
-                mfma_half(f1, std::true_type{});
-#pragma unroll
-                for (int i = 0; i < GEMM_RM + RN; ++i) {
-                    __builtin_amdgcn_sched_group_barrier(0x008, 2, 1);
-                    __builtin_amdgcn_sched_group_barrier(0x100, 1, 1);
-                }
-            }
-        }
-        for (; t < nt; ++t) {
-            const bool more = (t + 1) < nt;
-            Frag f1 = read_frag(t & 1, 1);
-            if (more) {
-                if (t + 2 == nt) st = mask_tile(st, kbeg + (t + 1) * LT_KT);
-                store_tile((t + 1) & 1, st);
-                if (t + 2 < nt) st = load_tile(kbeg + (t + 2) * LT_KT);
-            }
-            if (active) mfma_half(f0, std::integral_constant<bool, FULL>{});
-            __syncthreads();
-            if (more) f0 = read_frag((t + 1) & 1, 0);
-            if (active) mfma_half(f1, std::integral_constant<bool, FULL>{});
-        }
-    }
-    if (!active) return;
-
-    const int j0 = J0;
+    int nt = (kend - kbeg + LT_KT - 1) / LT_KT;
+    Stage st;
+    if (nt > 0) st = load_tile(kbeg);
     const bool direct = (slab == nullptr);
     cd* sl = direct ? nullptr : slab + (int64_t)z * m * n;
-#pragma unroll
-    for (int a = 0; a < GEMM_RM; ++a)
-#pragma unroll
-        for (int b = 0; b < RN; ++b)
-#pragma unroll
-            for (int r = 0; r < 4; ++r) {
-                const int gi = i0 + a * 16 + lk + 4 * r;
-                const int gj = j0 + b * 16 + li;
-                if (gi < m && gj < n && gj >= jmin && gi >= imin) {
-                    const double p1 = acc1[a][b][r], p2 = acc2[a][b][r], p3 = acc3[a][b][r];
-                    const double vr = REAL ? p1 : (CONJA ? p1 + p2 : p1 - p2);
-                    const double vi = REAL ? (CONJA ? 0.0 : p2) : (CONJA ? p3 - p1 + p2 : p3 - p1 - p2);
-                    if (direct) {
-                        cd* c = C + gi + (int64_t)gj * ldc;
-                        cd o = make_double2(alpha.x * vr - alpha.y * vi, alpha.x * vi + alpha.y * vr);
-                        if (beta.x != 0.0 || beta.y != 0.0) {
-                            const cd old = *c;
-                            o.x += beta.x * old.x - beta.y * old.y;
-                            o.y += beta.x * old.y + beta.y * old.x;
-                        }
-                        *c = o;
-                    } else {
-                        sl[gi + (int64_t)gj * m] = make_double2(vr, vi);
+    for (int pass = 0;; ++pass) {
+        if (nt > 0) {
+            if (nt == 1) st = mask_tile(st, kbeg);
+            store_tile(0, st, kbeg);
+            if (nt > 1) st = load_tile(kbeg + LT_KT);
+            __syncthreads();
+            Frag f0 = read_frag(0, 0);
+            int t = 0;
+            if (FULL) {
+                for (; t + 3 < nt; ++t) {
+                    Frag f1 = read_frag(t & 1, 1);
+                    store_tile((t + 1) & 1, st, kbeg + (t + 1) * LT_KT);
+                    st = load_fast();
+                    mfma_half(f0, std::true_type{});
+#pragma unroll
+                    for (int i = 0; i < GEMM_RM + RN; ++i) {
+                        __builtin_amdgcn_sched_group_barrier(0x008, 1, 0);
+                        __builtin_amdgcn_sched_group_barrier(0x100, 1, 0);
+                    }
+#pragma unroll
+                    for (int i = 0; i < 4 + RN / 2; ++i) {
+                        __builtin_amdgcn_sched_group_barrier(0x008, 1, 0);
+                        __builtin_amdgcn_sched_group_barrier(0x200, 1, 0);
+                        __builtin_amdgcn_sched_group_barrier(0x020, 1, 0);
+                        __builtin_amdgcn_sched_group_barrier(0x002, 2, 0);
+                    }
+                    __syncthreads();
+                    f0 = read_frag((t + 1) & 1, 0);
+                    mfma_half(f1, std::true_type{});
+#pragma unroll
+                    for (int i = 0; i < GEMM_RM + RN; ++i) {
+                        __builtin_amdgcn_sched_group_barrier(0x008, 2, 1);
+                        __builtin_amdgcn_sched_group_barrier(0x100, 1, 1);
                     }
                 }
             }
+            for (; t < nt; ++t) {
+                const bool more = (t + 1) < nt;
+                Frag f1 = read_frag(t & 1, 1);
+                if (more) {
+                    if (t + 2 == nt) st = mask_tile(st, kbeg + (t + 1) * LT_KT);
+                    store_tile((t + 1) & 1, st, kbeg + (t + 1) * LT_KT);
+                    if (t + 2 < nt) st = load_tile(kbeg + (t + 2) * LT_KT);
+                }
+                if (active) mfma_half(f0, std::integral_constant<bool, FULL>{});
+                __syncthreads();
+                if (more) f0 = read_frag((t + 1) & 1, 0);
+                if (active) mfma_half(f1, std::integral_constant<bool, FULL>{});
+            }
+        }
+        if (!active) return;
+
+        const int j0 = J0, jm = jmin;
+        const bool again = FOLD && pass == 0 && col2 >= 0;
+        if (again) {
+            tcn = col2 + ct0;
+            shifted = tcn == shift_ct;
+            J0 = shifted ? n - BN : tcn * BN;
+            jmin = shifted ? tcn * BN : 0;
+            kend = min(min(K, kbeg + kchunk), (upper & 2) ? J0 + BN : K);
+            nt = (kend - kbeg + LT_KT - 1) / LT_KT;
+            cB0 = (upper & 2) ? J0 + tc - tk : INT32_MAX;
+            cB1 = (upper & 2) ? J0 + tc + 32 - tk : INT32_MAX;
+            init_ptrs();
+            if (nt > 0) st = load_tile(kbeg);
+        }
+#pragma unroll
+        for (int a = 0; a < GEMM_RM; ++a)
+#pragma unroll
+            for (int b = 0; b < RN; ++b)
+#pragma unroll
+                for (int r = 0; r < 4; ++r) {
+                    const int gi = i0 + a * 16 + lk + 4 * r;
+                    const int gj = j0 + b * 16 + li;
+                    if (gi < m && gj < n && gj >= jm && gi >= imin) {
+                        const double p1 = acc1[a][b][r], p2 = acc2[a][b][r], p3 = acc3[a][b][r];
+                        const double vr = REAL ? p1 : (CONJA ? p1 + p2 : p1 - p2);
+                        const double vi = REAL ? (CONJA ? 0.0 : p2) : (CONJA ? p3 - p1 + p2 : p3 - p1 - p2);
+                        if (direct) {
+                            cd* c = C + gi + (int64_t)gj * ldc;
+                            cd o = make_double2(alpha.x * vr - alpha.y * vi, alpha.x * vi + alpha.y * vr);
+                            if (beta.x != 0.0 || beta.y != 0.0) {
+                                const cd old = *c;
+                                o.x += beta.x * old.x - beta.y * old.y;
+                                o.y += beta.x * old.y + beta.y * old.x;
+                            }
+                            *c = o;
+                        } else {
+                            sl[gi + (int64_t)gj * m] = make_double2(vr, vi);
+                        }
+                    }
+                }
+        if (!again) break;
+#pragma unroll
+        for (int a = 0; a < GEMM_RM; ++a)
+#pragma unroll
+            for (int b = 0; b < RN; ++b) {
+                acc1[a][b] = (v4d){0.0, 0.0, 0.0, 0.0};
+                acc2[a][b] = (v4d){0.0, 0.0, 0.0, 0.0};
+                acc3[a][b] = (v4d){0.0, 0.0, 0.0, 0.0};
+            }
+    }
 }
 
 #define REDUCE_UPPER_BN 64
@@ -338,7 +384,8 @@
     if (idx >= (int64_t)m * n) return;
     const int j = (int)(idx / m);
     const int i = (int)(idx - (int64_t)j * m);
-    if ((upper & 1) && (i / GEMM_BM) * GEMM_BM >= (j / REDUCE_UPPER_BN) * REDUCE_UPPER_BN + REDUCE_UPPER_BN)
+    if ((upper & 1) &&
+        (((i / GEMM_BM) * GEMM_BM) << ((upper >> 5) & 1)) >= min(n, (j / REDUCE_UPPER_BN) * REDUCE_UPPER_BN + REDUCE_UPPER_BN))
         return;
     const bool interior = i < mi && j < nj;
     const int nsplit = interior ? nsI : nsB;
@@ -471,7 +518,7 @@
 };
 #define GEMM_SLOTS (256 * M3_MIN_BLOCKS)
 static Split gemm_plan_split(int64_t m, int64_t n, int64_t k, int upper, const std::vector<int>& live_rows, bool border,
-                             bool compact_ok = false) {
+                             bool compact_ok = false, int rsc = 1) {
     const int64_t slots = GEMM_SLOTS;
     const int64_t plane = (int64_t)m * n * (int64_t)sizeof(cd);
     static std::map<std::vector<int64_t>, std::pair<int, int>> plan_cache;
@@ -484,7 +531,7 @@
     int best_ns = 1, best_zm = compact_ok ? 2 : 0;
     if (k >= 128 && total > 0 && total < slots) {
         const std::vector<int64_t> key = {m, n, k, (int64_t)(upper & 1), (int64_t)border, (int64_t)rot_rows,
-                                          (int64_t)compact_ok};
+                                          (int64_t)compact_ok, (int64_t)rsc};
         auto it = plan_cache.find(key);
         if (it != plan_cache.end()) {
             best_ns = it->second.first;
@@ -553,7 +600,7 @@
     int gmI;
     Split I, B;
 };
-static GemmTiling gemm_tiling(int64_t m, int64_t n, int64_t k, int upper, bool real) {
+static GemmTiling gemm_tiling(int64_t m, int64_t n, int64_t k, int upper, bool real, int rsc = 1) {
     GemmTiling t;
     t.BNt = real ? M3_BN_REAL : M3_BN;
     t.gm = (int)((m + GEMM_BM - 1) / GEMM_BM);
@@ -568,24 +615,57 @@
     t.nbottom = (t.gm > t.gmf && !t.shift_r) ? t.gnI : 0;
     auto live = [&](int tr, int tc) {
         const int64_t jend = (t.shift && tc == t.gnf) ? n : (int64_t)tc * t.BNt + t.BNt;
-        return !(upper & 1) || (int64_t)tr * GEMM_BM < jend;
+        return !(upper & 1) || (int64_t)tr * GEMM_BM * rsc < jend;
     };
     std::vector<int> rowsI(t.gmI, 0), rowsB(t.nright + t.nbottom, 0);
     for (int tr = 0; tr < t.gmI; ++tr)
         for (int tc = 0; tc < t.gnI; ++tc) rowsI[tr] += live(tr, tc) ? 1 : 0;
     for (int e = 0; e < t.nright; ++e) rowsB[e] = live(e, t.gnf) ? 1 : 0;
     for (int e = 0; e < t.nbottom; ++e) rowsB[t.nright + e] = live(t.gmf, e) ? 1 : 0;
-    bool compact_ok = (upper & 1) && GEMM_BM % t.BNt == 0;
+    bool compact_ok = (upper & 1) && (GEMM_BM * rsc) % t.BNt == 0;
     for (int tr = 0; tr < t.gmI && compact_ok; ++tr)
-        compact_ok = rowsI[tr] == std::max(0, t.gnI - tr * (GEMM_BM / t.BNt));
-    t.I = gemm_plan_split(m, n, k, upper, rowsI, false, compact_ok);
-    t.B = gemm_plan_split(m, n, k, upper, rowsB, true);
+        compact_ok = rowsI[tr] == std::max(0, t.gnI - tr * (GEMM_BM * rsc / t.BNt));
+    t.I = gemm_plan_split(m, n, k, upper, rowsI, false, compact_ok, rsc);
+    t.B = gemm_plan_split(m, n, k, upper, rowsB, true, false, rsc);
     return t;
 }
+bool zgemm_sym_result_pays(int64_t m, int64_t n, int64_t k, bool real) {
+    if (m <= 0 || n <= 0 || k <= 0) return false;
+    const GemmTiling t = gemm_tiling(m, n, k, 0, real);
+    return (int64_t)t.gmI * t.gnI * t.I.nsplit > GEMM_SLOTS;
+}
+
+static bool gemm_folds(const GemmTiling& t, bool conja, int upper) {
+    return !conja && (upper & 3) == 2 && t.I.nsplit == 1 && !t.I.zmajor && t.gmI >= 1 && t.gnI >= 2;
+}
+int zgemm_fold_host(char transA, int64_t m, int64_t n, int64_t k, int flags, int cap, int* items4, int* count) {
+    if (m <= 0 || n <= 0 || k <= 0 || (flags & ~(3 | DFTK_MI_GEMM_REAL)) || cap < 0 || !count || (cap > 0 && !items4))
+        return DFTK_MI_EINVAL;
+    const GemmTiling t = gemm_tiling(m, n, k, flags & 3, (flags & DFTK_MI_GEMM_REAL) != 0);
+    *count = 0;
+    if (!gemm_folds(t, transA == 'C' || transA == 'c', flags & 3)) return 0;
+    const int nblk = ((t.gmI + 7) / 8) * 8 * ((t.gnI + 1) / 2);
+    for (int id = 0; id < nblk; ++id) {
+        int row, c[2];
+        if (!gemm_fold_item(id, t.gmI, t.gnI, &row, &c[0], &c[1])) continue;
+        for (int i = 0; i < 2; ++i) {
+            if (c[i] < 0) continue;
+            if (*count < cap) {
+                const int64_t j0 = (t.shift && c[i] == t.gnf) ? n - t.BNt : (int64_t)c[i] * t.BNt;
+                int* e = items4 + 4 * (int64_t)*count;
+                e[0] = row; e[1] = c[i]; e[2] = 0; e[3] = (int)std::min<int64_t>(k, j0 + t.BNt);
+            }
+            ++*count;
+        }
+    }
+    return 0;
+}
+
 int zgemm_plan_host(char transA, int64_t m, int64_t n, int64_t k, int flags, int* out) {
-    if (m <= 0 || n <= 0 || k <= 0 || (flags & ~(3 | DFTK_MI_GEMM_REAL)) || !out) return DFTK_MI_EINVAL;
+    if (m <= 0 || n <= 0 || k <= 0 || (flags & ~(3 | DFTK_MI_GEMM_REAL | DFTK_MI_GEMM_SYM_RESULT)) || !out) return DFTK_MI_EINVAL;
     (void)transA;
-    const GemmTiling t = gemm_tiling(m, n, k, flags & 3, (flags & DFTK_MI_GEMM_REAL) != 0);
+    const bool real = (flags & DFTK_MI_GEMM_REAL) != 0, sym = (flags & DFTK_MI_GEMM_SYM_RESULT) != 0;
+    const GemmTiling t = gemm_tiling(m, n, k, (flags & 3) | (sym ? 1 : 0), real, (sym && real) ? 2 : 1);
     const int v[12] = {t.BNt, t.gmf, t.gnf, t.nright, t.nbottom, t.I.nsplit, t.I.kchunk, t.I.compact ? 2 : t.I.zmajor ? 1 : 0,
                        t.B.nsplit, t.B.kchunk, t.B.zmajor ? 1 : 0, t.shift};
     for (int i = 0; i < 12; ++i) out[i] = v[i];
@@ -594,10 +674,16 @@
 
 int zgemm(dftk_mi_basis* b, char transA, int64_t m, int64_t n, int64_t k, cd alpha, const cd* A, int64_t lda,
           const cd* B, int64_t ldb, cd beta, cd* C, int64_t ldc, int upper_in) {
-    const int upper = upper_in & 3;
     const bool real = (upper_in & DFTK_MI_GEMM_REAL) != 0;
     if (m <= 0 || n <= 0) return 0;
     const bool conja = (transA == 'C' || transA == 'c');
+    const bool sym = (upper_in & GEMM_SYM_RESULT) != 0;
+    if (sym && conja) {
+        dftk_set_error("zgemm: GEMM_SYM_RESULT is a flag of 'N' products");
+        return DFTK_MI_EINVAL;
+    }
+    const int upper = (upper_in & 3) | (sym ? 1 : 0);
+    const int rsc = (sym && real) ? 2 : 1;
     if (!conja && !(transA == 'N' || transA == 'n')) {
         dftk_set_error("zgemm: transA must be 'N' or 'C'");
         return DFTK_MI_EINVAL;
@@ -607,7 +693,8 @@
         BOp o;
         o.b = b;
         o.type = BOP_ZGEMM; o.trans = conja ? 'C' : 'N'; o.gm = m; o.gn = n; o.gk = k; o.alpha = alpha; o.A = A; o.lda = lda;
-        o.B = B; o.ldb = ldb; o.beta = beta; o.C = C; o.ldc = ldc; o.flags = upper_in;
+        o.B = B; o.ldb = ldb; o.beta = beta; o.C = C; o.ldc = ldc;
+        o.flags = upper_in & ~GEMM_SYM_RESULT;
         return batch_record(std::move(o));
     }
     if (k <= 0) {
@@ -624,7 +711,7 @@
                                  : ((uint64_t)conja << 63) | ((uint64_t)(m & 0x7FFFF) << 42) | ((uint64_t)(real ? 1 : 0) << 61) |
                                        ((uint64_t)(n & 0x3FFFF) << 22) | ((uint64_t)(upper_in & 3) << 40) |
                                        (uint64_t)(k & 0x3FFFFF) | (1ull << 62);
-    const GemmTiling til = gemm_tiling(m, n, k, upper, real);
+    const GemmTiling til = gemm_tiling(m, n, k, upper, real, rsc);
     double useful = 0.0, executed = 0.0;
     if (b->prof && b->prof->on) {
         const double mac_useful = real ? 4.0 : 8.0;
@@ -632,7 +719,7 @@
             useful = mac_useful * (double)m * (double)n * (double)k;
         } else {
             for (int64_t j = 0; j < n; ++j) {
-                const double rows = (upper & 1) ? (double)std::min<int64_t>(m, j + 1) : (double)m;
+                const double rows = (upper & 1) ? std::min((double)m, (double)(j + 1) / rsc) : (double)m;
                 const double kk = (upper & 2) ? (double)std::min<int64_t>(k, j + 1) : (double)k;
                 useful += mac_useful * rows * kk;
             }
@@ -645,7 +732,7 @@
         };
         auto live = [&](int64_t i0, int tc) {
             const int64_t jend = (til.shift && tc == til.gnf) ? n : std::min<int64_t>(n, (int64_t)tc * BNt + BNt);
-            return !(upper & 1) || i0 < jend;
+            return !(upper & 1) || i0 * rsc < jend;
         };
         for (int tr = 0; tr < til.gmI; ++tr)
             for (int tc = 0; tc < til.gnI; ++tc)
@@ -699,24 +786,29 @@
         if (gm_s <= 0 || gn_s <= 0) return 0;
         const bool zmajor = sp.zmajor;
         const bool compact = sp.compact && mode == 1 && lsplit < 0;
-        const int64_t nblk = compact  ? (((int64_t)sp.live * sp.nsplit + 7) / 8) * 8
-                             : zmajor ? (int64_t)((sp.nsplit + 7) / 8) * 8 * gm_s * gn_s
-                                      : grid_for(gm_s, gn_s, sp.nsplit);
+        const bool fold = mode == 1 && lsplit < 0 && gemm_folds(til, conja, upper);
+        const int64_t nblk = fold      ? grid_for(gm_s, (gn_s + 1) / 2, 1)
+                             : compact ? (((int64_t)sp.live * sp.nsplit + 7) / 8) * 8
+                             : zmajor  ? (int64_t)((sp.nsplit + 7) / 8) * 8 * gm_s * gn_s
+                                       : grid_for(gm_s, gn_s, sp.nsplit);
         if (nblk > INT32_MAX) return DFTK_MI_EINVAL;
         dim3 grid((unsigned)nblk);
-        const int upper = (upper_in & 3) | (compact ? 16 : zmajor ? 4 : 0) |
-                          ((!compact && !zmajor && (upper_in & 1) && gm_s <= 4) ? 8 : 0);
+        const int kupper = upper | (compact ? 16 : zmajor ? 4 : 0) | ((!compact && !zmajor && (upper & 1) && gm_s <= 4) ? 8 : 0) |
+                           (rsc == 2 ? 32 : 0);
 #define DFTK_LAUNCH_3M(CJ, MD)                                                                                         \
-    if (real) DFTK_LAUNCH_3M_(CJ, MD, true, M3_RN_REAL);                                                               \
-    else DFTK_LAUNCH_3M_(CJ, MD, false, M3_RN)
-#define DFTK_LAUNCH_3M_(CJ, MD, RL, RNN)                                                                               \
-    hipLaunchKernelGGL((k_zgemm_3m<CJ, MD, RL, RNN>), grid, dim3(GEMM_WAVES * 64), 0, b->stream, (int)m, (int)n, (int)k,  \
-                       sp.kchunk, gm_s, gn_s, rt0, ct0, lsplit, upper, til.shift ? gnf : -1,                           \
+    if (real) DFTK_LAUNCH_3M_(CJ, MD, true, M3_RN_REAL, false);                                                        \
+    else DFTK_LAUNCH_3M_(CJ, MD, false, M3_RN, false)
+#define DFTK_LAUNCH_3M_(CJ, MD, RL, RNN, FD)                                                                           \
+    hipLaunchKernelGGL((k_zgemm_3m<CJ, MD, RL, RNN, FD>), grid, dim3(GEMM_WAVES * 64), 0, b->stream, (int)m, (int)n, (int)k,  \
+                       sp.kchunk, gm_s, gn_s, rt0, ct0, lsplit, kupper, til.shift ? gnf : -1,                          \
                        (til.shift_r && lsplit < 0) ? gmf : -1, sp.nsplit, A, lda, B, ldb, C,                           \
                        ldc, alpha, beta, sp.slab)
         if (conja) {
             if (mode == 1) { DFTK_LAUNCH_3M(true, 1); }
             else { DFTK_LAUNCH_3M(true, 0); }
+        } else if (fold) {
+            if (real) DFTK_LAUNCH_3M_(false, 1, true, M3_RN_REAL, true);
+            else DFTK_LAUNCH_3M_(false, 1, false, M3_RN, true);
         } else {
             if (mode == 1) { DFTK_LAUNCH_3M(false, 1); }
             else { DFTK_LAUNCH_3M(false, 0); }
@@ -730,7 +822,7 @@
     if (spI.slab || spB.slab)
         hipLaunchKernelGGL(k_zgemm_reduce, dim3((unsigned)((m * n + 255) / 256)), dim3(256), 0, b->stream, (int)m,
                            (int)n, til.shift_r ? (int)m : gmf * GEMM_BM, til.shift ? (int)n : gnf * BNt, spI.slab ? spI.nsplit : -1, spI.slab,
-                           spB.slab ? spB.nsplit : -1, spB.slab, C, ldc, alpha, beta, upper);
+                           spB.slab ? spB.nsplit : -1, spB.slab, C, ldc, alpha, beta, upper | (rsc == 2 ? 32 : 0));
     HIPCHK(hipGetLastError());
     return 0;
 }
diff --git a/include/dftk_mi355x.h b/include/dftk_mi355x.h
--- a/include/dftk_mi355x.h
+++ b/include/dftk_mi355x.h
@@ -238,6 +238,7 @@
 #define DFTK_MI_GEMM_UPPER 1
 #define DFTK_MI_GEMM_B_UPPER 2
 #define DFTK_MI_GEMM_REAL 8
+#define DFTK_MI_GEMM_SYM_RESULT 32
 int dftk_mi_zgemm_ex(dftk_mi_basis* basis, char transA, int64_t m, int64_t n, int64_t k,
                      dftk_mi_cplx alpha, const dftk_mi_cplx* A_d, int64_t lda,
                      const dftk_mi_cplx* B_d, int64_t ldb, dftk_mi_cplx beta,
@@ -246,6 +247,7 @@
                  dftk_mi_cplx* V_d, int64_t ldv);
 int dftk_mi_heev_lowest(dftk_mi_basis* basis, int n, int nev, dftk_mi_cplx* A_d, int64_t lda, double* W_h,
                         dftk_mi_cplx* V_d, int64_t ldv);
+int dftk_mi_eig_mirror_tall(dftk_mi_basis* basis, int n, int real, dftk_mi_cplx* X_d, int64_t ldt);
 int dftk_mi_heev_sigma_host(int n, const double* diag_h, int nev, double* sigma, double* gap_guess,
                             int* hold_iterations, double norm_bound);
 int dftk_mi_potrf_trtri(dftk_mi_basis* basis, int n, dftk_mi_cplx* A_d, int64_t lda,
@@ -315,6 +317,7 @@
 int dftk_mi_diag_mfma_peak(dftk_mi_basis* basis, int waves_per_simd, int iters, double* tflops);
 
 int dftk_mi_zgemm_plan_host(char transA, int64_t m, int64_t n, int64_t k, int flags, int* out12);
+int dftk_mi_zgemm_fold_host(char transA, int64_t m, int64_t n, int64_t k, int flags, int cap, int* items4, int* count);
 int dftk_mi_jacobi_schedule_host(int n, int round, int* n_blocks, int* pairs ,
                                  int* where );
 int dftk_mi_fft_plan_host(int n, int* n_radices, int* radices , int* pos );
```
